# mario-linov/graphs4cfd

Measured on AMD Instinct MI355X. Metric: rollout timesteps/s (100k-node 2D mesh), higher is better.
Workload: dtype f32 (MLP products: two-way fp16 split of both operands, 22 significand bits each, 3 partial products on the f16 MFMA pipe, fp32 accumulate; error vs fp64 within that of an fp32 GEMM)

## Files before the change

### graphs4cfd_amd/_lib.py

```python
from __future__ import annotations

import ctypes as C
import os
from typing import Optional

import torch

_HERE = os.path.dirname(os.path.abspath(__file__))
LIB_PATH = os.environ.get("G4C_LIB_PATH") or os.path.join(_HERE, "lib", "libg4c.so")

OK, EINVAL, ELAUNCH, EUNSUPPORTED = 0, -1, -2, -3
ACT_NONE, ACT_SELU, ACT_TANH = 0, 1, 2
MAX_SRC, MAX_LAYERS = 4, 4
MAX_HEADS = 2
NARROW_MAX = 8
KERNEL_MLP_RS = 5
KERNEL_MLP_RS2 = 6
KERNEL_MLP_BX6, KERNEL_MLP_WS = 2, 4
KERNEL_MLP_BX6_CERT, KERNEL_MLP_WS_CERT = 7, 8
KERNEL_NAMES = {0: "none", 1: "mlp_split_kernel", 2: "mlp_bx6_kernel", 3: "mlp_bx6i_kernel", 4: "mlp_ws_kernel", 5: "mlp_rs1_kernel", 6: "mlp_rs2_kernel",
                7: "mlp_bx6_kernel", 8: "mlp_ws_kernel"}

TILE_SHAPE_GENERIC, TILE_SHAPE_NODE, TILE_SHAPE_UP, TILE_SHAPE_DOWN = 0, 1, 2, 3

_ACT_CODES = {None: ACT_NONE, "none": ACT_NONE, "selu": ACT_SELU, "tanh": ACT_TANH}


def act_code(activation) -> Optional[int]:
    if activation is None or isinstance(activation, str):
        return _ACT_CODES[activation]
    if activation is torch.tanh or activation is torch.nn.functional.tanh:
        return ACT_TANH
    if activation is torch.nn.functional.selu or activation is torch.selu:
        return ACT_SELU
    return None


class g4c_src_t(C.Structure):
    _fields_ = [("ptr", C.c_void_p), ("idx", C.c_void_p), ("width", C.c_int32), ("ld", C.c_int32),
                ("col0", C.c_int32), ("pre_act", C.c_int32), ("additive", C.c_int32), ("seg_mean", C.c_int32),
                ("w", C.c_void_p), ("seg_off", C.c_void_p), ("seg_perm", C.c_void_p), ("dtype", C.c_int32)]


class g4c_mlp_t(C.Structure):
    _fields_ = [("n_layers", C.c_int32), ("k_pad", C.c_int32 * MAX_LAYERS), ("n_pad", C.c_int32 * MAX_LAYERS),
                ("w", C.c_void_p * MAX_LAYERS), ("b", C.c_void_p * MAX_LAYERS),
                ("ln_gamma", C.c_void_p), ("ln_beta", C.c_void_p), ("ln_eps", C.c_float), ("n_out", C.c_int32), ("w_format", C.c_int32),
                ("range_slot", C.c_int32), ("range_certified", C.c_int32)]


WFMT_FP32, WFMT_F16X2, WFMT_BF16X3, WFMT_BF16_RS, WFMT_BF16_RS2, WFMT_BF16_RS2N, WFMT_BF16 = 0, 1, 2, 3, 4, 5, 6
DTYPE_F32, DTYPE_BF16 = 0, 1


class g4c_mlp_io_t(C.Structure):
    _fields_ = [("size", C.c_int32), ("act", C.c_int32), ("row_begin", C.c_int64), ("row_count", C.c_int64),
                ("out", C.c_void_p), ("out_ld", C.c_int32), ("out_dtype", C.c_int32), ("out_idx", C.c_void_p),
                ("resid", C.c_void_p), ("resid_ld", C.c_int32), ("resid_col0", C.c_int32),
                ("n_heads", C.c_int32), ("head_ld", C.c_int32), ("head_dtype", C.c_int32), ("head_out", C.c_void_p * MAX_HEADS),
                ("tile_rows", C.c_void_p), ("tile_seg", C.c_void_p), ("seg_off", C.c_void_p), ("n_tiles", C.c_int32),
                ("agg", C.c_void_p), ("agg_ld", C.c_int32), ("agg_mode", C.c_int32),
                ("n_save", C.c_int32), ("save", C.c_void_p * MAX_LAYERS), ("save_ld", C.c_int32),
                ("mul", C.c_void_p * MAX_LAYERS), ("mul_ld", C.c_int32),
                ("upd", C.POINTER(g4c_mlp_t)), ("v", C.c_void_p), ("v_ld", C.c_int32), ("v_act", C.c_int32),
                ("v_out", C.c_void_p), ("v_out_ld", C.c_int32), ("range_flag", C.c_void_p),
                ("save_dtype", C.c_int32), ("mul_dtype", C.c_int32)]

    def __init__(self, **kw):
        super().__init__(size=C.sizeof(g4c_mlp_io_t), **kw)


_SIGNATURES = {
    "g4c_version": (C.c_int, []),
    "g4c_device_info": (C.c_int, [C.c_void_p, C.POINTER(C.c_int32), C.POINTER(C.c_int32)]),
    "g4c_last_error": (C.c_char_p, []),
    "g4c_plan_csr": (C.c_int, [C.c_void_p, C.c_int64, C.c_int64, C.c_void_p, C.c_void_p]),
    "g4c_plan_pool_edge": (C.c_int64, [C.c_void_p, C.c_int64, C.c_void_p, C.c_int64, C.c_void_p, C.c_void_p,
                                       C.c_void_p, C.c_void_p]),
    "g4c_plan_pool_edge_ordered": (C.c_int64, [C.c_void_p, C.c_int64, C.c_void_p, C.c_int64, C.c_int32, C.c_void_p, C.c_void_p,
                                               C.c_void_p, C.c_void_p]),
    "g4c_segment_reduce": (C.c_int, [C.c_void_p, C.c_int32, C.c_void_p, C.c_void_p, C.c_int32, C.c_int32, C.c_int32,
                                     C.c_int32, C.c_int32, C.c_void_p, C.c_int32, C.c_void_p]),
    "g4c_weighted_segment_mean": (C.c_int, [C.c_void_p, C.c_int32, C.c_void_p, C.c_void_p, C.c_void_p, C.c_int32,
                                            C.c_int32, C.c_void_p, C.c_int32, C.c_void_p, C.c_void_p]),
    "g4c_mlp_pack_layer": (C.c_int, [C.c_void_p, C.c_int32, C.c_int32, C.c_void_p, C.c_void_p, C.c_int32, C.c_int32, C.c_void_p,
                                     C.c_int32, C.c_int32, C.c_void_p]),
    "g4c_mlp_run": (C.c_int, [C.POINTER(g4c_mlp_t), C.POINTER(g4c_src_t), C.c_int32, C.c_int64, C.POINTER(g4c_mlp_io_t), C.c_void_p]),
    "g4c_plan_tiles": (C.c_int64, [C.c_void_p, C.c_int32, C.c_int32, C.c_void_p, C.c_void_p, C.c_int64]),
    "g4c_mlp_bx6i_enable": (C.c_int, [C.c_int]),
    "g4c_mlp_ws_enable": (C.c_int, [C.c_int]),
    "g4c_mlp_small_launch_tiles": (C.c_int, [C.c_int]),
    "g4c_layer_norm": (C.c_int, [C.c_void_p, C.c_int32, C.c_int64, C.c_int32, C.c_void_p, C.c_void_p, C.c_float, C.c_int32, C.c_void_p, C.c_int32, C.c_void_p]),
    "g4c_debug_mean_div": (C.c_int, [C.c_void_p, C.c_void_p, C.c_void_p, C.c_int64, C.c_void_p]),
    "g4c_mlp_last_kernel": (C.c_int, []),
    "g4c_mlp_shapes_enable": (C.c_int, [C.c_int]),
    "g4c_mlp_last_shape": (C.c_int, []),
    "g4c_project_to_edges": (C.c_int, [C.c_void_p, C.c_int32, C.c_void_p, C.c_void_p, C.c_int64, C.c_int32,
                                       C.c_void_p, C.c_int32, C.c_void_p]),
    "g4c_edge_scalar_to_node_vector": (C.c_int, [C.c_void_p, C.c_int32, C.c_void_p, C.c_int32, C.c_int64, C.c_int32,
                                                 C.c_void_p, C.c_int32, C.c_void_p]),
    "g4c_knn_grid": (C.c_int, [C.c_void_p, C.c_void_p, C.c_void_p, C.c_void_p, C.c_int64, C.c_int32, C.c_void_p,
                               C.c_void_p, C.c_float, C.c_int32, C.c_void_p, C.c_void_p]),
    "g4c_knn_grid_query": (C.c_int, [C.c_void_p, C.c_void_p, C.c_void_p, C.c_int64, C.c_int32, C.c_void_p, C.c_void_p,
                                     C.c_float, C.c_void_p, C.c_void_p, C.c_int64, C.c_int32, C.c_void_p, C.c_void_p]),
    "g4c_rollout_advance": (C.c_int, [C.c_void_p, C.c_int32, C.c_void_p, C.c_int32, C.c_void_p, C.c_int32,
                                      C.c_void_p, C.c_int64, C.c_void_p]),
    "g4c_activation_inplace": (C.c_int, [C.c_void_p, C.c_int64, C.c_int32, C.c_void_p]),
    "g4c_add_cols": (C.c_int, [C.c_void_p, C.c_int32, C.c_int32, C.c_void_p, C.c_int32, C.c_void_p, C.c_int32,
                               C.c_int32, C.c_int64, C.c_void_p]),
    "g4c_copy_cols": (C.c_int, [C.c_void_p, C.c_int32, C.c_int32, C.c_void_p, C.c_void_p, C.c_int32, C.c_int32,
                                C.c_int32, C.c_int64, C.c_void_p]),
    "g4c_train_gather": (C.c_int, [C.c_void_p, C.c_int32, C.c_int32, C.c_void_p, C.c_int32, C.c_int32, C.c_void_p, C.c_int32,
                                   C.c_int32, C.c_int32, C.c_int64, C.c_int32, C.c_void_p]),
    "g4c_act_grad": (C.c_int, [C.c_void_p, C.c_int32, C.c_void_p, C.c_int32, C.c_int32, C.c_int32, C.c_void_p, C.c_int32,
                               C.c_int32, C.c_int64, C.c_void_p]),
    "g4c_act_grad_ref16": (C.c_int, [C.c_void_p, C.c_int32, C.c_void_p, C.c_int32, C.c_int32, C.c_int32, C.c_void_p, C.c_int32,
                                     C.c_int32, C.c_int64, C.c_void_p]),
    "g4c_layernorm_grad_partials": (C.c_int32, [C.c_int64]),
    "g4c_layernorm_grad": (C.c_int, [C.c_void_p, C.c_int32, C.c_void_p, C.c_void_p, C.c_int32, C.c_void_p, C.c_int32,
                                     C.c_void_p, C.c_int32, C.c_int64, C.c_float, C.c_void_p]),
    "g4c_layernorm_grad_z16": (C.c_int, [C.c_void_p, C.c_int32, C.c_void_p, C.c_void_p, C.c_int32, C.c_void_p, C.c_int32,
                                         C.c_void_p, C.c_int32, C.c_int64, C.c_float, C.c_void_p]),
    "g4c_colsum_partials": (C.c_int32, [C.c_int64]),
    "g4c_colsum": (C.c_int, [C.c_void_p, C.c_int32, C.c_int32, C.c_int64, C.c_void_p, C.c_void_p, C.c_void_p]),
    "g4c_weight_grad_partials": (C.c_int32, [C.c_int64]),
    "g4c_weight_grad_scratch_floats": (C.c_int64, [C.c_int64]),
    "g4c_weight_grad": (C.c_int, [C.c_void_p, C.c_int32, C.c_void_p, C.c_int32, C.c_int64, C.c_void_p, C.c_void_p, C.c_int32,
                                  C.c_void_p]),
    "g4c_weight_grad_bf16": (C.c_int, [C.c_void_p, C.c_int32, C.c_void_p, C.c_int32, C.c_int64, C.c_void_p, C.c_void_p, C.c_int32,
                                       C.c_void_p]),
    "g4c_weight_grad_bf16_a16": (C.c_int, [C.c_void_p, C.c_int32, C.c_void_p, C.c_int32, C.c_int64, C.c_void_p, C.c_void_p, C.c_int32,
                                           C.c_void_p]),
    "g4c_segment_broadcast": (C.c_int, [C.c_void_p, C.c_int32, C.c_void_p, C.c_void_p, C.c_int32, C.c_int32, C.c_int32,
                                        C.c_void_p, C.c_int32, C.c_void_p]),
}

EXPORTED_SYMBOLS = tuple(_SIGNATURES)

_lib = None


def load() -> C.CDLL:
    global _lib
    if _lib is None:
        if not os.path.exists(LIB_PATH):
            raise RuntimeError(
                f"graphs4cfd_amd: HIP library not found at {LIB_PATH}. Build it with "
                "`python -c 'import __graft_entry__ as g; g.build()'` (hipcc --offload-arch=gfx950). "
                "There is no CPU fallback.")
        lib = C.CDLL(LIB_PATH)
        for name, (res, args) in _SIGNATURES.items():
            fn = getattr(lib, name)
            fn.restype, fn.argtypes = res, args
        _lib = lib
    return _lib


def check(code: int) -> None:
    if code == OK:
        return
    msg = load().g4c_last_error().decode("utf-8", "replace")
    if code == EINVAL:
        raise ValueError(msg)
    if code == EUNSUPPORTED:
        raise NotImplementedError(msg)
    raise RuntimeError(msg)


def require_hip(*tensors: torch.Tensor) -> torch.device:
    dev = None
    for t in tensors:
        if t is None:
            continue
        if not t.is_cuda:
# ... 16 lines not shown
```

### graphs4cfd_amd/csrc/mlp_common.h

```cpp
#pragma once
#include "g4c_common.h"
#include <type_traits>

#ifndef G4C_ABLATE
#define G4C_ABLATE 0
#endif

namespace g4cm {

constexpr int KC = 32;
constexpr int XS = KC + 2;
constexpr int HS = 128 + 4;
constexpr int NP = 128;
constexpr int CHUNK_FLOATS = KC * NP;

typedef float f32x16 __attribute__((ext_vector_type(16)));
typedef float f32x8 __attribute__((ext_vector_type(8)));
typedef float f32x4 __attribute__((ext_vector_type(4)));
typedef float f32x2 __attribute__((ext_vector_type(2)));

struct Src {
    const float *ptr;
    const int *idx;
    int width, wpad, ld, col0, vec, pre_act;
// ... 101 lines not shown
    const u32x4 v = __builtin_amdgcn_raw_buffer_load_b128(rs, voff_bytes, soff_bytes, 0);
    return __builtin_bit_cast(bf16x8, v);
}

__device__ __forceinline__ f32x4 selu4(f32x4 x) {
    f32x4 y;
#pragma unroll
    for (int e = 0; e < 4; ++e) y[e] = g4c::selu_f(x[e]);
    return y;
}
__device__ __forceinline__ f32x2 selu2(f32x2 x) {
    f32x2 y;
    y[0] = g4c::selu_f(x[0]); y[1] = g4c::selu_f(x[1]);
    return y;
}

typedef __bf16 bf16x2 __attribute__((ext_vector_type(2)));
__device__ __forceinline__ unsigned pack_bf16(f32x2 x, f32x2 &back) {
    bf16x2 b;
    b[0] = (__bf16)x[0]; b[1] = (__bf16)x[1];
    const unsigned u = __builtin_bit_cast(unsigned, b);
    back[0] = __builtin_bit_cast(float, u << 16);
    back[1] = __builtin_bit_cast(float, u & 0xffff0000u);
    return u;
}
typedef _Float16 f16x8 __attribute__((ext_vector_type(8)));
typedef _Float16 f16x2 __attribute__((ext_vector_type(2)));
constexpr float F16_LO_SCALE = 2048.f, F16_LO_UNSCALE = 1.f / 2048.f;
__device__ __forceinline__ f32x16 mfma_f16(bf16x8 a, bf16x8 b, f32x16 c) {
    return __builtin_amdgcn_mfma_f32_32x32x16_f16(__builtin_bit_cast(f16x8, a), __builtin_bit_cast(f16x8, b), c, 0, 0, 0);
}
#ifndef G4C_F16_SATURATE
#define G4C_F16_SATURATE 1
#endif
__device__ __forceinline__ void f16_range_mode() { if (G4C_F16_SATURATE) __builtin_amdgcn_s_setreg(1 | (23 << 6) | (0 << 11), 1); }
__device__ __forceinline__ unsigned pack_f16(f32x2 x, f32x2 &back) {
    f16x2 b;
    b[0] = (_Float16)x[0]; b[1] = (_Float16)x[1];
    back[0] = (float)b[0]; back[1] = (float)b[1];
    return __builtin_bit_cast(unsigned, b);
}
#ifndef G4C_SPLIT_MIX
#define G4C_SPLIT_MIX 1
#endif
constexpr float F16_RANGE_END = 65504.f;
struct RangeV { float m = 0.f; };
struct RangeS { unsigned long long any = 0ull; };
struct RangeNone {};
__device__ __forceinline__ void range_track(RangeNone &, f32x2) {}
__device__ __forceinline__ void range_track(RangeNone &, f32x4) {}
__device__ __forceinline__ bool range_hit(const RangeNone &) { return false; }
__device__ __forceinline__ void range_track(RangeV &r, f32x2 y) { r.m = fmaxf(fmaxf(r.m, fabsf(y[0])), fabsf(y[1])); }
__device__ __forceinline__ void range_track(RangeS &r, f32x2 y) {
    r.any |= __builtin_amdgcn_ballot_w64(fmaxf(fabsf(y[0]), fabsf(y[1])) >= F16_RANGE_END);
}
__device__ __forceinline__ void range_track(RangeV &r, f32x4 y) {
    f32x2 a, b; a[0] = y[0]; a[1] = y[1]; b[0] = y[2]; b[1] = y[3];
    range_track(r, a); range_track(r, b);
}
__device__ __forceinline__ void range_track(RangeS &r, f32x4 y) {
    r.any |= __builtin_amdgcn_ballot_w64(fmaxf(fmaxf(fmaxf(fabsf(y[0]), fabsf(y[1])), fabsf(y[2])), fabsf(y[3])) >= F16_RANGE_END);
}
__device__ __forceinline__ bool range_hit(const RangeV &r) { return __builtin_amdgcn_ballot_w64(r.m >= F16_RANGE_END) != 0ull; }
__device__ __forceinline__ bool range_hit(const RangeS &r) { return r.any != 0ull; }
template <class R>
__device__ __forceinline__ void range_report(const Params &p, const R &r) {
    if (p.range_flag && range_hit(r)) {
        if ((threadIdx.x & 63) == 0) p.range_flag[p.range_slot] = 1;
    }
}
__device__ __forceinline__ void split_pair_f16(f32x2 y, unsigned &hu, unsigned &lu) {
    f16x2 b;
    b[0] = (_Float16)y[0]; b[1] = (_Float16)y[1];
    hu = __builtin_bit_cast(unsigned, b);
    if (G4C_SPLIT_MIX) {
        const f32x2 ys = y * F16_LO_SCALE;
        const float c = -F16_LO_SCALE;
        asm("v_fma_mixlo_f16 %0, %1, %2, %3 op_sel_hi:[1,0,0]" : "=v"(lu) : "v"(hu), "s"(c), "v"(ys[0]));
        asm("v_fma_mixhi_f16 %0, %1, %2, %3 op_sel:[1,0,0] op_sel_hi:[1,0,0]" : "+v"(lu) : "v"(hu), "s"(c), "v"(ys[1]));
    } else {
        f32x2 hf, lf;
        hf[0] = (float)b[0]; hf[1] = (float)b[1];
        lu = pack_f16((y - hf) * F16_LO_SCALE, lf);
    }
}
template <class R>
__device__ __forceinline__ void split_pair_f16(f32x2 y, unsigned &hu, unsigned &lu, R &rng) {
    range_track(rng, y);
    split_pair_f16(y, hu, lu);
}
template <class R>
__device__ __forceinline__ void split2x4(f32x4 x, bf16x4 &h, bf16x4 &l, R &rng) {
    range_track(rng, x);
    unsigned hu[2], lu[2];
#pragma unroll
    for (int j = 0; j < 2; ++j) {
        f32x2 v;
        v[0] = x[2 * j]; v[1] = x[2 * j + 1];
        split_pair_f16(v, hu[j], lu[j]);
    }
    typedef unsigned u32x2 __attribute__((ext_vector_type(2)));
    u32x2 hh, ll;
    hh[0] = hu[0]; hh[1] = hu[1]; ll[0] = lu[0]; ll[1] = lu[1];
    h = __builtin_bit_cast(bf16x4, hh); l = __builtin_bit_cast(bf16x4, ll);
}
__device__ __forceinline__ void split2(float x, __bf16 &h, __bf16 &l) {
    const _Float16 a = (_Float16)x;
    const _Float16 b = (_Float16)((x - (float)a) * F16_LO_SCALE);
    h = __builtin_bit_cast(__bf16, a); l = __builtin_bit_cast(__bf16, b);
}

template <int SP, class R> __device__ __forceinline__ void split3x4(f32x4 x, bf16x4 &h, bf16x4 &m, bf16x4 &l, R &rng);
template <int SP = 3>
__device__ __forceinline__ void split3x4(f32x4 x, bf16x4 &h, bf16x4 &m, bf16x4 &l) { RangeNone none; split3x4<SP>(x, h, m, l, none); }
template <int SP, class R>
__device__ __forceinline__ void split3x4(f32x4 x, bf16x4 &h, bf16x4 &m, bf16x4 &l, R &rng) {
    if (SP == 2) { split2x4(x, h, m, rng); l = m; return; }
    if (SP == 1 || (G4C_ABLATE & 512)) {
#pragma unroll
        for (int e = 0; e < 4; ++e) { h[e] = (__bf16)x[e]; m[e] = h[e]; l[e] = h[e]; }
        return;
    }
    unsigned hu[2], mu[2], lu[2];
#pragma unroll
    for (int j = 0; j < 2; ++j) {
        f32x2 v, hf, mf, lf;
        v[0] = x[2 * j]; v[1] = x[2 * j + 1];
        hu[j] = pack_bf16(v, hf);
        const f32x2 r1 = v - hf;
        mu[j] = pack_bf16(r1, mf);
        const f32x2 r2 = r1 - mf;
        lu[j] = pack_bf16(r2, lf);
    }
    typedef unsigned u32x2 __attribute__((ext_vector_type(2)));
    u32x2 hh, mm, ll;
    hh[0] = hu[0]; hh[1] = hu[1]; mm[0] = mu[0]; mm[1] = mu[1]; ll[0] = lu[0]; ll[1] = lu[1];
    h = __builtin_bit_cast(bf16x4, hh); m = __builtin_bit_cast(bf16x4, mm); l = __builtin_bit_cast(bf16x4, ll);
}

__device__ __forceinline__ void split3(float x, __bf16 &h, __bf16 &m, __bf16 &l) {
    h = (__bf16)x;
    const float r1 = x - (float)h;
    m = (__bf16)r1;
    l = (__bf16)(r1 - (float)m);
}

struct Launch {
    Params p;
    NodeParams node;
    bool has_node;
    int fmt;
    bool round1, f16x2, bx6, row_split;
    bool agg, save;
    bool all_vec;
    long long row_begin, row_count;
    int io_n_tiles;
    bool deep_ring, shapes;
};
struct Ran { int kernel = G4C_KERNEL_NONE, shape = G4C_TILE_SHAPE_GENERIC; };

inline bool message_form(const Launch &L) {
    const Params &p = L.p;
    const Src &s = p.src[0];
    if (L.save || p.n_src != 1 || p.n_nar != 0 || (p.n_add != 0 && p.n_add != 2) || p.n_heads || p.n_out != NP || p.resid) return false;
    if (p.out_idx && (L.agg || !p.out)) return false;
    if (s.width != NP || !s.vec || s.seg_off) return false;
    for (int a = 0; a < p.n_add; ++a)
        if (p.add[a].width != NP || (p.add[a].ld & 3) || ((uintptr_t)p.add[a].ptr & (p.add[a].bf16 ? 7 : 15))) return false;
    if (p.out && !p.out_bf16 && ((p.out_ld & 3) || ((uintptr_t)p.out & 15))) return false;
    if (p.gamma && (((uintptr_t)p.gamma & 15) || ((uintptr_t)p.beta & 15))) return false;
    return ((uintptr_t)p.b & 15) == 0 && p.M < (1LL << 31);
}

bool split_takes(const Launch &L);
int split_launch(const Launch &L, hipStream_t st, Ran &ran);
bool tile_takes(const Launch &L);
int tile_launch(const Launch &L, hipStream_t st, Ran &ran);
bool bx6i_takes(const Launch &L);
int bx6i_launch(const Launch &L, hipStream_t st, Ran &ran);
bool ws_takes(const Launch &L);
int ws_launch(const Launch &L, hipStream_t st, Ran &ran);
bool rs_takes(const Launch &L);
int rs_launch(const Launch &L, hipStream_t st, Ran &ran);
bool rs2_takes(const Launch &L);
int rs2_launch(const Launch &L, hipStream_t st, Ran &ran);

typedef unsigned u32x2 __attribute__((ext_vector_type(2)));
__device__ __forceinline__ f32x4 widen_bf16x4(u32x2 w) {
    f32x4 x;
    x[0] = __builtin_bit_cast(float, w[0] << 16); x[1] = __builtin_bit_cast(float, w[0] & 0xffff0000u);
    x[2] = __builtin_bit_cast(float, w[1] << 16); x[3] = __builtin_bit_cast(float, w[1] & 0xffff0000u);
    return x;
}


}
```

### graphs4cfd_amd/csrc/mlp_run.hip

```cpp
#include "mlp_common.h"
#include <atomic>
#include <climits>
using namespace g4cm;

namespace {

std::atomic<int> g_ws_mode{1};
std::atomic<int> g_bx6i_mode{1};
std::atomic<int> g_deep_tiles{512};
#ifndef G4C_TILE_SHAPES_DEFAULT
#define G4C_TILE_SHAPES_DEFAULT 1
#endif
std::atomic<int> g_shapes{G4C_TILE_SHAPES_DEFAULT};

constexpr long long WS_MIN_ROWS = 20000;
constexpr long long BX6I_MIN_ROWS = 400000;

int knob(std::atomic<int> &k, int value, int max_value) {
    const int prev = k.load(std::memory_order_relaxed);
    if (value >= 0) k.store(value > max_value ? max_value : value, std::memory_order_relaxed);
    return prev;
}

thread_local Ran g_last;

int stage_call(const g4c_mlp_t *mlp, const g4c_src_t *srcs, int32_t n_src, int64_t n_rows, const g4c_mlp_io_t *io, Launch &L) {
    G4C_REQUIRE(io && io->size == (int32_t)sizeof(g4c_mlp_io_t), G4C_EINVAL,
                "g4c_mlp_run: io->size %d, this library's g4c_mlp_io_t has %d bytes (a binding out of step with g4c.h)", io ? io->size : 0,
                (int)sizeof(g4c_mlp_io_t));
    G4C_REQUIRE(mlp && srcs, G4C_EINVAL, "g4c_mlp_run: null pointer");
    const int fmt = L.fmt = mlp->w_format;
    G4C_REQUIRE(fmt >= G4C_WFMT_FP32 && fmt <= G4C_WFMT_BF16, G4C_EINVAL, "g4c_mlp_run: unknown w_format %d", fmt);
    L.row_split = fmt == G4C_WFMT_BF16_RS || fmt == G4C_WFMT_BF16_RS2 || fmt == G4C_WFMT_BF16_RS2N;
    L.round1 = fmt == G4C_WFMT_BF16 || L.row_split;
    L.f16x2 = fmt == G4C_WFMT_F16X2;
    L.bx6 = fmt != G4C_WFMT_FP32;
    L.agg = io->agg != nullptr; L.save = io->n_save != 0; L.has_node = io->upd != nullptr;
    L.row_begin = io->row_begin; L.row_count = io->row_count; L.io_n_tiles = io->n_tiles;
    G4C_REQUIRE(L.row_begin >= 0 && L.row_count >= 0 && L.row_begin + L.row_count <= n_rows && L.row_begin % 32 == 0, G4C_EINVAL,
                "g4c_mlp_run: bad row range [%lld, +%lld) of %lld (row_begin must be a multiple of 32)", L.row_begin, L.row_count,
                (long long)n_rows);
    G4C_REQUIRE(n_src >= 1 && n_src <= G4C_MAX_SRC, G4C_EUNSUPPORTED, "g4c_mlp_run: %d sources (max %d)", n_src, G4C_MAX_SRC);
    G4C_REQUIRE(mlp->n_layers >= 1 && mlp->n_layers <= G4C_MAX_LAYERS, G4C_EUNSUPPORTED,
                "g4c_mlp_run: %d layers (supported 1..%d)", mlp->n_layers, G4C_MAX_LAYERS);
    G4C_REQUIRE(n_rows >= 0 && n_rows < (1LL << 31), G4C_EINVAL, "g4c_mlp_run: n_rows %lld out of range", (long long)n_rows);
    G4C_REQUIRE(io->act >= 0 && io->act <= 2, G4C_EINVAL, "g4c_mlp_run: bad activation %d", io->act);
    G4C_REQUIRE(io->n_heads >= 0 && io->n_heads <= G4C_MAX_HEADS, G4C_EINVAL, "g4c_mlp_run: bad heads (n=%d)", io->n_heads);
    G4C_REQUIRE((L.row_begin == 0 && L.row_count == n_rows) || (!L.agg && !L.save && !L.has_node && !io->n_heads && !io->out_dtype),
                G4C_EUNSUPPORTED, "g4c_mlp_run: a row sub-range needs a plain launch (no heads / aggregation / save / upd / out_dtype)");
    G4C_REQUIRE(!L.agg || (io->tile_rows && io->tile_seg && io->seg_off && io->n_tiles >= 0 && io->agg_ld >= NP), G4C_EINVAL,
                "g4c_mlp_run: bad aggregation plan");
    G4C_REQUIRE(io->out_dtype == G4C_DTYPE_F32 || io->out_dtype == G4C_DTYPE_BF16 || io->out_dtype == G4C_DTYPE_BF16_SELU, G4C_EINVAL,
                "g4c_mlp_run: unknown out_dtype %d", io->out_dtype);
    G4C_REQUIRE(io->out_dtype != G4C_DTYPE_BF16_SELU || (L.agg && io->act == G4C_ACT_NONE), G4C_EINVAL,
                "g4c_mlp_run: G4C_DTYPE_BF16_SELU needs the fused aggregation and no output activation");
    G4C_REQUIRE(io->head_dtype == G4C_DTYPE_F32 || io->head_dtype == G4C_DTYPE_BF16, G4C_EINVAL, "g4c_mlp_run: unknown head_dtype %d", io->head_dtype);
    G4C_REQUIRE(!io->range_flag || (mlp->range_slot >= 0 && (!L.has_node || io->upd->range_slot >= 0)), G4C_EINVAL,
                "g4c_mlp_run: negative range_slot (mlp %d, upd %d)", mlp->range_slot, L.has_node ? io->upd->range_slot : 0);
    return G4C_OK;
}

int stage_sources(const g4c_src_t *srcs, int32_t n_src, int32_t k_pad0, Launch &L) {
    Params &p = L.p;
    const bool bx6 = L.bx6, round1 = L.round1;
    int kp = 0, nk = 0;
    L.all_vec = true;
    for (int s = 0; s < n_src; ++s) {
        const g4c_src_t &g = srcs[s];
        G4C_REQUIRE(g.ptr && g.width > 0 && g.ld >= g.col0 + g.width && g.col0 >= 0, G4C_EINVAL,
                    "g4c_mlp_run: bad source %d (width=%d ld=%d col0=%d)", s, g.width, g.ld, g.col0);
        if (g.additive == 2) {
            G4C_REQUIRE(bx6, G4C_EUNSUPPORTED, "g4c_mlp_run: narrow sources (additive == 2) need a split-operand w_format");
            G4C_REQUIRE(g.width <= G4C_NARROW_MAX && !g.idx && g.pre_act == G4C_ACT_NONE && g.w && ((uintptr_t)g.w & 15) == 0, G4C_EINVAL,
                        "g4c_mlp_run: bad narrow source %d (width %d <= %d, no index, no pre_act, 16-byte aligned weights)", s,
                        g.width, G4C_NARROW_MAX);
            NarSrc &a = p.nar[p.n_nar++];
            a.ptr = g.ptr + g.col0; a.w = g.w; a.width = g.width; a.ld = g.ld;
            continue;
        }
        if (g.additive) {
            G4C_REQUIRE(g.pre_act == G4C_ACT_NONE && g.width <= NP && (g.dtype == G4C_DTYPE_F32 || g.dtype == G4C_DTYPE_BF16), G4C_EINVAL,
                        "g4c_mlp_run: bad additive source %d", s);
            AddSrc &a = p.add[p.n_add++];
            a.idx = g.idx; a.width = g.width; a.ld = g.ld; a.bf16 = g.dtype == G4C_DTYPE_BF16;
            if (a.bf16) {
                G4C_REQUIRE(round1 && g.width == NP && g.ld % 4 == 0 && g.col0 % 4 == 0 && (uintptr_t)g.ptr % 8 == 0, G4C_EUNSUPPORTED,
                            "g4c_mlp_run: bf16 additive rows need the rounded-bf16 mode (w_format G4C_WFMT_BF16*) and a 128-wide, 8-byte aligned block");
                a.ptr = reinterpret_cast<const float *>(reinterpret_cast<const __bf16 *>(g.ptr) + g.col0);
            } else {
                a.ptr = g.ptr + g.col0;
            }
            continue;
        }
        G4C_REQUIRE(g.pre_act == G4C_ACT_NONE || g.pre_act == G4C_ACT_SELU, G4C_EUNSUPPORTED,
                    "g4c_mlp_run: source %d pre_act %d (only NONE / SELU can be applied on load)", s, g.pre_act);
        Src &d = p.src[nk++];
        if (bx6) G4C_REQUIRE(g.width <= NP, G4C_EUNSUPPORTED, "g4c_mlp_run: input block %d is %d wide (max 128 in a split-operand w_format)", s, g.width);
        d.ptr = g.ptr; d.idx = g.idx; d.width = g.width; d.wpad = bx6 ? NP : (g.width + KC - 1) / KC * KC; d.ld = g.ld; d.col0 = g.col0;
        d.pre_act = g.pre_act;
        d.bf16 = g.dtype == G4C_DTYPE_BF16;
        if (d.bf16)
            G4C_REQUIRE(round1 && g.width == NP && !g.seg_off && g.ld % 4 == 0 && g.col0 % 4 == 0 && (uintptr_t)g.ptr % 8 == 0, G4C_EUNSUPPORTED,
                        "g4c_mlp_run: bf16 rows need the rounded-bf16 mode (w_format G4C_WFMT_BF16*) and a 128-wide, 8-byte aligned block");
        else
            G4C_REQUIRE(g.dtype == G4C_DTYPE_F32, G4C_EINVAL, "g4c_mlp_run: source %d has unknown dtype %d", s, g.dtype);
        d.seg_off = g.seg_off; d.seg_mean = g.seg_mean; d.seg_perm = g.seg_off ? g.seg_perm : nullptr;
        if (g.seg_off)
            G4C_REQUIRE(bx6 && !g.idx && g.width == NP && g.ld % 4 == 0 && g.col0 % 4 == 0 && (uintptr_t)g.ptr % 16 == 0, G4C_EUNSUPPORTED,
                        "g4c_mlp_run: aggregation on load needs a split-operand w_format and a 128-wide aligned block without gather index");
        d.vec = (g.width % 4 == 0) && (g.ld % 4 == 0) && (g.col0 % 4 == 0) && ((uintptr_t)g.ptr % (d.bf16 ? 8 : 16) == 0);
        L.all_vec = L.all_vec && d.vec;
        kp += d.wpad;
    }
    G4C_REQUIRE(nk >= 1 || p.n_nar >= 1, G4C_EINVAL, "g4c_mlp_run: no input block goes through the weights");
    p.n_src = nk;
    if (nk == 0) p.src[0] = Src{nullptr, nullptr, 0, 0, 0, 0, 1, 0, nullptr, 0, nullptr, 0};
    for (int s = (nk ? nk : 1); s < G4C_MAX_SRC; ++s) p.src[s] = p.src[0];
    G4C_REQUIRE(kp == k_pad0, G4C_EINVAL, "g4c_mlp_run: sources give %d padded columns, layer 1 packed for %d", kp, k_pad0);
    p.chunks0 = kp / KC;
    return G4C_OK;
}

int check_contiguous(const g4c_mlp_t *m, int wbytes, const char *w_text, const char *b_text) {
    for (int l = 1; l < m->n_layers; ++l) {
        G4C_REQUIRE((const char *)m->w[l] == (const char *)m->w[l - 1] + (size_t)m->k_pad[l - 1] * NP * wbytes, G4C_EINVAL, w_text, l);
        G4C_REQUIRE((const float *)m->b[l] == (const float *)m->b[l - 1] + NP, G4C_EINVAL, b_text, l);
    }
    return G4C_OK;
}

int stage_stream(const g4c_mlp_t *mlp, Launch &L) {
    Params &p = L.p;
    p.n_layers = mlp->n_layers;
    for (int l = 0; l < mlp->n_layers; ++l) {
        G4C_REQUIRE(mlp->n_pad[l] == NP, G4C_EINVAL, "g4c_mlp_run: layer %d n_pad %d (must be 128)", l, mlp->n_pad[l]);
        if (l > 0) G4C_REQUIRE(mlp->k_pad[l] == NP, G4C_EINVAL, "g4c_mlp_run: layer %d k_pad %d (must be 128)", l, mlp->k_pad[l]);
    }
    if (const int rc = check_contiguous(mlp, L.bx6 ? 6 : 4, "g4c_mlp_run: packed layers must be contiguous (layer %d)",
                                        "g4c_mlp_run: padded biases must be contiguous (layer %d)"))
        return rc;
    p.w = (const float *)mlp->w[0]; p.b = (const float *)mlp->b[0];
    G4C_REQUIRE(p.w && p.b, G4C_EINVAL, "g4c_mlp_run: null weights");
    p.gamma = mlp->ln_gamma; p.beta = mlp->ln_beta; p.eps = mlp->ln_eps;
    G4C_REQUIRE((p.gamma == nullptr) == (p.beta == nullptr), G4C_EINVAL, "g4c_mlp_run: LayerNorm needs both gamma and beta");
    p.n_out = mlp->n_out;
    return G4C_OK;
}

int stage_outputs(const g4c_mlp_io_t *io, Launch &L) {
    Params &p = L.p;
    p.out = (float *)io->out; p.out_ld = io->out_ld; p.out_idx = io->out_idx; p.act = io->act;
    G4C_REQUIRE(p.out || L.agg, G4C_EINVAL, "g4c_mlp_run: null output");
    G4C_REQUIRE(p.n_out > 0 && p.n_out <= NP && p.out_ld >= p.n_out, G4C_EINVAL, "g4c_mlp_run: n_out=%d out_ld=%d", p.n_out, p.out_ld);
    p.resid = io->resid; p.resid_ld = io->resid_ld; p.resid_col0 = io->resid_col0;
    p.row_base = L.row_begin;
    p.M = L.row_begin + L.row_count;
    if (L.agg) {
        G4C_REQUIRE(L.bx6 && p.n_out == NP && !p.out_idx && !p.resid, G4C_EUNSUPPORTED,
                    "g4c_mlp_run: the fused aggregation needs a split-operand w_format and a plain 128-wide output");
        const int32_t mode = io->agg_mode;
        p.tile_rows = io->tile_rows; p.tile_seg = io->tile_seg; p.seg_off = io->seg_off;
        p.agg = (float *)io->agg; p.agg_ld = io->agg_ld; p.agg_mean = mode & 1; p.agg_deg = (mode >> 8) & 0xff; p.agg_bf16 = (mode >> 16) & 1;
        const bool rs_fmt = L.fmt == G4C_WFMT_BF16_RS;
        G4C_REQUIRE((mode >> 17) == 0 && (!p.agg_bf16 || rs_fmt) && p.agg_deg <= 32 && (p.agg_deg == 0 || L.row_count % p.agg_deg == 0), G4C_EINVAL,
                    "fused aggregation: agg_mode = %d is not 0 / 1 [| G4C_AGG_UNIFORM(k), 1 <= k <= 32, k dividing the %lld rows]", mode,
                    L.row_count);
        G4C_REQUIRE(p.agg_deg == 0 || L.row_begin == 0, G4C_EINVAL,
                    "g4c_mlp_run: uniform segments (G4C_AGG_UNIFORM) need the whole row range, got rows [%lld, %lld)", L.row_begin, p.M);
    }
    if (io->out_dtype) {
        G4C_REQUIRE(L.round1 && !p.resid && !p.out_idx && p.n_out == NP && (!p.out || ((p.out_ld & 3) == 0 && ((uintptr_t)p.out & 7) == 0)), G4C_EUNSUPPORTED,
                    "g4c_mlp_run: bf16 output rows need the rounded-bf16 mode, a plain 128-wide output, out_ld a multiple of 4 and an 8-byte aligned out");
        p.out_bf16 = io->out_dtype;
    }
    return G4C_OK;
}

int stage_save(const g4c_mlp_io_t *io, Launch &L) {
    Params &p = L.p;
    const int n_layers = p.n_layers;
    if (!L.save) return G4C_OK;
    G4C_REQUIRE(L.bx6 && (!L.round1 || L.fmt == G4C_WFMT_BF16) && !io->out_dtype && !L.agg && !io->n_heads && !p.out_idx && io->save_ld >= NP &&
                    (io->save_ld & 3) == 0,
                G4C_EUNSUPPORTED,
                "g4c_mlp_run: save needs w_format BF16X3 / F16X2 / BF16 without heads / aggregation / output index / bf16 rows, save_ld >= 128 "
                "and a multiple of 4");
    G4C_REQUIRE(io->n_save == n_layers, G4C_EINVAL, "g4c_mlp_run: n_save %d for %d layers", io->n_save, n_layers);
    G4C_REQUIRE((io->save_dtype == G4C_DTYPE_F32 || io->save_dtype == G4C_DTYPE_BF16) &&
                    (io->mul_dtype == G4C_DTYPE_F32 || io->mul_dtype == G4C_DTYPE_BF16),
                G4C_EINVAL, "g4c_mlp_run: save_dtype %d / mul_dtype %d (G4C_DTYPE_F32 or G4C_DTYPE_BF16)", io->save_dtype, io->mul_dtype);
    G4C_REQUIRE((!io->save_dtype && !io->mul_dtype) || L.fmt == G4C_WFMT_BF16, G4C_EINVAL,
                "g4c_mlp_run: bf16 save / mul rows need w_format G4C_WFMT_BF16 (the plain rounded-bf16 stream); w_format %d keeps fp32 rows",
                L.fmt);
    bool mul = false;
    for (int l = 0; l < n_layers; ++l) {
        G4C_REQUIRE(((uintptr_t)io->save[l] & 15) == 0, G4C_EINVAL, "g4c_mlp_run: save[%d] is not 16-byte aligned", l);
        p.save[l] = static_cast<float *>(io->save[l]);
        if (l + 1 == n_layers) break;
        G4C_REQUIRE(((uintptr_t)io->mul[l] & 15) == 0, G4C_EINVAL, "g4c_mlp_run: mul[%d] is not 16-byte aligned", l);
        p.mul[l] = static_cast<const float *>(io->mul[l]);
        mul = mul || io->mul[l];
    }
    p.save_bf16 = io->save_dtype == G4C_DTYPE_BF16;
    p.mul_bf16 = io->mul_dtype == G4C_DTYPE_BF16;
    p.save_ld = io->save_ld;
    G4C_REQUIRE(!mul || (io->mul_ld >= NP && (io->mul_ld & 3) == 0), G4C_EINVAL, "g4c_mlp_run: mul_ld=%d", io->mul_ld);
    p.mul_ld = io->mul_ld;
    return G4C_OK;
}

void stage_range(const g4c_mlp_t *mlp, const g4c_mlp_io_t *io, Launch &L) {
    L.p.range_certified = (L.f16x2 && mlp->range_certified && !L.save && (!L.has_node || io->upd->range_certified)) ? 1 : 0;
    L.p.range_flag = (L.f16x2 && !L.p.range_certified) ? io->range_flag : nullptr;
    L.p.range_slot = mlp->range_slot;
}

int stage_heads(const g4c_mlp_io_t *io, Launch &L) {
    Params &p = L.p;
    const int n_heads = io->n_heads;
    for (int hd = 0; hd < n_heads; ++hd) G4C_REQUIRE(io->head_out[hd], G4C_EINVAL, "g4c_mlp_run: null head output %d", hd);
    if (L.has_node || !n_heads) return G4C_OK;
    p.n_heads = n_heads; p.head_ld = io->head_ld;
    for (int hd = 0; hd < n_heads; ++hd) p.head_out[hd] = (float *)io->head_out[hd];
    if (io->head_dtype) {
        G4C_REQUIRE(L.round1 && (p.head_ld & 1) == 0, G4C_EUNSUPPORTED, "g4c_mlp_run: bf16 head rows need the rounded-bf16 mode and an even head_ld");
        for (int hd = 0; hd < n_heads; ++hd)
            G4C_REQUIRE(((uintptr_t)io->head_out[hd] & 3) == 0, G4C_EINVAL, "g4c_mlp_run: head output %d is not 4-byte aligned", hd);
        p.head_bf16 = 1;
    }
    G4C_REQUIRE(!L.agg, G4C_EUNSUPPORTED, "g4c_mlp_run: heads with the fused aggregation");
    G4C_REQUIRE((p.head_ld & 3) == 0 || !L.bx6, G4C_EINVAL, "g4c_mlp_run: head outputs need a leading dimension that is a multiple of 4");
    G4C_REQUIRE(p.n_out == NP && !p.resid && !p.out_idx && p.head_ld >= NP, G4C_EINVAL,
                "g4c_mlp_run: heads need a 128-wide output without residual / output index (n_out=%d)", p.n_out);
    return G4C_OK;
}

int stage_node(const g4c_mlp_io_t *io, Launch &L) {
    if (!L.has_node) return G4C_OK;
    const g4c_mlp_t *u = io->upd;
    const int n_heads = io->n_heads;
    G4C_REQUIRE(L.f16x2 && L.agg && u->w_format == G4C_WFMT_F16X2 && io->act == G4C_ACT_NONE, G4C_EUNSUPPORTED,
                "g4c_mlp_run: the fused node update needs the f16x3 format (G4C_WFMT_F16X2) for both MLPs, the aggregation plan and act NONE");
    G4C_REQUIRE(u->n_layers == L.p.n_layers && u->k_pad[0] == 2 * NP && u->n_out == NP && u->w[0] && u->b[0], G4C_EUNSUPPORTED,
                "g4c_mlp_run: upd must have the message MLP's depth (%d), two 128-wide input blocks and a 128-wide output", L.p.n_layers);
    for (int l = 0; l < u->n_layers; ++l)
        G4C_REQUIRE(u->n_pad[l] == NP && (l == 0 || u->k_pad[l] == NP), G4C_EUNSUPPORTED, "g4c_mlp_run: upd layer %d is not 128 wide", l);
    const char *const text = "g4c_mlp_run: upd's packed layers / biases must be contiguous (layer %d)";
    if (const int rc = check_contiguous(u, 6, text, text)) return rc;
    G4C_REQUIRE((u->ln_gamma == nullptr) == (u->ln_beta == nullptr), G4C_EINVAL, "g4c_mlp_run: upd's LayerNorm needs both gamma and beta");
    G4C_REQUIRE(!u->ln_gamma || (((uintptr_t)u->ln_gamma & 15) == 0 && ((uintptr_t)u->ln_beta & 15) == 0), G4C_EINVAL,
                "g4c_mlp_run: upd's LayerNorm parameters must be 16-byte aligned");
    G4C_REQUIRE(io->v && io->v_out && (io->v_ld & 3) == 0 && io->v_ld >= NP && (io->v_out_ld & 3) == 0 && io->v_out_ld >= NP &&
                ((uintptr_t)io->v & 15) == 0 && ((uintptr_t)io->v_out & 15) == 0 && (io->agg_ld & 3) == 0 && ((uintptr_t)io->agg & 15) == 0,
                G4C_EINVAL, "g4c_mlp_run: v / v_out / agg need 16-byte aligned rows of at least 128 columns");
    G4C_REQUIRE(io->v_act >= 0 && io->v_act <= 2, G4C_EINVAL, "g4c_mlp_run: bad v_act %d", io->v_act);
    NodeParams &q = L.node;
    q.v = io->v; q.v_ld = io->v_ld; q.w = (const float *)u->w[0]; q.b = (const float *)u->b[0];
    q.gamma = u->ln_gamma; q.beta = u->ln_beta; q.eps = u->ln_eps; q.act = io->v_act;
    q.out = io->v_out; q.out_ld = io->v_out_ld; q.n_heads = n_heads; q.head_ld = io->head_ld;
    q.range_flag = L.p.range_certified ? nullptr : io->range_flag; q.range_slot = u->range_slot;
    if (n_heads) {
        G4C_REQUIRE(io->head_dtype == G4C_DTYPE_F32 && (io->head_ld & 3) == 0 && io->head_ld >= NP, G4C_EINVAL,
                    "g4c_mlp_run: upd's heads need fp32 rows, head_ld a multiple of 4 and >= 128");
        for (int hd = 0; hd < n_heads; ++hd) {
            G4C_REQUIRE(((uintptr_t)io->head_out[hd] & 15) == 0, G4C_EINVAL, "g4c_mlp_run: bad head output %d", hd);
            q.head_out[hd] = (float *)io->head_out[hd];
        }
    }
    return G4C_OK;
}

typedef int (*LaunchFn)(const Launch &, hipStream_t, Ran &);

bool at_size(const std::atomic<int> &mode_knob, long long min_rows, const Launch &L) {
    const int mode = mode_knob.load(std::memory_order_relaxed);
    return mode == 2 || (mode == 1 && L.row_count >= min_rows);
}

LaunchFn choose(Launch &L) {
    L.deep_ring = L.p.n_tiles <= g_deep_tiles.load(std::memory_order_relaxed);
    L.shapes = g_shapes.load(std::memory_order_relaxed) != 0;
    if (L.has_node) {
        G4C_REQUIRE(ws_takes(L), nullptr,
                    "g4c_mlp_run: the message launch of the fused MP layer is outside the weight-stationary kernel's envelope (one 128-wide "
                    "weighted block, two 128-wide additive blocks, two or three 128-wide layers, aligned rows)");
        return ws_launch;
    }
    if (L.fmt == G4C_WFMT_BF16_RS) {
        G4C_REQUIRE(!L.save && rs_takes(L), nullptr,
                    "g4c_mlp_run: weights packed for the row-split kernel (G4C_WFMT_BF16_RS), launch outside its envelope");
        return rs_launch;
    }
    if (L.row_split) {
        G4C_REQUIRE(!L.save && !L.agg && rs2_takes(L), nullptr,
                    "g4c_mlp_run: weights packed for the row-split update kernel (G4C_WFMT_BF16_RS2), launch outside its envelope");
        return rs2_launch;
    }
    if (at_size(g_ws_mode, WS_MIN_ROWS, L) && ws_takes(L)) return ws_launch;
    if (at_size(g_bx6i_mode, BX6I_MIN_ROWS, L) && bx6i_takes(L)) return bx6i_launch;
    return tile_takes(L) ? tile_launch : split_launch;
}

}

extern "C" int g4c_mlp_run(const g4c_mlp_t *mlp, const g4c_src_t *srcs, int32_t n_src, int64_t n_rows, const g4c_mlp_io_t *io,
                           void *stream) {
    g_last = Ran{};
    Launch L{};
    int rc;
    if ((rc = stage_call(mlp, srcs, n_src, n_rows, io, L))) return rc;
    if (n_rows == 0) return G4C_OK;
    g4c::DeviceGuard on_device(mlp->w[0]);
    if ((rc = stage_sources(srcs, n_src, mlp->k_pad[0], L))) return rc;
    if ((rc = stage_stream(mlp, L))) return rc;
    if ((rc = stage_outputs(io, L))) return rc;
    if ((rc = stage_save(io, L))) return rc;
    stage_range(mlp, io, L);
    if ((rc = stage_heads(io, L))) return rc;
    if (L.row_count == 0) return G4C_OK;
    if ((rc = stage_node(io, L))) return rc;
    L.p.n_tiles = (L.agg && !L.row_split) ? L.io_n_tiles : (int)((L.row_count + 31) / 32);
    const LaunchFn launch = choose(L);
    if (!launch) return G4C_EUNSUPPORTED;
    if (L.p.n_tiles == 0) return G4C_OK;
    return launch(L, (hipStream_t)stream, g_last);
}

extern "C" int g4c_mlp_ws_enable(int on) { return knob(g_ws_mode, on, 2); }
extern "C" int g4c_mlp_bx6i_enable(int on) { return knob(g_bx6i_mode, on, 2); }
extern "C" int g4c_mlp_small_launch_tiles(int n_tiles) { return knob(g_deep_tiles, n_tiles, INT_MAX); }
extern "C" int g4c_mlp_shapes_enable(int on) { return knob(g_shapes, on, 1); }
extern "C" int g4c_mlp_last_kernel(void) { return g_last.kernel; }
extern "C" int g4c_mlp_last_shape(void) { return g_last.shape; }
```

### graphs4cfd_amd/csrc/mlp_ws.hip

```cpp
#include "mlp_common.h"
#include <cstdlib>
using namespace g4cm;

#ifdef G4C_WS_TIMING
__device__ unsigned long long g4c_ws_stamps[256 * 32];
extern "C" int g4c_ws_read_stamps(unsigned long long *host, int n) {
    return (int)hipMemcpyFromSymbol(host, HIP_SYMBOL(g4c_ws_stamps), sizeof(unsigned long long) * n);
}
#define WS_STAMP(k) do { if (it == 1 && tid == 0 && blockIdx.x < 256) g4c_ws_stamps[blockIdx.x * 32 + (k)] = __builtin_readcyclecounter(); } while (0)
#define WS_STAMP_T(k) do { if (its == 1 && tid == 0 && blockIdx.x < 256) { asm volatile("s_waitcnt lgkmcnt(0)" ::: "memory"); g4c_ws_stamps[blockIdx.x * 32 + (k)] = __builtin_readcyclecounter(); } } while (0)
#define WS_STAMP_ONCE(k, v) do { if (tid == 0 && blockIdx.x < 256) g4c_ws_stamps[blockIdx.x * 32 + (k)] = (v); } while (0)
#else
#define WS_STAMP(k) do {} while (0)
#define WS_STAMP_T(k) do {} while (0)
#define WS_STAMP_ONCE(k, v) do {} while (0)
#endif

#ifndef G4C_WS_ABLATE
#define G4C_WS_ABLATE 0
#endif

namespace {

constexpr int PS = 128;
constexpr int PLN = 32 * PS;
constexpr int TILE_BF16 = 2 * PLN;
constexpr int FIN = 32 * HS;
constexpr int SEGCAP = 64;

template <int SP>
__device__ __forceinline__ f32x4 mfma16(bf16x8 a, bf16x8 b, f32x4 c) {
    if constexpr (SP == 1) return __builtin_amdgcn_mfma_f32_16x16x32_bf16(a, b, c, 0, 0, 0);
    else return __builtin_amdgcn_mfma_f32_16x16x32_f16(__builtin_bit_cast(f16x8, a), __builtin_bit_cast(f16x8, b), c, 0, 0, 0);
}

struct Meta { int r0[2], n[2], s0[2], s1[2]; };

struct Other {
    __bf16 *plane_acc;
    __bf16 *plane_park;
    float *fin;
};

template <bool LOADED = false>
__device__ __forceinline__ f32x2 selu2w(f32x2 x) {
    if (G4C_WS_ABLATE & 16) return x;
    if constexpr (!LOADED) return selu2(x);
    const float sa = 1.6732632423543772848170429916717f * 1.0507009873554804934193349852946f;
    const float scale = 1.0507009873554804934193349852946f;
    f32x2 r;
#pragma unroll
    for (int e = 0; e < 2; ++e) {
        const float ex = __builtin_amdgcn_fmed3f(__builtin_amdgcn_exp2f(x[e] * 1.4426950408889634f), 0.f, 1.f);
        float m;
        asm("v_max_f32 %0, 0, %1" : "=v"(m) : "v"(x[e]));
        r[e] = fmaf(m, scale, fmaf(sa, ex, -sa));
    }
    return r;
}

#ifndef G4C_WS_SCALED
#define G4C_WS_SCALED 1
#endif
#ifndef G4C_WS_MEAN_DIV
#define G4C_WS_MEAN_DIV 1
#endif


template <bool LOADED = false>
__device__ __forceinline__ f32x2 selu2w_scaled(f32x2 x) {
    const float sa = 1.6732632423543772848170429916717f * 1.0507009873554804934193349852946f * F16_LO_SCALE;
    const float scale = 1.0507009873554804934193349852946f * F16_LO_SCALE;
    f32x2 r;
#pragma unroll
    for (int e = 0; e < 2; ++e) {
        const float ex = __builtin_amdgcn_fmed3f(__builtin_amdgcn_exp2f(x[e] * 1.4426950408889634f), 0.f, 1.f);
        float m;
        if constexpr (LOADED) asm("v_max_f32 %0, 0, %1" : "=v"(m) : "v"(x[e]));
        else m = fmaxf(x[e], 0.f);
        r[e] = fmaf(m, scale, fmaf(sa, ex, -sa));
    }
    return r;
}
__device__ __forceinline__ void range_track_scaled(RangeV &rng, f32x2 S) { rng.m = fmaxf(fmaxf(rng.m, fabsf(S[0])), fabsf(S[1])); }
__device__ __forceinline__ void range_track_scaled(RangeNone &, f32x2) {}
template <class R>
__device__ __forceinline__ void put_pair_scaled(__bf16 *d, f32x2 S, R &rng) {
    range_track_scaled(rng, S);
    unsigned hu, lu;
    const float up = F16_LO_UNSCALE, dn = -F16_LO_SCALE;
    asm("v_fma_mixlo_f16 %0, %2, %4, 0\n\t"
        "v_fma_mixhi_f16 %0, %3, %4, 0\n\t"
        "v_fma_mixlo_f16 %1, %0, %5, %2 op_sel_hi:[1,0,0]\n\t"
        "v_fma_mixhi_f16 %1, %0, %5, %3 op_sel:[1,0,0] op_sel_hi:[1,0,0]"
        : "=&v"(hu), "=&v"(lu) : "v"(S[0]), "v"(S[1]), "s"(up), "s"(dn));
    *reinterpret_cast<unsigned *>(d) = hu;
    *reinterpret_cast<unsigned *>(d + PLN) = lu;
}

template <int SP, class R>
__device__ __forceinline__ void put_pair(__bf16 *d, f32x2 y, R &rng) {
    if constexpr (SP == 1) {
        typedef __bf16 bf16x2 __attribute__((ext_vector_type(2)));
        bf16x2 b;
        b[0] = (__bf16)y[0]; b[1] = (__bf16)y[1];
        *reinterpret_cast<bf16x2 *>(d) = b;
    } else {
        unsigned hu, lu;
        split_pair_f16(y, hu, lu, rng);
        if (G4C_WS_ABLATE & 32) lu = hu;
        *reinterpret_cast<unsigned *>(d) = hu;
        *reinterpret_cast<unsigned *>(d + PLN) = lu;
    }
}

__device__ __forceinline__ float row16_sum(float v) {
    v += __builtin_bit_cast(float, __builtin_amdgcn_update_dpp(0, __builtin_bit_cast(int, v), 0xB1, 0xF, 0xF, false));
    v += __builtin_bit_cast(float, __builtin_amdgcn_update_dpp(0, __builtin_bit_cast(int, v), 0x4E, 0xF, 0xF, false));
    v += __builtin_bit_cast(float, __builtin_amdgcn_update_dpp(0, __builtin_bit_cast(int, v), 0x141, 0xF, 0xF, false));
    v += __builtin_bit_cast(float, __builtin_amdgcn_update_dpp(0, __builtin_bit_cast(int, v), 0x140, 0xF, 0xF, false));
    return v;
}

__device__ __forceinline__ void row16_sum2(float &a, float &b) {
#define G4C_DPP_ADD(v, ctrl) v += __builtin_bit_cast(float, __builtin_amdgcn_update_dpp(0, __builtin_bit_cast(int, v), ctrl, 0xF, 0xF, false))
    G4C_DPP_ADD(a, 0xB1); G4C_DPP_ADD(b, 0xB1);
    G4C_DPP_ADD(a, 0x4E); G4C_DPP_ADD(b, 0x4E);
    G4C_DPP_ADD(a, 0x141); G4C_DPP_ADD(b, 0x141);
    G4C_DPP_ADD(a, 0x140); G4C_DPP_ADD(b, 0x140);
#undef G4C_DPP_ADD
}

template <int SP, int EK, bool PACT, class R>
__device__ __forceinline__ void other_piece(int s, const f32x4 (&accE)[2], const f32x4 (&accE1)[2], const f32x4 (&xe)[2], const Other &o, f32x2 &hold, R &rng) {
    const int u = s >> 2, pc4 = s & 3, pr = pc4 >> 1;
    if (EK == 1) {
        if ((pc4 & 1) == 0) {
            f32x2 x, x1;
            x[0] = accE[u][2 * pr]; x[1] = accE[u][2 * pr + 1];
            x1[0] = accE1[u][2 * pr]; x1[1] = accE1[u][2 * pr + 1];
            if (SP == 2 && G4C_WS_SCALED && !(G4C_WS_ABLATE & 48)) hold = selu2w_scaled(x1 * F16_LO_UNSCALE + x);
            else hold = SP == 1 ? selu2w(x) : selu2w(x1 * F16_LO_UNSCALE + x);
        } else {
            if (SP == 2 && G4C_WS_SCALED && !(G4C_WS_ABLATE & 48)) put_pair_scaled(o.plane_acc + u * 16 * PS + 2 * pr, hold, rng);
            else put_pair<SP>(o.plane_acc + u * 16 * PS + 2 * pr, hold, rng);
        }
    } else if (EK == 2) {
        if ((pc4 & 1) == 0) {
            f32x2 x;
            x[0] = xe[u][2 * pr]; x[1] = xe[u][2 * pr + 1];
            if (SP == 2 && G4C_WS_SCALED && !(G4C_WS_ABLATE & 48)) hold = PACT ? selu2w_scaled<true>(x) : x * F16_LO_SCALE;
            else hold = PACT ? selu2w<true>(x) : x;
        } else {
            if (SP == 2 && G4C_WS_SCALED && !(G4C_WS_ABLATE & 48)) put_pair_scaled(o.plane_park + u * 16 * PS + 2 * pr, hold, rng);
            else put_pair<SP>(o.plane_park + u * 16 * PS + 2 * pr, hold, rng);
        }
    } else if (EK == 3) {
        if (pc4 == 0) {
            f32x4 x;
#pragma unroll
            for (int e = 0; e < 4; ++e) x[e] = SP == 1 ? accE[u][e] : fmaf(accE1[u][e], F16_LO_UNSCALE, accE[u][e]);
            *reinterpret_cast<f32x4 *>(o.fin + u * 16 * HS) = x;
        }
    }
}

constexpr int WS_VALU_PER_MFMA = 4;
constexpr int WS_FRAG_AHEAD = 2;
template <int SP, int EK, bool PACT = false, class R>
__device__ __forceinline__ void m_block(const __bf16 *const (&pa)[4], const bf16x8 (&W)[4][SP], f32x4 (&acc)[2], f32x4 (&acc1)[2],
                                        const f32x4 (&accE)[2], const f32x4 (&accE1)[2], const f32x4 (&xe)[2], const Other &o, R &rng) {
    constexpr int AH = WS_FRAG_AHEAD, RING = AH + 1;
    bf16x8 fh[RING], fl[RING];
#pragma unroll
    for (int s = 0; s < AH; ++s) {
        const __bf16 *pn = pa[s >> 1] + (s & 1) * 16 * PS;
        fh[s] = *reinterpret_cast<const bf16x8 *>(pn);
        if (SP == 2) fl[s] = *reinterpret_cast<const bf16x8 *>(pn + PLN);
    }
    f32x2 hold = {0.f, 0.f};
#pragma unroll
    for (int s = 0; s < 8; ++s) {
        const int ks = s >> 1, rb = s & 1;
        if (s + AH < 8 && !(G4C_WS_ABLATE & 4)) {
            const __bf16 *pn = pa[(s + AH) >> 1] + ((s + AH) & 1) * 16 * PS;
            fh[(s + AH) % RING] = *reinterpret_cast<const bf16x8 *>(pn);
            if (SP == 2) fl[(s + AH) % RING] = *reinterpret_cast<const bf16x8 *>(pn + PLN);
        }
        if (!EK) __builtin_amdgcn_sched_barrier(0);
        if constexpr (EK == 4) {
            other_piece<SP, 3, false>(s, accE, accE1, xe, o, hold, rng);
            other_piece<SP, 2, PACT>(s, accE, accE1, xe, o, hold, rng);
        } else {
            other_piece<SP, EK, PACT>(s, accE, accE1, xe, o, hold, rng);
        }
        const bf16x8 ch = fh[s % RING];
        if constexpr (SP == 1) {
            acc[rb] = mfma16<1>(W[ks][0], ch, acc[rb]);
        } else {
            const bf16x8 cl = fl[s % RING];
            if (G4C_WS_ABLATE & 2) {
                asm volatile("" :: "v"(ch), "v"(cl));
            } else {
                acc1[rb] = mfma16<2>(W[ks][0], cl, acc1[rb]);
                acc[rb] = mfma16<2>(W[ks][0], ch, acc[rb]);
                acc1[rb] = mfma16<2>(W[ks][1], ch, acc1[rb]);
            }
        }
        if (EK) {
            __builtin_amdgcn_sched_group_barrier(0x100, SP, 0);
#pragma unroll
            for (int m = 0; m < (SP == 2 ? 3 : 1); ++m) {
                __builtin_amdgcn_sched_group_barrier(0x008, 1, 0);
                __builtin_amdgcn_sched_group_barrier(0x002, SP == 2 ? WS_VALU_PER_MFMA : 3 * WS_VALU_PER_MFMA, 0);
            }
            __builtin_amdgcn_sched_group_barrier(0x200, SP, 0);
        }
        __builtin_amdgcn_sched_barrier(0);
    }
}

template <int SP, int EK, bool PACT, class R>
__device__ __forceinline__ void other_all(const f32x4 (&accE)[2], const f32x4 (&accE1)[2], const f32x4 (&xe)[2], const Other &o, R &rng) {
    f32x2 hold = {0.f, 0.f};
#pragma unroll
    for (int s = 0; s < 8; ++s) other_piece<SP, EK, PACT>(s, accE, accE1, xe, o, hold, rng);
}

struct NodeCtx {
    int tid, wave, n, g, fcol, prow, pc;
    unsigned lo_b;
    const float *sBiasN, *sGBN;
    float *fA, *fB;
    Other oA, oB;
    const __bf16 *paA[4], *paB[4];
};

template <int SP, int NL, bool TRACK>
__device__ __forceinline__ void node_phase(const NodeCtx &c, const float *x0, const int x0_ld, const NodeParams &q, const int S0, const int S1) {
    const int wave = c.wave, n = c.n, g = c.g, fcol = c.fcol, prow = c.prow, pc = c.pc;
    const unsigned lo_b = c.lo_b;
    const float *const sBiasN = c.sBiasN, *const sGBN = c.sGBN;
    float *const fA = c.fA, *const fB = c.fB;
    const Other &oA = c.oA, &oB = c.oB;
    const __bf16 *const (&paA)[4] = c.paA;
    const __bf16 *const (&paB)[4] = c.paB;
    f32x4 accA[2], accB[2], accA1[2], accB1[2];
    const __amdgpu_buffer_rsrc_t rq = __builtin_amdgcn_make_buffer_rsrc(const_cast<float *>(q.w), 0, 0x7fffffff, 0x00020000);
    typename std::conditional<TRACK, RangeV, RangeNone>::type rngN;
    const int n_blk = NL + 1 + q.n_heads;
    auto ld_block = [&](bf16x8 (&Wb)[4][SP], int blk) __attribute__((always_inline)) {
        if (blk >= n_blk) return;
#pragma unroll
        for (int ks = 0; ks < 4; ++ks)
#pragma unroll
            for (int pl = 0; pl < SP; ++pl) Wb[ks][pl] = ldw(rq, lo_b + 1024u * pl, (unsigned)blk * 2u * BLOCK6 + (unsigned)ks * 4u * STEP6);
    };
    auto bias_n = [&](f32x4 (&acc)[2], f32x4 (&acc1)[2], int l) __attribute__((always_inline)) {
        f32x4 b4 = {0.f, 0.f, 0.f, 0.f};
        if (l >= 0) b4 = *reinterpret_cast<const f32x4 *>(sBiasN + l * NP + fcol);
        acc[0] = b4; acc[1] = b4;
        acc1[0] = f32x4{0.f, 0.f, 0.f, 0.f}; acc1[1] = f32x4{0.f, 0.f, 0.f, 0.f};
    };
    const int rowL = wave * 4 + g;
    const int cqn[2] = {n * 4, 64 + n * 4};
    auto finish_rows = [&](float *frows, int rb, int nrows) __attribute__((always_inline)) {
        float x[8];
        float *const rowp = frows + rowL * HS;
#pragma unroll
        for (int c = 0; c < 8; c += 4) {
            const f32x4 v4 = *reinterpret_cast<const f32x4 *>(rowp + cqn[c >> 2]);
            x[c] = v4[0]; x[c + 1] = v4[1]; x[c + 2] = v4[2]; x[c + 3] = v4[3];
        }
        if (q.gamma) {
            float sum = 0.f;
#pragma unroll
            for (int c = 0; c < 8; ++c) sum += x[c];
            sum = row16_sum(sum);
            const float mean = sum * (1.0f / NP);
            float var = 0.f;
#pragma unroll
            for (int c = 0; c < 8; ++c) { const float dl = x[c] - mean; var += dl * dl; }
            var = row16_sum(var);
            const float rstd = rsqrtf(var * (1.0f / NP) + q.eps);
#pragma unroll
            for (int c = 0; c < 8; c += 4) {
                const f32x4 g4 = *reinterpret_cast<const f32x4 *>(sGBN + cqn[c >> 2]), b4 = *reinterpret_cast<const f32x4 *>(sGBN + NP + cqn[c >> 2]);
#pragma unroll
                for (int u = 0; u < 4; ++u) x[c + u] = fmaf((x[c + u] - mean) * rstd, g4[u], b4[u]);
            }
        }
        if (q.act == G4C_ACT_SELU) {
#pragma unroll
            for (int c = 0; c < 8; ++c) x[c] = g4c::selu_f(x[c]);
        } else if (q.act == G4C_ACT_TANH) {
#pragma unroll
            for (int c = 0; c < 8; ++c) x[c] = g4c::tanh_f(x[c]);
        }
        f32x4 v0, v1;
        v0[0] = x[0]; v0[1] = x[1]; v0[2] = x[2]; v0[3] = x[3]; v1[0] = x[4]; v1[1] = x[5]; v1[2] = x[6]; v1[3] = x[7];
        if (q.n_heads) { *reinterpret_cast<f32x4 *>(rowp + cqn[0]) = v0; *reinterpret_cast<f32x4 *>(rowp + cqn[1]) = v1; }
        if (rowL < nrows) {
            float *op = q.out + (long long)(rb + rowL) * q.out_ld;
            *reinterpret_cast<f32x4 *>(op + cqn[0]) = v0; *reinterpret_cast<f32x4 *>(op + cqn[1]) = v1;
        }
    };
    auto store_head = [&](int hd, const float *frows, int rb, int nrows) __attribute__((always_inline)) {
        if (rowL < nrows) {
            const float *rowp = frows + rowL * HS;
            float *op = q.head_out[hd] + (long long)(rb + rowL) * q.head_ld;
            *reinterpret_cast<f32x4 *>(op + cqn[0]) = *reinterpret_cast<const f32x4 *>(rowp + cqn[0]);
            *reinterpret_cast<f32x4 *>(op + cqn[1]) = *reinterpret_cast<const f32x4 *>(rowp + cqn[1]);
        }
    };
    auto load_rows = [&](const float *base, int ld, int rb, int nrows, f32x4 (&x)[2]) __attribute__((always_inline)) {
#pragma unroll
        for (int hh = 0; hh < 2; ++hh) {
            const int r = prow + 16 * hh;
            x[hh] = *reinterpret_cast<const f32x4 *>(base + (long long)(rb + (r < nrows ? r : nrows - 1)) * ld + pc);
        }
    };
    for (int r0 = S0; r0 < S1; r0 += 64) {
        const int nr = (S1 - r0) < 64 ? (S1 - r0) : 64;
        bf16x8 Wa[4][SP], Wb[4][SP];
        ld_block(Wa, 0); ld_block(Wb, 1);
        auto &H0 = (NL == 3) ? Wa : Wb;
        auto &H1 = (NL == 3) ? Wb : Wa;
        f32x4 ga[2], va[2], gb[2], vb[2];
        {
            const int nA = nr < 32 ? nr : 32;
            load_rows(x0, x0_ld, r0, nA, ga); load_rows(q.v, q.v_ld, r0, nA, va);
            if (nr > 32) { load_rows(x0, x0_ld, r0 + 32, nr - 32, gb); load_rows(q.v, q.v_ld, r0 + 32, nr - 32, vb); }
        }
        if (nr > 32) {
            const int nB = nr - 32;
            other_all<SP, 2, false>(accA, accA1, ga, oA, rngN);
            other_all<SP, 2, false>(accA, accA1, gb, oB, rngN);
            bias_n(accA, accA1, 0); bias_n(accB, accB1, 0);
            __syncthreads();
            m_block<SP, 0>(paA, Wa, accA, accA1, accA, accA1, ga, oA, rngN);
            __syncthreads();
            m_block<SP, 2, false>(paB, Wa, accB, accB1, accB, accB1, va, oA, rngN);
            ld_block(Wa, 2);
            __syncthreads();
            m_block<SP, 2, false>(paA, Wb, accA, accA1, accA, accA1, vb, oB, rngN);
// ... 9 lines not shown
                m_block<SP, 1>(paB, Wa, accB, accB1, accA, accA1, va, oA, rngN);
                ld_block(Wa, 4);
                bias_n(accA, accA1, 2);
                __syncthreads();
                m_block<SP, 1>(paA, Wb, accA, accA1, accB, accB1, va, oB, rngN);
                bias_n(accB, accB1, 2);
                __syncthreads();
                m_block<SP, 3>(paB, Wb, accB, accB1, accA, accA1, va, oA, rngN);
                ld_block(Wb, 5);
            } else {
                m_block<SP, 3>(paB, Wa, accB, accB1, accA, accA1, va, oA, rngN);
                ld_block(Wa, 4);
            }
            other_all<SP, 3, false>(accB, accB1, va, oB, rngN);
            __syncthreads();
            finish_rows(fA, r0, 32);
            finish_rows(fB, r0 + 32, nB);
            if (q.n_heads) {
                __syncthreads();
                f32x4 ha[2], hb[2];
#pragma unroll
                for (int hh = 0; hh < 2; ++hh) {
                    ha[hh] = *reinterpret_cast<const f32x4 *>(fA + (prow + 16 * hh) * HS + pc);
                    hb[hh] = *reinterpret_cast<const f32x4 *>(fB + (prow + 16 * hh) * HS + pc);
                }
                other_all<SP, 2, false>(accA, accA1, ha, oA, rngN);
                other_all<SP, 2, false>(accA, accA1, hb, oB, rngN);
                bias_n(accA, accA1, -1); bias_n(accB, accB1, -1);
                __syncthreads();
                m_block<SP, 0>(paA, H0, accA, accA1, accA, accA1, va, oA, rngN);
                m_block<SP, 3>(paB, H0, accB, accB1, accA, accA1, va, oA, rngN);
                bias_n(accA, accA1, -1);
                __syncthreads();
                store_head(0, fA, r0, 32);
                if (q.n_heads > 1) {
                    m_block<SP, 3>(paA, H1, accA, accA1, accB, accB1, va, oB, rngN);
                    bias_n(accB, accB1, -1);
                    __syncthreads();
                    store_head(0, fB, r0 + 32, nB);
                    m_block<SP, 3>(paB, H1, accB, accB1, accA, accA1, va, oA, rngN);
                    __syncthreads();
                    store_head(1, fA, r0, 32);
                    other_all<SP, 3, false>(accB, accB1, va, oB, rngN);
                    __syncthreads();
                    store_head(1, fB, r0 + 32, nB);
                } else {
                    other_all<SP, 3, false>(accB, accB1, va, oB, rngN);
                    __syncthreads();
                    store_head(0, fB, r0 + 32, nB);
                }
            }
            __syncthreads();
            continue;
        }
        other_all<SP, 2, false>(accA, accA1, ga, oA, rngN);
        other_all<SP, 2, false>(accA, accA1, va, oB, rngN);
        bias_n(accA, accA1, 0);
        __syncthreads();
        m_block<SP, 0>(paA, Wa, accA, accA1, accA, accA1, ga, oA, rngN);
        ld_block(Wa, 2);
        m_block<SP, 0>(paB, Wb, accA, accA1, accA, accA1, ga, oA, rngN);
        ld_block(Wb, 3);
        __syncthreads();
        other_all<SP, 1, false>(accA, accA1, ga, oA, rngN);
        bias_n(accA, accA1, 1);
        __syncthreads();
        m_block<SP, 0>(paA, Wa, accA, accA1, accA, accA1, ga, oA, rngN);
        if constexpr (NL == 3) {
            ld_block(Wa, 4);
            other_all<SP, 1, false>(accA, accA1, ga, oB, rngN);
            bias_n(accA, accA1, 2);
            __syncthreads();
            m_block<SP, 0>(paB, Wb, accA, accA1, accA, accA1, ga, oA, rngN);
            ld_block(Wb, 5);
        } else {
            ld_block(Wa, 4);
        }
        other_all<SP, 3, false>(accA, accA1, ga, oA, rngN);
        __syncthreads();
        finish_rows(fA, r0, nr);
        if (q.n_heads) {
            __syncthreads();
            f32x4 xh[2];
#pragma unroll
            for (int hh = 0; hh < 2; ++hh) xh[hh] = *reinterpret_cast<const f32x4 *>(fA + (prow + 16 * hh) * HS + pc);
            other_all<SP, 2, false>(accA, accA1, xh, oA, rngN);
            bias_n(accA, accA1, -1);
            bias_n(accB, accB1, -1);
            __syncthreads();
            m_block<SP, 0>(paA, H0, accA, accA1, accA, accA1, ga, oA, rngN);
            if (q.n_heads > 1) m_block<SP, 0>(paA, H1, accB, accB1, accA, accA1, ga, oA, rngN);
            other_all<SP, 3, false>(accA, accA1, ga, oB, rngN);
            other_all<SP, 3, false>(accB, accB1, ga, oA, rngN);
            __syncthreads();
            store_head(0, fB, r0, nr);
            if (q.n_heads > 1) store_head(1, fA, r0, nr);
        }
        __syncthreads();
    }
    if constexpr (TRACK) {
        if (G4C_WS_SCALED && !(G4C_WS_ABLATE & 48)) rngN.m *= F16_LO_UNSCALE;
        if (q.range_flag && range_hit(rngN)) {
            if ((threadIdx.x & 63) == 0) q.range_flag[q.range_slot] = 1;
        }
    }
}

struct WsArgs {
    const float *x;
    const int *x_idx;
    int x_ld, x_pact;
    const float *add_ptr[2];
    const int *add_idx[2];
    int add_ld[2];
    const float *w, *b, *gamma, *beta;
    float eps;
    int act;
    float *out;
    const int *out_idx;
    int out_ld, out_bf16;
    const int *tile_rows, *tile_seg, *seg_off;
    float *agg;
    int agg_ld, agg_mean, agg_deg;
    int M, row_base, n_tiles;
    int *range_flag;
    int range_slot;
};
struct WsKernArgs {
    WsArgs a;
    int n_pairs;
    NodeParams q;
};
__device__ __forceinline__ NodeParams node_params_now() {
    typedef const WsKernArgs __attribute__((address_space(4))) *KernArgPtr;
    KernArgPtr k = (KernArgPtr)__builtin_amdgcn_kernarg_segment_ptr();
    asm volatile("" : "+s"(k));
    NodeParams q;
    q.v = k->q.v; q.v_ld = k->q.v_ld; q.w = k->q.w; q.b = k->q.b; q.gamma = k->q.gamma; q.beta = k->q.beta; q.eps = k->q.eps; q.act = k->q.act;
    q.out = k->q.out; q.out_ld = k->q.out_ld; q.n_heads = k->q.n_heads; q.head_ld = k->q.head_ld;
#pragma unroll
    for (int hd = 0; hd < G4C_MAX_HEADS; ++hd) q.head_out[hd] = k->q.head_out[hd];
    q.range_flag = k->q.range_flag; q.range_slot = k->q.range_slot;
    return q;
}
__device__ __forceinline__ int *range_word_now() {
    typedef const WsKernArgs __attribute__((address_space(4))) *KernArgPtr;
    KernArgPtr k = (KernArgPtr)__builtin_amdgcn_kernarg_segment_ptr();
    asm volatile("" : "+s"(k));
    int *const flag = k->a.range_flag;
    return flag ? flag + k->a.range_slot : nullptr;
}

constexpr int G4C_WS_SP1_MINW = 2;
template <bool AGG, bool DIRECT, bool ADDS, int SP, int NL, bool XB16, bool AB16 = false, bool NODE = false, bool DENSE = false, bool TRACK = true>
__global__ __launch_bounds__(512, SP == 1 ? G4C_WS_SP1_MINW : 2) void mlp_ws_kernel(const WsKernArgs ka) {
    const WsArgs &p = ka.a;
    const int n_pairs = ka.n_pairs;
    static_assert((SP == 1 || SP == 2) && (NL == 2 || NL == 3) && (SP == 1 || !XB16) && (SP == 1 || !AB16) && (ADDS || !AB16) &&
                  (!NODE || (AGG && SP == 2)) && (TRACK || SP == 2), "mlp_ws_kernel: unsupported instantiation");
    typedef typename std::conditional<AB16, u32x2, f32x4>::type AddV;
    __shared__ __attribute__((aligned(16))) __bf16 sP[2 * TILE_BF16];
    __shared__ __attribute__((aligned(16))) float sF[2 * FIN];
    __shared__ int sIdx[2][2 * 3 * 32];
    __shared__ int sSeg[4][2 * (SEGCAP + 1)];
    __shared__ __attribute__((aligned(16))) float sBias[3 * NP];
    __shared__ __attribute__((aligned(16))) float sGB[2 * NP];
    __shared__ __attribute__((aligned(16))) float sZero[NP];
    __shared__ __attribute__((aligned(16))) float sCarry[NP];
    __shared__ __attribute__((aligned(16))) float sBiasN[NODE ? 3 * NP : 4];
    __shared__ __attribute__((aligned(16))) float sGBN[NODE ? 2 * NP : 4];

    const int tid = threadIdx.x, lane = tid & 63;
    const int wave = __builtin_amdgcn_readfirstlane(tid >> 6);
    const int n = lane & 15, g = lane >> 4;
    const int fcol = 16 * wave + 4 * g;
    const int prow = tid >> 5, pc = (tid & 31) * 4;

    static_assert((AGG || !DENSE) && !(NODE && DENSE), "dense pairs belong to the fused aggregation of a plain message launch");
    const int KU = DENSE ? p.agg_deg : 0;
    int p_begin, p_end, R0 = 0, R1 = 0;
    {
        const int G = gridDim.x, b = blockIdx.x;
        const int slot = (G & 7) ? b : (b & 7) * (G >> 3) + (b >> 3);
        if constexpr (DENSE) {
            const int n_seg = p.M / KU;
            R0 = __builtin_amdgcn_readfirstlane((int)(((long long)slot * n_seg) / G) * KU);
            R1 = __builtin_amdgcn_readfirstlane((int)(((long long)(slot + 1) * n_seg) / G) * KU);
            p_begin = 0; p_end = (R1 - R0 + 63) >> 6;
        } else {
            p_begin = __builtin_amdgcn_readfirstlane((int)(((long long)slot * n_pairs) / G));
            p_end = __builtin_amdgcn_readfirstlane((int)(((long long)(slot + 1) * n_pairs) / G));
        }
    }
    if (p_begin >= p_end) return;
    WS_STAMP_ONCE(12, __builtin_readcyclecounter());
    WS_STAMP_ONCE(14, (unsigned long long)(p_end - p_begin));

    auto load_meta = [&](int pair) __attribute__((always_inline)) {
        Meta m;
        if constexpr (DENSE) {
            if (pair > p_end - 1) pair = p_end - 1;
            const int r0 = R0 + 64 * pair, nr = (R1 - r0) < 64 ? (R1 - r0) : 64;
            m.r0[0] = r0; m.n[0] = nr < 32 ? nr : 32; m.r0[1] = r0 + 32; m.n[1] = nr - m.n[0];
            m.s0[0] = m.s1[0] = m.s0[1] = m.s1[1] = 0;
            if (m.n[1] == 0) m.r0[1] = m.r0[0];
            return m;
        }
        if (pair > n_pairs - 1) pair = n_pairs - 1;
        const int t0 = 2 * pair;
        if (AGG) {
            const int t1 = t0 + 1 < p.n_tiles ? t0 + 1 : p.n_tiles, t2 = t0 + 2 < p.n_tiles ? t0 + 2 : p.n_tiles;
            const int r0 = p.tile_rows[t0], r1 = p.tile_rows[t1], r2 = p.tile_rows[t2];
            const int q0 = p.tile_seg[t0], q1 = p.tile_seg[t1], q2 = p.tile_seg[t2];
            m.r0[0] = r0; m.n[0] = r1 - r0; m.r0[1] = r1; m.n[1] = r2 - r1;
            m.s0[0] = q0; m.s1[0] = q1; m.s0[1] = q1; m.s1[1] = q2;
        } else {
#pragma unroll
            for (int t = 0; t < 2; ++t) {
                const int tile = t0 + t;
                m.s0[t] = 0; m.s1[t] = 0;
                if (tile >= p.n_tiles) { m.r0[t] = 0; m.n[t] = 0; }
                else { m.r0[t] = p.row_base + tile * 32; const int lim = p.M - m.r0[t]; m.n[t] = lim < 32 ? lim : 32; }
            }
        }
        if (m.n[1] == 0) m.r0[1] = m.r0[0];
        return m;
    };
    auto fix_meta = [&](const Meta &r) __attribute__((always_inline)) {
        Meta m;
#pragma unroll
        for (int t = 0; t < 2; ++t) {
            m.r0[t] = __builtin_amdgcn_readfirstlane(r.r0[t]); m.n[t] = __builtin_amdgcn_readfirstlane(r.n[t]);
            m.s0[t] = __builtin_amdgcn_readfirstlane(r.s0[t]); m.s1[t] = __builtin_amdgcn_readfirstlane(r.s1[t]);
        }
        return m;
    };
    const int *const dummy = reinterpret_cast<const int *>(p.x);
    auto load_tables = [&](const Meta &m) __attribute__((always_inline)) {
        const int *ix0 = DIRECT ? nullptr : p.x_idx, *ix1 = ADDS ? p.add_idx[0] : nullptr, *ix2 = ADDS ? p.add_idx[1] : nullptr;
        const int tt = tid < 192 ? tid : 0;
        const int t = tt / 96, k = (tt % 96) >> 5, r = tt & 31;
        const int nn = m.n[t] > 0 ? m.n[t] : m.n[0];
        const int gr = m.r0[t] + (r < nn ? r : nn - 1);
        const int *ix = (k == 0) ? ix0 : (k == 1 ? ix1 : ix2);
        const int *addr = ix ? ix + gr : dummy;
        int j = 0, ts = 0;
        if (AGG && !DENSE) {
            const int q = tid - 256;
            const bool is_seg = q >= 0 && q < 2 * (SEGCAP + 1);
            ts = is_seg && q >= SEGCAP + 1 ? 1 : 0;
            j = is_seg ? q - ts * (SEGCAP + 1) : 0;
            int sg = m.s0[ts] + j;
            if (sg > m.s1[ts]) sg = m.s1[ts];
            if (is_seg) addr = p.seg_off + sg;
        }
        const int v = *addr;
        return (tid < 192 && !ix) ? gr : v;
    };
    auto store_tables = [&](int v, int it) __attribute__((always_inline)) {
        if (tid < 192) sIdx[it & 1][tid] = v;
        if (AGG && !DENSE && tid >= 256 && tid < 256 + 2 * (SEGCAP + 1)) sSeg[it & 3][tid - 256] = v;
    };
    auto gather_x = [&](const Meta &m, int ring, int t, f32x4 (&xt)[2], unsigned (&raw)[2][2]) __attribute__((always_inline)) {
        {
            const int nn = m.n[t] > 0 ? m.n[t] : m.n[0];
#pragma unroll
            for (int hh = 0; hh < 2; ++hh) {
                const int r = prow + 16 * hh;
                const int gr = DIRECT ? m.r0[t] + (r < nn ? r : nn - 1) : sIdx[ring][t * 96 + r];
                if constexpr (XB16) {
                    typedef unsigned u32x2 __attribute__((ext_vector_type(2)));
                    const u32x2 w = *reinterpret_cast<const u32x2 *>(reinterpret_cast<const __bf16 *>(p.x) + (long long)gr * p.x_ld + pc);
                    raw[hh][0] = w[0]; raw[hh][1] = w[1];
                } else
                xt[hh] = *reinterpret_cast<const f32x4 *>(p.x + (long long)gr * p.x_ld + pc);
            }
        }
    };
    auto widen_x = [&](f32x4 (&xt)[2], const unsigned (&raw)[2][2]) __attribute__((always_inline)) {
        if constexpr (XB16) {
#pragma unroll
            for (int hh = 0; hh < 2; ++hh) {
                xt[hh][0] = __builtin_bit_cast(float, raw[hh][0] << 16); xt[hh][1] = __builtin_bit_cast(float, raw[hh][0] & 0xffff0000u);
                xt[hh][2] = __builtin_bit_cast(float, raw[hh][1] << 16); xt[hh][3] = __builtin_bit_cast(float, raw[hh][1] & 0xffff0000u);
            }
        }
    };
    auto gather_adds = [&](int t, int ring, AddV (&ad)[2][2]) __attribute__((always_inline)) {
        if (ADDS) {
#pragma unroll
            for (int rb = 0; rb < 2; ++rb) {
                const int r = n + 16 * rb;
                if constexpr (AB16) {
                    ad[rb][0] = *reinterpret_cast<const u32x2 *>(reinterpret_cast<const __bf16 *>(p.add_ptr[0]) + (long long)sIdx[ring][t * 96 + 32 + r] * p.add_ld[0] + fcol);
                    ad[rb][1] = *reinterpret_cast<const u32x2 *>(reinterpret_cast<const __bf16 *>(p.add_ptr[1]) + (long long)sIdx[ring][t * 96 + 64 + r] * p.add_ld[1] + fcol);
                } else {
                    ad[rb][0] = *reinterpret_cast<const f32x4 *>(p.add_ptr[0] + (long long)sIdx[ring][t * 96 + 32 + r] * p.add_ld[0] + fcol);
                    ad[rb][1] = *reinterpret_cast<const f32x4 *>(p.add_ptr[1] + (long long)sIdx[ring][t * 96 + 64 + r] * p.add_ld[1] + fcol);
                }
            }
        }
    };

    const __amdgpu_buffer_rsrc_t rs = __builtin_amdgcn_make_buffer_rsrc(const_cast<float *>(p.w), 0, 0x7fffffff, 0x00020000);
    const unsigned lo_b = 2u * (unsigned)((wave >> 1) * 8 * STEP6 + (g >> 1) * STEP6 + ((g & 1) * 32 + 16 * (wave & 1) + n) * 8);
    bf16x8 W[NL][4][SP];
    if (SP == 2) f16_range_mode();
    typename std::conditional<TRACK, RangeV, RangeNone>::type rng;

    Meta m0 = fix_meta(load_meta(p_begin)), m1 = fix_meta(load_meta(p_begin + 1)), m2 = fix_meta(load_meta(p_begin + 2));
    auto meta_at = [&](int pair_, const Meta &carried) __attribute__((always_inline)) {
        if constexpr (DENSE) { asm volatile("" : "+s"(pair_)); return load_meta(pair_); }
        else return carried;
    };
    {
        const int v0 = load_tables(m0), v1 = load_tables(m1);
        store_tables(v0, 0);
        store_tables(v1, 1);
    }
#pragma unroll
    for (int l = 0; l < NL; ++l)
#pragma unroll
        for (int ks = 0; ks < 4; ++ks)
#pragma unroll
            for (int pl = 0; pl < SP; ++pl) W[l][ks][pl] = ldw(rs, lo_b + 1024u * pl, (unsigned)l * 2u * BLOCK6 + (unsigned)ks * 4u * STEP6);
    if (tid < NL * NP) sBias[tid] = p.b[tid];
    if (tid < NP) sZero[tid] = 0.f;
    if (tid < 2 * NP) sGB[tid] = p.gamma ? (tid < NP ? p.gamma[tid] : p.beta[tid - NP]) : 0.f;
    if constexpr (NODE) {
        const NodeParams &q = ka.q;
        if (tid < NL * NP) sBiasN[tid] = q.b[tid];
        if (tid < 2 * NP) sGBN[tid] = q.gamma ? (tid < NP ? q.gamma[tid] : q.beta[tid - NP]) : 0.f;
    }
    __syncthreads();

    const bool pact = p.x_pact != 0;
    __bf16 *const sA = sP, *const sB = sP + TILE_BF16;
    float *const fA = sF, *const fB = sF + FIN;
    Other oA, oB;
    {
        const int l32 = tid & 31;
        const int acc_off = n * PS + 8 * ((2 * wave + (g >> 1)) ^ n) + 4 * (g & 1);
        const int park_off = prow * PS + 8 * ((l32 >> 1) ^ prow) + 4 * (l32 & 1);
        oA.plane_acc = sA + acc_off; oA.plane_park = sA + park_off; oA.fin = fA + n * HS + fcol;
        oB.plane_acc = sB + acc_off; oB.plane_park = sB + park_off; oB.fin = fB + n * HS + fcol;
    }
    const __bf16 *paA[4], *paB[4];
#pragma unroll
    for (int ks = 0; ks < 4; ++ks) { paA[ks] = sA + n * PS + 8 * ((4 * ks + g) ^ n); paB[ks] = paA[ks] + TILE_BF16; }

    f32x4 accA[2], accB[2], accA1[2], accB1[2];
    f32x4 xr[2][2];
    auto bias_init = [&](f32x4 (&acc)[2], f32x4 (&acc1)[2], int l) __attribute__((always_inline)) {
        const f32x4 b4 = *reinterpret_cast<const f32x4 *>(sBias + l * NP + fcol);
        acc[0] = b4; acc[1] = b4;
        acc1[0] = f32x4{0.f, 0.f, 0.f, 0.f}; acc1[1] = f32x4{0.f, 0.f, 0.f, 0.f};
    };
    auto start_values = [&](f32x4 (&acc)[2], f32x4 (&acc1)[2], const AddV (&a)[2][2]) __attribute__((always_inline)) {
        bias_init(acc, acc1, 0);
        if (ADDS) {
#pragma unroll
            for (int rb = 0; rb < 2; ++rb) {
                f32x4 a0, a1;
                if constexpr (AB16) { a0 = widen_bf16x4(a[rb][0]); a1 = widen_bf16x4(a[rb][1]); }
                else { a0 = a[rb][0]; a1 = a[rb][1]; }
#pragma unroll
                for (int e = 0; e < 4; ++e) acc[rb][e] = (acc[rb][e] + a0[e]) + a1[e];
            }
        }
    };
    auto ln_tail = [&](const Meta &mm, const int its) __attribute__((always_inline)) {
        {
            const int row = wave * 4 + g;
            constexpr bool rows16 = SP == 1;
            const int cq[2] = {rows16 ? n * 8 : n * 4, rows16 ? n * 8 + 4 : 64 + n * 4};
            float *const rowp[2] = {fA + row * HS, fB + row * HS};
            float x[2][8];
#pragma unroll
            for (int t = 0; t < 2; ++t)
#pragma unroll
                for (int c = 0; c < 8; c += 4) {
                    const f32x4 v = *reinterpret_cast<const f32x4 *>(rowp[t] + cq[c >> 2]);
                    x[t][c] = v[0]; x[t][c + 1] = v[1]; x[t][c + 2] = v[2]; x[t][c + 3] = v[3];
                }
            WS_STAMP_T(17);
            if (p.gamma) {
                float sum[2], mean[2], var[2], rstd[2];
#pragma unroll
                for (int t = 0; t < 2; ++t) {
                    sum[t] = 0.f;
#pragma unroll
                    for (int c = 0; c < 8; ++c) sum[t] += x[t][c];
                }
                row16_sum2(sum[0], sum[1]);
#pragma unroll
                for (int t = 0; t < 2; ++t) {
                    mean[t] = sum[t] * (1.0f / NP);
                    var[t] = 0.f;
#pragma unroll
                    for (int c = 0; c < 8; ++c) { const float dl = x[t][c] - mean[t]; var[t] += dl * dl; }
                }
                row16_sum2(var[0], var[1]);
#pragma unroll
                for (int t = 0; t < 2; ++t) rstd[t] = rsqrtf(var[t] * (1.0f / NP) + p.eps);
#pragma unroll
                for (int c = 0; c < 8; c += 4) {
                    const f32x4 g4 = *reinterpret_cast<const f32x4 *>(sGB + cq[c >> 2]), b4 = *reinterpret_cast<const f32x4 *>(sGB + NP + cq[c >> 2]);
#pragma unroll
                    for (int t = 0; t < 2; ++t)
#pragma unroll
                        for (int u = 0; u < 4; ++u) x[t][c + u] = fmaf((x[t][c + u] - mean[t]) * rstd[t], g4[u], b4[u]);
                }
            }
            if (p.act == G4C_ACT_SELU) {
#pragma unroll
                for (int t = 0; t < 2; ++t)
#pragma unroll
                    for (int c = 0; c < 8; ++c) x[t][c] = g4c::selu_f(x[t][c]);
            } else if (p.act == G4C_ACT_TANH) {
#pragma unroll
                for (int t = 0; t < 2; ++t)
#pragma unroll
                    for (int c = 0; c < 8; ++c) x[t][c] = g4c::tanh_f(x[t][c]);
            }
            WS_STAMP_T(18);
#pragma unroll
            for (int t = 0; t < 2; ++t) {
                f32x4 v0, v1;
                v0[0] = x[t][0]; v0[1] = x[t][1]; v0[2] = x[t][2]; v0[3] = x[t][3]; v1[0] = x[t][4]; v1[1] = x[t][5]; v1[2] = x[t][6]; v1[3] = x[t][7];
                if (AGG) { *reinterpret_cast<f32x4 *>(rowp[t] + cq[0]) = v0; *reinterpret_cast<f32x4 *>(rowp[t] + cq[1]) = v1; }
                if (G4C_WS_ABLATE & 64) { asm volatile("" :: "v"(v0), "v"(v1)); continue; }
                if (p.out && row < mm.n[t]) {
                    const long long orow = (!AGG && p.out_idx) ? p.out_idx[mm.r0[t] + row] : mm.r0[t] + row;
                    if (SP == 1 && p.out_bf16) {
                        f32x4 w0 = v0, w1 = v1;
                        if (p.out_bf16 == 2) { w0 = selu4(v0); w1 = selu4(v1); }
                        bf16x8 b;
#pragma unroll
                        for (int c = 0; c < 4; ++c) { b[c] = (__bf16)w0[c]; b[4 + c] = (__bf16)w1[c]; }
                        *reinterpret_cast<bf16x8 *>(reinterpret_cast<__bf16 *>(p.out) + orow * p.out_ld + n * 8) = b;
                    } else {
                        float *op = p.out + orow * p.out_ld;
                        *reinterpret_cast<f32x4 *>(op + cq[0]) = v0; *reinterpret_cast<f32x4 *>(op + cq[1]) = v1;
                    }
                }
            }
        }
    };
    auto agg_tail = [&](const Meta &mm, const int itp) __attribute__((always_inline)) {
            const int its = itp; (void)its;
            const int c4 = (tid & 31) * 4;
            const int *sg_tab = sSeg[itp & 3];
            const int nsA = mm.s1[0] - mm.s0[0], nsB = mm.s1[1] - mm.s0[1];
            auto reduce_rows = [&](const float *sH, int b, int e, int sg) __attribute__((always_inline)) {
                f32x4 a = {0.f, 0.f, 0.f, 0.f};
                WS_STAMP_T(20);
                for (int r0 = b; r0 < e; r0 += 8) {
                    f32x4 v[8];
                    if constexpr (SP == 1) {
#pragma unroll
                        for (int u = 0; u < 8; ++u) v[u] = *reinterpret_cast<const f32x4 *>((r0 + u < e ? sH + __umul24((unsigned)(r0 + u), (unsigned)HS) : sZero) + c4);
#pragma unroll
                        for (int u = 0; u < 8; ++u)
#pragma unroll
                            for (int el = 0; el < 4; ++el) a[el] += v[u][el];
                    } else {
#pragma unroll
                        for (int u = 0; u < 8; ++u) v[u] = *reinterpret_cast<const f32x4 *>(sH + (r0 + u < e ? r0 + u : e - 1) * HS + c4);
#pragma unroll
                        for (int u = 0; u < 8; ++u) {
                            const bool on = r0 + u < e;
#pragma unroll
                            for (int el = 0; el < 4; ++el) a[el] += on ? v[u][el] : 0.f;
                        }
                    }
                }
                WS_STAMP_T(21);
                if (p.agg_mean) {
                    if (G4C_WS_MEAN_DIV) {
                        a = g4c::mean_div4(a, (e - b) > 1 ? (e - b) : 1);
                    } else {
                        const float cnt = (float)((e - b) > 1 ? (e - b) : 1);
#pragma unroll
                        for (int el = 0; el < 4; ++el) a[el] /= cnt;
                    }
                }
                WS_STAMP_T(22);
                *reinterpret_cast<f32x4 *>(p.agg + (long long)sg * p.agg_ld + c4) = a;
            };
            auto reduce_uniform = [&](auto KC) __attribute__((always_inline)) {
                constexpr int K = decltype(KC)::value;
                constexpr float cK = (float)K, yK = 1.0f / (float)K;
                const int r0 = mm.r0[0], nr = mm.n[0] + mm.n[1], j0 = (int)((unsigned)r0 / (unsigned)K);
                const int lead = (j0 * K < r0) ? (j0 * K + K - r0) : 0;
                const int nfull = (nr - lead) / K, rest = nr - lead - nfull * K;
                const int jf = j0 + (lead ? 1 : 0);
                auto mean4 = [&](f32x4 a) __attribute__((always_inline)) {
                    if (p.agg_mean) {
#pragma unroll
                        for (int el = 0; el < 4; ++el) {
                            const float q0 = a[el] * yK;
                            a[el] = fmaf(fmaf(-cK, q0, a[el]), yK, q0);
                        }
                    }
                    return a;
                };
                for (int q = tid >> 5; q < nfull; q += 16) {
                    const float *base = fA + __umul24((unsigned)(lead + q * K), (unsigned)HS) + c4;
                    f32x4 v[K];
                    WS_STAMP_T(20);
#pragma unroll
                    for (int u = 0; u < K; ++u) v[u] = *reinterpret_cast<const f32x4 *>(base + u * HS);
                    f32x4 a = {0.f, 0.f, 0.f, 0.f};
#pragma unroll
                    for (int u = 0; u < K; ++u) a += v[u];
                    WS_STAMP_T(21);
                    a = mean4(a);
                    WS_STAMP_T(22);
                    *reinterpret_cast<f32x4 *>(p.agg + (long long)(jf + q) * p.agg_ld + c4) = a;
                }
                if (wave == 7 && (lead | rest)) {
                    const bool hi = lane >= 32;
                    const int b = hi ? nr - rest : 0, cnt = hi ? rest : lead;
                    f32x4 v[K - 1];
#pragma unroll
                    for (int u = 0; u < K - 1; ++u) v[u] = *reinterpret_cast<const f32x4 *>((u < cnt ? fA + __umul24((unsigned)(b + u), (unsigned)HS) : sZero) + c4);
                    f32x4 a = *reinterpret_cast<const f32x4 *>((hi || !lead ? sZero : sCarry) + c4);
#pragma unroll
                    for (int u = 0; u < K - 1; ++u) a += v[u];
                    if (!hi && lead) *reinterpret_cast<f32x4 *>(p.agg + (long long)j0 * p.agg_ld + c4) = mean4(a);
                    if (hi && rest) *reinterpret_cast<f32x4 *>(sCarry + c4) = a;
                }
            };
            if constexpr (DENSE) {
                typedef std::integral_constant<int, 4> K4; typedef std::integral_constant<int, 5> K5; typedef std::integral_constant<int, 6> K6;
                typedef std::integral_constant<int, 7> K7; typedef std::integral_constant<int, 8> K8;
                if (KU == 6) reduce_uniform(K6{});
                else if (KU == 5) reduce_uniform(K5{});
                else if (KU == 4) reduce_uniform(K4{});
                else if (KU == 7) reduce_uniform(K7{});
                else reduce_uniform(K8{});
                return;
            }
            for (int q = tid >> 5; q < nsA + nsB; q += 16) {
                const int t = q >= nsA ? 1 : 0, j = q - (t ? nsA : 0);
                if (j < SEGCAP) {
                    const int b = sg_tab[t * (SEGCAP + 1) + j] - mm.r0[t], e = sg_tab[t * (SEGCAP + 1) + j + 1] - mm.r0[t];
                    reduce_rows(t ? fB : fA, b, e, mm.s0[t] + j);
                }
            }
            if (nsA > SEGCAP || nsB > SEGCAP) {
                for (int q = tid >> 5; q < nsA + nsB; q += 16) {
                    const int t = q >= nsA ? 1 : 0, j = q - (t ? nsA : 0);
                    if (j >= SEGCAP) {
                        const int sg = mm.s0[t] + j;
                        reduce_rows(t ? fB : fA, p.seg_off[sg] - mm.r0[t], p.seg_off[sg + 1] - mm.r0[t], sg);
                    }
                }
            }
    };
    AddV adB[2][2];
    unsigned rawB[2][2] = {{0u, 0u}, {0u, 0u}};
    {
        AddV adA[2][2];
        unsigned rawA[2][2] = {{0u, 0u}, {0u, 0u}};
        gather_x(m0, 0, 0, xr[0], rawA);
        gather_x(m0, 0, 1, xr[1], rawB);
        gather_adds(0, 0, adA);
        gather_adds(1, 0, adB);
        widen_x(xr[0], rawA);
        if (pact) other_all<SP, 2, true>(accA, accA1, xr[0], oA, rng);
        else other_all<SP, 2, false>(accA, accA1, xr[0], oA, rng);
        start_values(accA, accA1, adA);
    }
    __syncthreads();

    for (int it = 0, pair = p_begin; pair < p_end; ++pair, ++it) {
        WS_STAMP(0);
        Meta m3raw;
        if constexpr (!DENSE) m3raw = load_meta(pair + 3);
        const int tv = load_tables(meta_at(pair + 2, m2));
        WS_STAMP(1);
        widen_x(xr[1], rawB);
        if (pact) m_block<SP, 2, true>(paA, W[0], accA, accA1, accA, accA1, xr[1], oB, rng);
        else m_block<SP, 2, false>(paA, W[0], accA, accA1, accA, accA1, xr[1], oB, rng);
        start_values(accB, accB1, adB);
        __syncthreads();
        WS_STAMP(2);
        f32x4 nxa[2];
        AddV nadA[2][2];
        unsigned nraw[2][2] = {{0u, 0u}, {0u, 0u}};
        gather_x(meta_at(pair + 1, m1), (it + 1) & 1, 0, nxa, nraw);
        m_block<SP, 1>(paB, W[0], accB, accB1, accA, accA1, xr[1], oA, rng);
        bias_init(accA, accA1, 1);
        __syncthreads();
        WS_STAMP(3);
        gather_adds(0, (it + 1) & 1, nadA);
        m_block<SP, 1>(paA, W[1], accA, accA1, accB, accB1, xr[1], oB, rng);
        bias_init(accB, accB1, 1);
        __syncthreads();
        WS_STAMP(4);
        if constexpr (NL == 3) {
            m_block<SP, 1>(paB, W[1], accB, accB1, accA, accA1, xr[1], oA, rng);
            bias_init(accA, accA1, 2);
            __syncthreads();
            WS_STAMP(5);
            m_block<SP, 1>(paA, W[2], accA, accA1, accB, accB1, xr[1], oB, rng);
            bias_init(accB, accB1, 2);
            __syncthreads();
            WS_STAMP(6);
        }
        widen_x(nxa, nraw);
        if (pact) m_block<SP, 4, true>(paB, W[NL - 1], accB, accB1, accA, accA1, nxa, oA, rng);
        else m_block<SP, 4, false>(paB, W[NL - 1], accB, accB1, accA, accA1, nxa, oA, rng);
        other_all<SP, 3, false>(accB, accB1, xr[1], oB, rng);
        __syncthreads();
        WS_STAMP(7);
        start_values(accA, accA1, nadA);
        asm volatile("" : "+v"(accA[0]), "+v"(accA[1]) :: "memory");
        Meta m3;
        if constexpr (!DENSE) m3 = fix_meta(m3raw);
        gather_x(meta_at(pair + 1, m1), (it + 1) & 1, 1, xr[1], rawB);
        store_tables(tv, it + 2);
        WS_STAMP(8);

        if (!(G4C_WS_ABLATE & 256)) ln_tail(meta_at(pair, m0), it);
        if constexpr (SP == 1) gather_adds(1, (it + 1) & 1, adB);
        WS_STAMP(9);
        if (AGG) {
            __syncthreads();
            WS_STAMP(15);
            if (!(G4C_WS_ABLATE & 128)) agg_tail(meta_at(pair, m0), it);
        }
        WS_STAMP(16);
        if constexpr (SP != 1) gather_adds(1, (it + 1) & 1, adB);
        WS_STAMP(10);
        if constexpr (!DENSE) { m0 = m1; m1 = m2; m2 = m3; }
    }

    if constexpr (NODE) {
        __builtin_amdgcn_fence(__ATOMIC_RELEASE, "workgroup");
        __syncthreads();
        __builtin_amdgcn_fence(__ATOMIC_ACQUIRE, "workgroup");
        NodeCtx nc;
        nc.tid = tid; nc.wave = wave; nc.n = n; nc.g = g; nc.fcol = fcol; nc.prow = prow; nc.pc = pc; nc.lo_b = lo_b;
        nc.sBiasN = sBiasN; nc.sGBN = sGBN; nc.fA = fA; nc.fB = fB; nc.oA = oA; nc.oB = oB;
#pragma unroll
        for (int ks = 0; ks < 4; ++ks) { nc.paA[ks] = paA[ks]; nc.paB[ks] = paB[ks]; }
        const int t1 = 2 * p_end < p.n_tiles ? 2 * p_end : p.n_tiles;
        const int S0 = __builtin_amdgcn_readfirstlane(p.tile_seg[2 * p_begin]), S1 = __builtin_amdgcn_readfirstlane(p.tile_seg[t1]);
        const NodeParams q = node_params_now();
        node_phase<SP, NL, TRACK>(nc, p.agg, p.agg_ld, q, S0, S1);
    }
    WS_STAMP_ONCE(13, __builtin_readcyclecounter());
    if constexpr (SP == 2 && TRACK) {
        if (G4C_WS_SCALED && !(G4C_WS_ABLATE & 48)) rng.m *= F16_LO_UNSCALE;
        if (range_hit(rng)) {
            int *const word = range_word_now();
            if (word && (threadIdx.x & 63) == 0) *word = 1;
        }
    }
}


#ifdef G4C_WS_ISA_ONLY
template __global__ void mlp_ws_kernel<true, true, true, 2, 3, false, false, false, true, true>(const WsKernArgs);
template __global__ void mlp_ws_kernel<true, true, true, 2, 3, false, false, false, true, false>(const WsKernArgs);
template __global__ void mlp_ws_kernel<true, true, true, 2, 3, false, false, true, false, true>(const WsKernArgs);
template __global__ void mlp_ws_kernel<true, true, true, 2, 3, false, false, true, false, false>(const WsKernArgs);
#endif

}

#ifndef G4C_WS_ISA_ONLY
namespace g4cm {

bool ws_takes(const Launch &L) {
    const Params &p = L.p;
    const bool round1 = L.round1;
    if (!(L.f16x2 || round1) || !message_form(L)) return false;
    if ((round1 && p.n_add != 2) || (p.n_layers != 3 && p.n_layers != 2)) return false;
    if (p.out_bf16 && (!round1 || (p.out_ld & 7) || ((uintptr_t)p.out & 15))) return false;
    if (p.src[0].bf16 && !round1) return false;
    for (int a = 0; a < p.n_add; ++a)
        if (p.add[a].bf16 != p.add[0].bf16 || (p.add[a].bf16 && !round1)) return false;
    return true;
}

int ws_launch(const Launch &L, hipStream_t st, Ran &ran) {
    const Params &p = L.p;
    const bool agg = L.agg, round1 = L.round1, node = L.has_node;
    const bool dense = agg && !node && p.agg_deg >= 4 && p.agg_deg <= 8;
    const int n_pairs = dense ? (int)((p.M + 63) / 64) : (p.n_tiles + 1) / 2;
    ran.kernel = G4C_KERNEL_MLP_WS;
    const int n_wg = g4c::cu_count() * (round1 ? G4C_WS_SP1_MINW / 2 : 1);
    const dim3 grid(n_pairs < n_wg ? n_pairs : n_wg), blk(512);
    const bool direct = p.src[0].idx == nullptr, adds = p.n_add == 2, two = p.n_layers == 2, xb16 = p.src[0].bf16 != 0;
    const bool ab16 = adds && p.add[0].bf16 != 0;
    const bool cert = p.range_certified && !round1 && adds;
    if (cert) ran.kernel = G4C_KERNEL_MLP_WS_CERT;
    WsArgs a{};
    const Src &s = p.src[0];
    a.x = s.bf16 ? reinterpret_cast<const float *>(reinterpret_cast<const __bf16 *>(s.ptr) + s.col0) : s.ptr + s.col0;
    a.x_idx = s.idx; a.x_ld = s.ld; a.x_pact = s.pre_act;
    for (int j = 0; j < 2; ++j) { a.add_ptr[j] = adds ? p.add[j].ptr : nullptr; a.add_idx[j] = adds ? p.add[j].idx : nullptr; a.add_ld[j] = adds ? p.add[j].ld : 0; }
    a.w = p.w; a.b = p.b; a.gamma = p.gamma; a.beta = p.beta; a.eps = p.eps; a.act = p.act;
    a.out = p.out; a.out_idx = p.out_idx; a.out_ld = p.out_ld; a.out_bf16 = p.out_bf16;
    a.tile_rows = p.tile_rows; a.tile_seg = p.tile_seg; a.seg_off = p.seg_off;
    a.agg = p.agg; a.agg_ld = p.agg_ld; a.agg_mean = p.agg_mean; a.agg_deg = p.agg_deg;
    a.M = (int)p.M; a.row_base = (int)p.row_base; a.n_tiles = p.n_tiles;
    a.range_flag = p.range_certified ? nullptr : p.range_flag; a.range_slot = p.range_slot;
    const WsKernArgs ka{a, n_pairs, L.node};
    if (node) {
        G4C_REQUIRE(agg && !round1 && adds, G4C_EUNSUPPORTED, "g4c_mlp_run (upd): needs the hoisted f16x3 message launch with the fused aggregation");
#define G4C_WS_NODE(DIRECT, NL)                                                                                                        \
    do { if (cert) mlp_ws_kernel<true, DIRECT, true, 2, NL, false, false, true, false, false><<<grid, blk, 0, st>>>(ka);    \
         else mlp_ws_kernel<true, DIRECT, true, 2, NL, false, false, true><<<grid, blk, 0, st>>>(ka); } while (0)
        if (direct) { if (two) G4C_WS_NODE(true, 2); else G4C_WS_NODE(true, 3); }
        else { if (two) G4C_WS_NODE(false, 2); else G4C_WS_NODE(false, 3); }
#undef G4C_WS_NODE
        return g4c::check_launch("g4c_mlp_run (ws, upd)");
    }
#define G4C_WS_GO(AGG, DIRECT, ADDS, SP, NL, XB16)                                                                                      \
    do { if (AGG && dense) mlp_ws_kernel<AGG, DIRECT, ADDS, SP, NL, XB16, false, false, AGG><<<grid, blk, 0, st>>>(ka);       \
         else mlp_ws_kernel<AGG, DIRECT, ADDS, SP, NL, XB16><<<grid, blk, 0, st>>>(ka); } while (0)
#define G4C_WS_GOC(AGG, DIRECT, NL)                                           \
    do { if (AGG && dense) mlp_ws_kernel<AGG, DIRECT, true, 2, NL, false, false, false, AGG, false><<<grid, blk, 0, st>>>(ka);       \
         else mlp_ws_kernel<AGG, DIRECT, true, 2, NL, false, false, false, false, false><<<grid, blk, 0, st>>>(ka); } while (0)
#define G4C_WS_GO1(AGG, DIRECT, NL, XB16)                                                                                               \
    do { if (AGG && dense) { if (ab16) mlp_ws_kernel<AGG, DIRECT, true, 1, NL, XB16, true, false, AGG><<<grid, blk, 0, st>>>(ka);       \
                             else mlp_ws_kernel<AGG, DIRECT, true, 1, NL, XB16, false, false, AGG><<<grid, blk, 0, st>>>(ka); }        \
         else if (ab16) mlp_ws_kernel<AGG, DIRECT, true, 1, NL, XB16, true><<<grid, blk, 0, st>>>(ka);                        \
         else mlp_ws_kernel<AGG, DIRECT, true, 1, NL, XB16, false><<<grid, blk, 0, st>>>(ka); } while (0)
#define G4C_WS_SHAPE(AGG, DIRECT)                                                                    \
    do {                                                                                             \
        if (round1) {                                                                                \
            if (two) { if (xb16) G4C_WS_GO1(AGG, DIRECT, 2, true); else G4C_WS_GO1(AGG, DIRECT, 2, false); }      \
            else { if (xb16) G4C_WS_GO1(AGG, DIRECT, 3, true); else G4C_WS_GO1(AGG, DIRECT, 3, false); }          \
        } else if (cert) {                                                                           \
            if (two) G4C_WS_GOC(AGG, DIRECT, 2); else G4C_WS_GOC(AGG, DIRECT, 3);                    \
        } else if (two) {                                                                            \
            if (adds) G4C_WS_GO(AGG, DIRECT, true, 2, 2, false); else G4C_WS_GO(AGG, DIRECT, false, 2, 2, false);                 \
        } else {                                                                                     \
            if (adds) G4C_WS_GO(AGG, DIRECT, true, 2, 3, false); else G4C_WS_GO(AGG, DIRECT, false, 2, 3, false);                 \
        }                                                                                            \
    } while (0)
    if (agg) { if (direct) G4C_WS_SHAPE(true, true); else G4C_WS_SHAPE(true, false); }
    else { if (direct) G4C_WS_SHAPE(false, true); else G4C_WS_SHAPE(false, false); }
#undef G4C_WS_SHAPE
#undef G4C_WS_GO1
#undef G4C_WS_GOC
#undef G4C_WS_GO
    return g4c::check_launch("g4c_mlp_run (ws)");
}

}
#endif
```

### graphs4cfd_amd/nn/blocks.py

```python
from __future__ import annotations

from collections import OrderedDict
from dataclasses import dataclass
from typing import Callable, List, Optional, Sequence, Tuple

import torch
from torch import nn

from .. import _lib, ops, plan
from ..graph import Graph
from ..ops import Source

import os
HOIST_MIN_ROWS = 24576

Tensor = torch.Tensor


def _narrow_flags(sources: Sequence[Source]) -> List[bool]:
    return [s.width <= _lib.NARROW_MAX and s.index is None and s.pre_act == _lib.ACT_NONE and not s.additive for s in sources]


def _split_wide(sources: Sequence[Source]) -> List[Source]:
    if ops.grad_mode() or not any(s.width > 128 and not s.additive and s.segments is None for s in sources):
# ... 347 lines not shown
        if (len(lin) not in (2, 3) or tuple(lin[0].weight.shape) != (128, 384) or any(tuple(l.weight.shape) != (128, 128) for l in lin[1:])
                or getattr(self.MLP, "layer_norm", None) is None or not self.fits_one_launch()):
            return False
        return n_rows >= RS1_MIN_ROWS and n_rows == csr.n and 4 <= csr.uniform_deg <= 8 and csr.tiles() is not None

    def _rs1_takes(self, k_sources, gathered, n_rows, act_code, products, kw) -> bool:
        agg = kw.get("agg")
        if agg is None or act_code != _lib.ACT_NONE or not set(kw) <= {"agg", "store_rows", "rows_dtype", "rows_act"}:
            return False
        if not self.rs1_ready(n_rows, agg[0]) or len(k_sources) != 1 or len(gathered) != 2:
            return False
        x = k_sources[0]
        if (x.width != 128 or x.col0 != 0 or x.negate or x.index is not None or x.segments is not None or x.additive
                or x.pre_act not in (_lib.ACT_NONE, _lib.ACT_SELU)):
            return False
        if x.tensor.dtype == torch.bfloat16 and not (isinstance(x.tensor, ops.RsOrderedRows) and x.pre_act == _lib.ACT_NONE):
            return False
        if any(int(t.size(1)) != 128 for t, _ in gathered):
            return False
        if products is None and any(t.dtype not in (torch.float32, torch.bfloat16) for t, _ in gathered):
            return False
        if products is not None and not (len(products) == 2 and all(isinstance(t, ops.RsOrderedRows) for t in products)):
            return False
        if kw.get("rows_dtype") == torch.bfloat16 and kw.get("store_rows", True) and kw.get("rows_act", _lib.ACT_NONE) != _lib.ACT_SELU:
            return False
        return (agg[1].dtype in (torch.float32, torch.bfloat16) and agg[1].stride(1) == 1 and agg[1].data_ptr() % 16 == 0
                and agg[1].stride(0) % (8 if agg[1].dtype == torch.bfloat16 else 4) == 0)

    def _run_rs1(self, x: Source, gathered, n_rows: int, products, kw) -> Optional[Tensor]:
        adds = []
        for j, (t, idx) in enumerate(gathered):
            if products is not None:
                part = products[j]
            else:
                tagged = isinstance(t, ops.RsOrderedRows)
                pk1 = self._packed_cols(128 * (j + 1), 128 * (j + 2), [128], [False], True, rs_rows=True, rs_in=tagged)
                part = torch.empty((int(t.size(0)), 128), dtype=torch.bfloat16, device=t.device)
                ops.mlp_forward(pk1, [Source(t)], int(t.size(0)), out=part)
                part = ops.RsOrderedRows.tag(part)
            adds.append(Source(part, index=idx, additive=True))
        pk = self._packed_cols(0, 128, [128], [False], False, rs_order=True)
        y = ops.mlp_forward(pk, [x] + adds, n_rows, _lib.ACT_NONE, **kw)
        return ops.RsOrderedRows.tag(y) if (y is not None and y.dtype == torch.bfloat16) else y

    def forward(self, x: Tensor) -> Tensor:
        lead = x.shape[:-1]
        x2 = x.reshape(-1, x.size(-1))
        y = self.run([Source(x2)], int(x2.size(0)))
        return y.reshape(*lead, y.size(-1))


def _blocks(sources: Sequence[Source]):
    return [s.width for s in sources], [s.negate for s in sources], _narrow_flags(sources), _rs_blocks(sources)


def _rs_blocks(sources: Sequence[Source]) -> Tuple[bool, ...]:
    return tuple(isinstance(s.tensor, ops.RsOrderedRows) and s.width == 128 and s.col0 == 0 and s.segments is None
                 for s in sources if not s.additive)


def scatter(src: Tensor, index: Tensor, dim: int = 0, dim_size: Optional[int] = None, reduce: str = "sum") -> Tensor:
    if dim != 0:
        raise NotImplementedError("scatter along dim != 0")
    if reduce not in ("sum", "add", "mean"):
        raise ValueError(f"unsupported reduce {reduce!r}")
    csr = plan.segments_of_sorted(index, dim_size)
    squeeze = src.dim() == 1
    out = ops.segment_reduce(src.reshape(src.size(0), -1), csr, reduce == "mean")
    return out.reshape(-1) if squeeze else out.reshape((csr.n_seg,) + tuple(src.shape[1:]))


def restriction(graph: Graph, coarse_mask: Tensor, edge_attr: Tensor, edge_index: Tensor, num_nodes: int,
                device: torch.device) -> None:
    lut = torch.full((num_nodes,), -1, dtype=torch.long, device=device)
    lut[coarse_mask] = torch.arange(graph.field.size(0), dtype=torch.long, device=device)
    graph.edge_index = lut[edge_index]
    graph.edge_attr = edge_attr


def knn_interpolate(x: Tensor, y_idx: Tensor, x_idx: Tensor, weights: Tensor,
                    *, out: Optional[Tensor] = None, out_idx32: Optional[Tensor] = None) -> Tensor:
    csr = plan.segments_of_sorted(y_idx)
    return ops.weighted_segment_mean(x, plan.index32(x_idx), weights, csr, out, out_idx32)


def pool_edge(idxHR_to_idxLR: Tensor, edge_index: Tensor, edge_attr: Tensor, aggr: str = "mean") -> Tuple[Tensor, Tensor]:
    if aggr not in ("mean", "sum", "add"):
        raise ValueError(f"unsupported aggr {aggr!r}")
    pp = plan.pool_edge_plan(idxHR_to_idxLR, edge_index)
    return pp.edge_index, ops.segment_reduce(edge_attr, pp.csr, aggr == "mean")


def lstsq(A: Tensor, B: Tensor) -> Tensor:
    return torch.linalg.pinv(A) @ B


def _num_nodes_of(edge_index: Tensor) -> int:
    return plan.segments_of_sorted(edge_index[1]).n_seg


def edgeScalarToNodeVector(edge_attr: Tensor, edge_index: Tensor, edgeUnitVector: Optional[Tensor] = None,
                           edgeUnitVectorInverse: Optional[Tensor] = None, coarse_mask: Optional[Tensor] = None) -> Tensor:
    assert (edgeUnitVector is None) != (edgeUnitVectorInverse is None), \
        "Either edgeUnitVector or edgeUnitVectorInverse must be provided."
    if edgeUnitVectorInverse is None:
        n = int(coarse_mask.sum()) if coarse_mask is not None else _num_nodes_of(edge_index)
        edgeUnitVectorInverse = torch.linalg.pinv(edgeUnitVector.reshape(n, -1, 2))
    n, k = int(edgeUnitVectorInverse.size(0)), int(edgeUnitVectorInverse.size(2))
    if edge_attr.size(0) != n * k:
        raise ValueError(f"{edge_attr.size(0)} edges cannot be viewed as {n} nodes x {k} incoming edges")
    return ops.edge_scalar_to_node_vector(edge_attr, edgeUnitVectorInverse, n, k)


COMPACT_MESSAGES = True
HOIST_BF16 = True
PRODUCTS_BF16 = True
ROW_SPLIT_BF16 = __import__('os').environ.get('G4C_ROW_SPLIT_BF16', '1') != '0'
AGGREGATE_BF16 = __import__('os').environ.get('G4C_AGGREGATE_BF16', '1') != '0'
COMPACT_LATENTS = __import__('os').environ.get('G4C_COMPACT_LATENTS', '1') != '0'
UPDATE_ROW_SPLIT = __import__('os').environ.get('G4C_UPDATE_ROW_SPLIT', '1') != '0'
RS1_MIN_ROWS = 20000


FUSE_LAYER = os.environ.get("G4C_FUSE_LAYER", "1") != "0"
FUSE_LAYER_MIN_ROWS = 2048
FUSE_LAYER_MAX_ROWS = 120_000


def will_fuse_layer(msg_mlp: MLP, upd_mlp: MLP, edge_index: Tensor, n_nodes: int) -> bool:
    if not FUSE_LAYER or ops.grad_mode() or ops.mlp_precision() != "f16x3":
        return False
    if not (FUSE_LAYER_MIN_ROWS <= int(edge_index.size(1)) < FUSE_LAYER_MAX_ROWS):
        return False
    lm, lu = msg_mlp._linears(), upd_mlp._linears()
    if len(lm) != len(lu) or len(lm) not in (2, 3) or any(l.out_features != 128 for l in lm + lu):
        return False
    if msg_mlp.input_size != 384 or upd_mlp.input_size != 256:
        return False
    _, csr = plan.edge_csr(edge_index, n_nodes)
    return csr.perm is None and csr.tiles() is not None


def _can_fuse_layer(msg_mlp: MLP, upd_mlp: MLP, v: Tensor, e, edge_index: Tensor, csr, v_src, n_targets, v_out, compact_messages: bool) -> bool:
    if v_src is not None or n_targets is not None or v_out is not None or compact_messages:
        return False
    if not will_fuse_layer(msg_mlp, upd_mlp, edge_index, int(v.size(0))):
        return False
    e_t = e.tensor if isinstance(e, Source) else e
    if isinstance(e, Source) and (e.index is not None or e.col0 != 0 or e.negate or e.segments is not None or e.additive):
        return False
    return int(v.size(1)) == 128 and int(e_t.size(1)) == 128 and e_t.dtype == torch.float32


def _fused_layer(msg_mlp: MLP, upd_mlp: MLP, v: Tensor, e_src: Source, ep, csr, mean: bool, act_code: int, products,
                 next_msg: Optional[MLP], keep_e: bool, rb: ops.RangeBounds):
    H = 128
    dev = v.device
    n_t = int(v.size(0))
    pb = [rb.product(0), rb.product(1)]
    if products is None:
        products = []
        for j in range(2):
            products.append(ops.mlp_forward(msg_mlp._packed_cols(H * (1 + j), H * (2 + j), [H], [False], True), [Source(v, bound=rb.v)], n_t))
            pb[j] = ops.take_bounds().out
    pk_msg = msg_mlp._packed_cols(0, H, [H], [e_src.negate], False)
    srcs = [e_src, Source(products[0], index=ep.row, additive=True, bound=pb[0]), Source(products[1], index=ep.col, additive=True, bound=pb[1])]
    heads = None
    if next_msg is not None and next_msg.input_size == 3 * H and next_msg._linears()[0].out_features == H:
        spec = upd_mlp._heads_spec(([H, H], [False, False]), next_msg, next_msg.input_size - 2 * H, [H, H])
        if spec is not None:
            pk_upd = upd_mlp._image(spec)
            heads = [torch.empty((n_t, H), dtype=torch.float32, device=dev) for _ in range(2)]
    if heads is None:
        pk_upd = upd_mlp.packed([H, H], [False, False])
    e_new, v_new, _ = ops.mp_layer_forward(pk_msg, srcs, ep.n_edges, csr, mean, pk_upd, v, act_code, store_rows=keep_e, head_outs=heads,
                                           v_bound=rb.v)
    lb = ops.take_bounds()
    rb.v, rb.e, rb.products = lb.out, lb.e, (lb.heads if heads is not None else None)
    return v_new, e_new, heads


def _mp_step(msg_mlp: MLP, upd_mlp: MLP, v: Tensor, e: Tensor, index: Tensor, aggr: str, act_code: int,
             e_pre_act: int = _lib.ACT_NONE, v_src: Optional[Tensor] = None,
             products: Optional[Sequence[Tensor]] = None, next_msg: Optional[MLP] = None, keep_e: bool = True,
             n_targets: Optional[int] = None, v_out: Optional[Tensor] = None, compact_messages: bool = False,
             next_graph: Optional[Tuple[int, "plan.CsrPlan"]] = None, compact_v: bool = False,
             bounds: Optional[ops.RangeBounds] = None):
    if aggr not in ("mean", "sum", "add"):
        raise ValueError(f"unsupported aggr {aggr!r}")
    n_t = int(v.size(0)) if n_targets is None else int(n_targets)
    if n_targets is not None and next_msg is not None:
        raise NotImplementedError("next_msg with n_targets")
    ep, csr = plan.edge_csr(index, n_t)
    senders = v if v_src is None else v_src
    mean = aggr == "mean"
    rb = bounds if bounds is not None else ops.RangeBounds()
    e_src = e if isinstance(e, Source) else Source(e, pre_act=e_pre_act, bound=rb.e)
    if next_graph is None and _can_fuse_layer(msg_mlp, upd_mlp, v, e, index, csr, v_src, n_targets, v_out, compact_messages):
        v_new, e_new, nxt = _fused_layer(msg_mlp, upd_mlp, v, e_src, ep, csr, mean, act_code, products, next_msg, keep_e, rb)
        return (v_new, e_new, nxt) if next_msg is not None else (v_new, e_new)
    hoist_kw = dict(gathered_bounds=[rb.v if v_src is None else None, rb.v], product_bounds=rb.products)
    v_in = Source(v, bound=rb.v)
    if ops.can_fuse_aggregation(csr, msg_mlp.output_size):
        kw = dict(store_rows=keep_e, rows_dtype=torch.bfloat16 if compact_messages and COMPACT_MESSAGES else None,
                  rows_act=_lib.ACT_SELU if compact_messages and COMPACT_MESSAGES else _lib.ACT_NONE)
        gathered = [(senders, ep.row), (v, ep.col)]
        agg = None
        if (AGGREGATE_BF16 and ops.mlp_precision() == "bf16" and msg_mlp.output_size == 128 and int(v.size(1)) == 128
                and upd_mlp.fits_one_launch() and ops.effective_precision([128, 128]) == "bf16"):
            agg16 = torch.empty((csr.n_seg, 128), dtype=torch.bfloat16, device=v.device)
            if msg_mlp._rs1_takes([e_src], gathered, ep.n_edges, _lib.ACT_NONE, products, dict(kw, agg=(csr, agg16, mean))):
                agg = agg16
        if agg is None:
            agg = torch.empty((csr.n_seg, msg_mlp.output_size), dtype=torch.float32, device=v.device)
        e_new = msg_mlp.run_hoisted([e_src], gathered, ep.n_edges, products=products, agg=(csr, agg, mean), **hoist_kw, **kw)
        rb.e = ops.take_bounds().out
        agg_src = Source(ops.RsOrderedRows.tag(agg) if agg.dtype == torch.bfloat16 else agg, bound=ops.agg_bound(rb.e, csr, mean))
    elif ops.can_aggregate_on_load(csr, msg_mlp.output_size, [msg_mlp.output_size, int(v.size(1))]):
        e_new = msg_mlp.run_hoisted([e_src], [(senders, ep.row), (v, ep.col)], ep.n_edges, products=products, **hoist_kw)
        rb.e = ops.take_bounds().out
        agg_src = Source(e_new, segments=csr, seg_mean=mean, bound=rb.e)
    elif ops.grad_mode():
        e_new = msg_mlp.run_hoisted([e_src], [(senders, ep.row), (v, ep.col)], ep.n_edges)
        rb.e = None
        agg_src = Source(ops.segment_reduce(e_new, csr, mean))
    else:
        agg = torch.empty((csr.n_seg, msg_mlp.output_size), dtype=torch.float32, device=v.device)
        e_new = msg_mlp.run_hoisted([e_src], [(senders, ep.row), (v, ep.col)], ep.n_edges,
                                    products=products, agg=(csr, agg, mean), **hoist_kw)
        rb.e = ops.take_bounds().out
        agg_src = Source(agg, bound=ops.agg_bound(rb.e, csr, mean))
    v16 = (compact_v and compact_latents_now(upd_mlp.output_size) and upd_mlp.fits_one_launch() and n_targets is None and v_out is None
           and ops.effective_precision([128, int(v.size(1))]) == "bf16")
    if next_msg is not None:
        nxt = None
        nx_rows, nx_csr = (ep.n_edges, csr) if next_graph is None else next_graph
        if nx_rows >= HOIST_MIN_ROWS:
            w = upd_mlp.output_size
            nxt = upd_mlp.run_with_heads([agg_src, v_in], int(v.size(0)), act_code, next_msg,
                                         next_msg.input_size - 2 * w, [w, w], rs_rows=next_msg.rs1_ready(nx_rows, nx_csr),
                                         out=torch.empty((int(v.size(0)), 128), dtype=torch.bfloat16, device=v.device) if v16 else None)
        if nxt is None:
            out16 = torch.empty((int(v.size(0)), 128), dtype=torch.bfloat16, device=v.device) if v16 else None
            v_new = upd_mlp.run_coded([agg_src, v_in], int(v.size(0)), act_code, out=out16)
            rb.v, rb.products = ops.take_bounds().out, None
            return v_new, e_new, None
        lb = ops.take_bounds()
        rb.v, rb.products = lb.out, lb.heads
        return nxt[0], e_new, nxt[1]
    v_new = upd_mlp.run_coded([agg_src, v_in], n_t, act_code,
                              out=torch.empty((n_t, 128), dtype=torch.bfloat16, device=v.device) if v16 else v_out)
    rb.v, rb.products = ops.take_bounds().out, None
    return v_new, e_new


def compact_latents_now(width: int = 128) -> bool:
    return bool(COMPACT_LATENTS and PRODUCTS_BF16 and HOIST_BF16 and ops.mlp_precision() == "bf16" and width == 128 and not ops.grad_mode()
                and ops.effective_precision([128, 128]) == "bf16")


def pending_act(e: Optional[Tensor]) -> int:
    return _lib.ACT_NONE if (e is not None and torch.is_tensor(e) and e.dtype == torch.bfloat16) else _lib.ACT_SELU


def _public_mp(msg_mlp: MLP, upd_mlp: MLP, v, e, index, aggr, activation, v_src=None):
    code = _lib.act_code(activation)
    v_new, e_new = _mp_step(msg_mlp, upd_mlp, v, e, index, aggr, _lib.ACT_NONE if code is None else code, v_src=v_src)
    if activation is not None:
        if code is None:
            v_new, e_new = activation(v_new), activation(e_new)
        elif ops.grad_mode():
            e_new = torch.nn.functional.selu(e_new) if code == _lib.ACT_SELU else (torch.tanh(e_new) if code == _lib.ACT_TANH else e_new)
        else:
            ops.activation_(e_new, code)
    return v_new, e_new


class GNBlock(nn.Module):

    def __init__(self, edge_mlp_args: Tuple, node_mlp_args: Tuple, aggr: str = 'mean'):
        super().__init__()
        self.edge_mlp = MLP(*edge_mlp_args)
        self.node_mlp = MLP(*node_mlp_args)
        self.aggr = aggr

    def reset_parameters(self):
        for m in (self.node_mlp, self.edge_mlp):
            if m is not None and hasattr(m, 'reset_parameters'):
                m.reset_parameters()

    def step(self, v: Tensor, e: Tensor, edge_index: Tensor, act_code: int, e_pre_act: int = _lib.ACT_NONE,
             products: Optional[Sequence[Tensor]] = None, next_msg: Optional[MLP] = None, keep_e: bool = True,
             bounds: Optional[ops.RangeBounds] = None):
        return _mp_step(self.edge_mlp, self.node_mlp, v, e, edge_index, self.aggr, act_code, e_pre_act,
                        products=products, next_msg=next_msg, keep_e=keep_e, bounds=bounds)

    def forward(self, v: Tensor, e: Tensor, edge_index: Tensor, *, activation=None) -> Tuple[Tensor, Tensor]:
        return _public_mp(self.edge_mlp, self.node_mlp, v, e, edge_index, self.aggr, activation)


MP = GNBlock


class DownMP(nn.Module):

    def __init__(self, down_mlp_args: Tuple, hr_graph_idx: int):
        super().__init__()
        self.down_mlp = MLP(*down_mlp_args)
        self.hr_graph_idx = hr_graph_idx
        self.lr_graph_idx = hr_graph_idx + 1
        self.reset_parameters()

    def reset_parameters(self):
        for item in [self.down_mlp]:
            if hasattr(item, 'reset_parameters'):
                item.reset_parameters()

    def pool(self, graph: Graph, field: Tensor, edge_index: Tensor, edge_attr: Tensor, activation=None,
             e_pre_act: int = _lib.ACT_NONE, target_major: bool = False, bounds: Optional[ops.RangeBounds] = None):
        rb = bounds if bounds is not None else ops.RangeBounds()
        h, l = self.hr_graph_idx, self.lr_graph_idx
        rel = getattr(graph, f'e_{h}{l}')
        csr = plan.cluster_plan(getattr(graph, f'cluster_{l}'), getattr(graph, f'mask_{l}'))
        m = self.down_mlp.run([Source(rel), Source(field, bound=rb.v)], int(field.size(0)))
        m_bound = ops.take_bounds().out
        code = _lib.act_code(activation)
        pooled = ops.segment_reduce(m, csr, True, _lib.ACT_NONE if code is None else code)
        pooled = _finish(pooled, activation, code)
        pp = plan.pool_edge_plan(getattr(graph, f'idx{h}_to_idx{l}'), edge_index, target_major)
        ea_l = ops.segment_reduce(edge_attr, pp.csr, True, src_act=e_pre_act)
        rb.v = ops.act_bound(m_bound, code) if (activation is None or code is not None) else None
        rb.e, rb.products = ops.act_bound(rb.e, e_pre_act), None
        return pooled, pp.edge_index, ea_l

    def forward(self, graph: Graph, activation: Optional[Callable] = None) -> Graph:
        field, ei, ea = self.pool(graph, graph.field, graph.edge_index, graph.edge_attr, activation)
        graph.pos = getattr(graph, f'pos_{self.lr_graph_idx}')
        graph.field, graph.edge_index, graph.edge_attr = field, ei, ea
        return graph


class UpMP(nn.Module):

    def __init__(self, up_mlp_args: Tuple, lr_graph_idx: int):
        super().__init__()
        self.up_mlp = MLP(*up_mlp_args)
        self.lr_graph_idx = lr_graph_idx
        self.hr_graph_idx = lr_graph_idx - 1
        self.reset_parameters()

    def reset_parameters(self):
        for item in [self.up_mlp]:
            if hasattr(item, 'reset_parameters'):
                item.reset_parameters()

    def sources(self, graph: Graph, field_lr: Tensor, field_hr_old: Tensor,
                bounds: Tuple[Optional[float], Optional[float]] = (None, None)) -> List[Source]:
        h, l = self.hr_graph_idx, self.lr_graph_idx
        parent = plan.index32(getattr(graph, f'idx{h}_to_idx{l}'))
        return [Source(getattr(graph, f'e_{h}{l}'), negate=True), Source(field_lr, parent, bound=bounds[0]),
                Source(field_hr_old, bound=bounds[1])]

    def unpool(self, graph: Graph, field_lr: Tensor, field_hr_old: Tensor, activation=None) -> Tensor:
        return self.up_mlp.run(self.sources(graph, field_lr, field_hr_old), int(field_hr_old.size(0)), activation=activation)

    def forward(self, graph: Graph, field_hr_old: Tensor, pos_hr: Tensor, activation: Optional[Callable] = None) -> Graph:
        graph.field = self.unpool(graph, graph.field, field_hr_old, activation)
        graph.pos = pos_hr
        return graph


class EdgeMP(nn.Module):

    def __init__(self, angle_mlp_args: Tuple, edge_mlp_args: Tuple, aggr: str = "mean"):
        super().__init__()
        self.angle_mlp = MLP(*angle_mlp_args)
        self.edge_mlp = MLP(*edge_mlp_args)
        self.aggr = aggr
        self.reset_parameters()

    def reset_parameters(self):
        for item in [self.edge_mlp, self.angle_mlp]:
            if hasattr(item, 'reset_parameters'):
                item.reset_parameters()

    def step(self, e: Tensor, a: Tensor, angle_index: Tensor, act_code: int, a_pre_act: int = _lib.ACT_NONE,
             products: Optional[Sequence[Tensor]] = None, next_msg: Optional[MLP] = None, keep_e: bool = True, compact_e: bool = False):
        return _mp_step(self.angle_mlp, self.edge_mlp, e, a, angle_index, self.aggr, act_code, a_pre_act,
                        products=products, next_msg=next_msg, keep_e=keep_e, compact_messages=True, compact_v=compact_e)

    def forward(self, e: Tensor, a: Tensor, angle_index: Tensor, *, activation=None) -> Tuple[Tensor, Tensor]:
        return _public_mp(self.angle_mlp, self.edge_mlp, e, a, angle_index, self.aggr, activation)


class DownEdgeMP(nn.Module):

    def __init__(self, angle_mlp_args: Tuple, edge_mlp_args: Tuple):
        super().__init__()
        self.angle_mlp = MLP(*angle_mlp_args)
        self.edge_mlp = MLP(*edge_mlp_args)
        self.reset_parameters()

    def reset_parameters(self):
        for item in [self.edge_mlp, self.angle_mlp]:
            if hasattr(item, 'reset_parameters'):
                item.reset_parameters()

    def forward(self, e1: Tensor, e2: Tensor, a12: Tensor, angle_index12: Tensor, *, activation=None) -> Tensor:
        return self.step(e1, e2, a12, angle_index12, activation)[0]

    def step(self, e1: Tensor, e2: Tensor, a12: Tensor, angle_index12: Tensor, activation=None, next_msg: Optional[MLP] = None,
             next_graph=None) -> Tuple[Tensor, Optional[Sequence[Tensor]]]:
        code = _lib.act_code(activation)
        if next_msg is None or code is None:
            e2_new, _ = _mp_step(self.angle_mlp, self.edge_mlp, e2, a12, angle_index12, "mean",
                                 _lib.ACT_NONE if code is None else code, v_src=e1, keep_e=False)
            return _finish(e2_new, activation, code), None
        e2_new, _, prods = _mp_step(self.angle_mlp, self.edge_mlp, e2, a12, angle_index12, "mean", code, v_src=e1, keep_e=False,
                                    next_msg=next_msg, next_graph=next_graph, compact_v=True)
        return e2_new, prods


class UpEdgeMP(nn.Module):

    def __init__(self, up_mlp_args: Tuple):
        super().__init__()
        self.up_mlp = MLP(*up_mlp_args)
        self.reset_parameters()

    def reset_parameters(self):
        for item in [self.up_mlp]:
            if hasattr(item, 'reset_parameters'):
                item.reset_parameters()

    def forward(self, pos: Tensor, y_idx_21: Tensor, x_idx_21: Tensor, weights_21: Tensor, edge_attr2: Tensor,
                edge_index2: Tensor, edgeUnitVectorInverse2: Tensor, coarse_mask2: Tensor, edge_attr1: Tensor,
                edge_index1: Tensor, edgeUnitVector1: Tensor, coarse_mask1=None, *, activation=None) -> Tensor:
        return self.step(pos, y_idx_21, x_idx_21, weights_21, edge_attr2, edge_index2, edgeUnitVectorInverse2, coarse_mask2, edge_attr1,
                         edge_index1, edgeUnitVector1, coarse_mask1, activation=activation)[0]

    def step(self, pos: Tensor, y_idx_21: Tensor, x_idx_21: Tensor, weights_21: Tensor, edge_attr2: Tensor,
             edge_index2: Tensor, edgeUnitVectorInverse2: Tensor, coarse_mask2: Tensor, edge_attr1: Tensor,
             edge_index1: Tensor, edgeUnitVector1: Tensor, coarse_mask1=None, *, activation=None, next_msg: Optional[MLP] = None,
             next_graph=None) -> Tuple[Tensor, Optional[Sequence[Tensor]]]:
        n_total, nfeat = int(pos.size(0)), int(edge_attr2.size(1))
        v2 = edgeScalarToNodeVector(edge_attr2, edge_index2, edgeUnitVectorInverse=edgeUnitVectorInverse2,
                                    coarse_mask=coarse_mask2)
        if ops.grad_mode() and v2.requires_grad:
# ... 21 lines not shown
```

### graphs4cfd_amd/nn/mus_gnn.py

```python
from __future__ import annotations

from typing import Optional

import torch

from .. import _lib, ops
from ..graph import Graph
from ..ops import Source
from . import blocks as _blocks
from .blocks import MLP, MP, DownMP, UpMP
from .model import GNN

SELU, TANH, NONE = _lib.ACT_SELU, _lib.ACT_TANH, _lib.ACT_NONE


class _MuSGNN(GNN):
    _PROGRAM: tuple = ()
    _PRETRAINED: dict = {}

    def __init__(self, model: str = None, *args, **kwargs) -> None:
        if model is not None:
            super().__init__(arch=None, weights=None, checkpoint=self._pretrained(self._PRETRAINED, model), *args, **kwargs)
        else:
            super().__init__(*args, **kwargs)

    def load_arch(self, arch: dict):
        self.arch = arch
        self.edge_encoder = MLP(*arch["edge_encoder"])
        self.node_encoder = MLP(*arch["node_encoder"])
        for name in self._PROGRAM:
            if name.startswith("down_mp"):
                setattr(self, name, DownMP(arch[name], int(name[-2])))
            elif name.startswith("up_mp"):
                setattr(self, name, UpMP(arch[name], int(name[-2])))
            else:
                setattr(self, name, MP(*arch[name]))
        self.node_decoder = MLP(*arch["decoder"])
        self.to(self.device)

    def _launch_for(self, mlp: MLP, sources, n_rows: int, act_code: int, k: int, edge_index: torch.Tensor):
        nxt = self._PROGRAM[k] if k < len(self._PROGRAM) else ""
        n_edges = int(edge_index.size(1))
        if nxt.startswith("mp") and (n_edges >= _blocks.HOIST_MIN_ROWS
                                     or _blocks.will_fuse_layer(getattr(self, nxt).edge_mlp, getattr(self, nxt).node_mlp, edge_index, n_rows)):
            cons = getattr(self, nxt).edge_mlp
            w = mlp.output_size
            res = mlp.run_with_heads(sources, n_rows, act_code, cons, cons.input_size - 2 * w, [w, w])
            if res is not None:
                return res
        return mlp.run_coded(sources, n_rows, act_code), None

    def forward(self, graph: Graph, t: Optional[int] = None) -> torch.Tensor:
        field0 = graph.field
        n = int(field0.size(0))
        inputs = [Source(getattr(graph, k)) for k in ('field', 'loc', 'glob', 'omega') if hasattr(graph, k)]
        edge_index = graph.edge_index
        e = ops.static_launch("edge_encoder", [graph.edge_attr],
                              lambda: self.edge_encoder.run_coded([Source(graph.edge_attr)], int(graph.edge_attr.size(0)), SELU))
        rb = ops.RangeBounds(e=ops.take_bounds().out)
        v, products = self._launch_for(self.node_encoder, inputs, n, SELU, 0, edge_index)
        lb = ops.take_bounds()
        rb.v, rb.products = lb.out, (lb.heads if products is not None else None)
        e_pending = NONE
        stash = []
        prog = self._PROGRAM
        for k, name in enumerate(prog):
            block = getattr(self, name)
            if name.startswith("down_mp"):
                stash.append((v, edge_index, e, e_pending, rb.v, rb.e))
                v, edge_index, e = block.pool(graph, v, edge_index, e, torch.tanh, e_pre_act=e_pending, target_major=True, bounds=rb)
                e_pending, products = NONE, None
            elif name.startswith("up_mp"):
                v_old, edge_index, e, e_pending, v_old_bound, rb.e = stash.pop()
                v, products = self._launch_for(block.up_mlp, block.sources(graph, v, v_old, (rb.v, v_old_bound)), int(v_old.size(0)), TANH,
                                               k + 1, edge_index)
                lb = ops.take_bounds()
                rb.v, rb.products = lb.out, (lb.heads if products is not None else None)
            else:
                nxt = prog[k + 1] if k + 1 < len(prog) else ""
                if nxt.startswith("mp"):
                    v, e, products = block.step(v, e, edge_index, SELU, e_pre_act=e_pending, products=products,
                                                next_msg=getattr(self, nxt).edge_mlp, bounds=rb)
                else:
                    drop_e = nxt.startswith("up_mp") or nxt == ""
                    v, e = block.step(v, e, edge_index, SELU, e_pre_act=e_pending, products=products, keep_e=not drop_e, bounds=rb)
                    products = None
                e_pending = SELU
        nf = self.num_fields
        return self.node_decoder.run_coded([Source(v)], n, NONE, resid=field0, resid_col0=int(field0.size(1)) - nf)


def _model(name: str, program: str, pretrained: dict, doc: str):
    cls = type(name, (_MuSGNN,), {"_PROGRAM": tuple(program.split()), "_PRETRAINED": pretrained, "__doc__": doc})
    cls.__module__ = __name__
    return cls


_DOC = """The {n}-GNN for {what} inference from Lino et al. (2022) (https://doi.org/10.1063/5.0097679)
(reference: nn/mus_gnn.py:{lines}).  `arch` keys: edge_encoder, node_encoder, {keys}, decoder — each MP entry
`((in, widths, layer_norm), (in, widths, layer_norm))`, each down/up entry `(in, widths, layer_norm)`."""

NsOneScaleGNN = _model(
    "NsOneScaleGNN", "mp11 mp12 mp13 mp14 mp15 mp16 mp17 mp18",
    {"1S-GNN-NsCircle-v1": "weights/NsMuSGNN/NsOneScaleGNN.chk"},
    _DOC.format(n="1S", what="incompressible flow", lines="11-97", keys="mp11..mp18"))

NsTwoScaleGNN = _model(
    "NsTwoScaleGNN", "mp111 mp112 mp113 mp114 down_mp12 mp21 mp22 mp23 mp24 up_mp21 mp121 mp122 mp123 mp124",
    {"2S-GNN-NsCircle-v1": "weights/NsMuSGNN/NsTwoScaleGNN.chk"},
    _DOC.format(n="2S", what="incompressible flow", lines="100-218", keys="mp111..mp114, down_mp12, mp21..mp24, up_mp21, mp121..mp124"))

NsThreeScaleGNN = _model(
    "NsThreeScaleGNN",
    "mp111 mp112 mp113 mp114 down_mp12 mp211 mp212 down_mp23 mp31 mp32 mp33 mp34 up_mp32 mp221 mp222 up_mp21 "
    "mp121 mp122 mp123 mp124",
    {"3S-GNN-NsCircle-v1": "weights/NsMuSGNN/NsThreeScaleGNN.chk"},
    _DOC.format(n="3S", what="incompressible flow", lines="221-373", keys="mp111.., down_mp12, mp211, mp212, down_mp23, mp31..mp34, up_mp32, mp221, mp222, up_mp21, mp121..mp124"))

NsFourScaleGNN = _model(
    "NsFourScaleGNN",
    "mp111 mp112 mp113 mp114 down_mp12 mp211 mp212 down_mp23 mp311 mp312 down_mp34 mp41 mp42 mp43 mp44 up_mp43 "
    "mp321 mp322 up_mp32 mp221 mp222 up_mp21 mp121 mp122 mp123 mp124",
    {"4S-GNN-NsCircle-v1": "weights/NsMuSGNN/NsFourScaleGNN.chk"},
    _DOC.format(n="4S", what="incompressible flow", lines="376-562", keys="mp111.., down_mp12, mp211.., down_mp23, mp311.., down_mp34, mp41..mp44, up_mp43, mp321.., up_mp32, mp221.., up_mp21, mp121.."))

AdvOneScaleGNN = _model(
    "AdvOneScaleGNN", "mp111 mp112 mp121 mp122",
    {"1S-GNN-UniformAdv-v1": "weights/AdvMuSGNN/AdvOneScaleGNN.chk"},
    _DOC.format(n="1S", what="advection", lines="566-636", keys="mp111, mp112, mp121, mp122"))

AdvTwoScaleGNN = _model(
    "AdvTwoScaleGNN", "mp111 mp112 down_mp12 mp21 mp22 mp23 mp24 up_mp21 mp121 mp122",
    {"2S-GNN-UniformAdv-v1": "weights/AdvMuSGNN/AdvTwoScaleGNN.chk"},
    _DOC.format(n="2S", what="advection", lines="639-741", keys="mp111, mp112, down_mp12, mp21..mp24, up_mp21, mp121, mp122"))

AdvThreeScaleGNN = _model(
    "AdvThreeScaleGNN",
    "mp111 mp112 down_mp12 mp211 mp212 down_mp23 mp31 mp32 mp33 mp34 up_mp32 mp221 mp222 up_mp21 mp121 mp122",
    {"3S-GNN-UniformAdv-v1": "weights/AdvMuSGNN/AdvThreeScaleGNN.chk"},
    _DOC.format(n="3S", what="advection", lines="744-880", keys="mp111, mp112, down_mp12, mp211, mp212, down_mp23, mp31..mp34, up_mp32, mp221, mp222, up_mp21, mp121, mp122"))

AdvFourScaleGNN = _model(
    "AdvFourScaleGNN",
    "mp111 mp112 down_mp12 mp211 mp212 down_mp23 mp311 mp312 down_mp34 mp41 mp42 mp43 mp44 up_mp43 mp321 mp322 "
    "up_mp32 mp221 mp222 up_mp21 mp121 mp122",
    {"4S-GNN-UniformAdv-v1": "weights/AdvMuSGNN/AdvFourScaleGNN.chk"},
    _DOC.format(n="4S", what="advection", lines="883-1053", keys="mp111, mp112, down_mp12, ..., up_mp21, mp121, mp122"))

__all__ = ["NsOneScaleGNN", "NsTwoScaleGNN", "NsThreeScaleGNN", "NsFourScaleGNN",
           "AdvOneScaleGNN", "AdvTwoScaleGNN", "AdvThreeScaleGNN", "AdvFourScaleGNN"]
```

### graphs4cfd_amd/ops.py

```python
from __future__ import annotations

import ctypes as C
import os
from typing import List, Optional, Sequence, Tuple

import torch

from . import _lib
from .plan import CsrPlan

Tensor = torch.Tensor


class KernelTimer:
    active = None

    def __init__(self):
        self.records = []

    def __enter__(self):
        KernelTimer.active = self
        return self

    def __exit__(self, *exc):
        KernelTimer.active = None
        return False

    def launch(self, kind: str, flops: float, nbytes: float, fn):
        a, b = torch.cuda.Event(enable_timing=True), torch.cuda.Event(enable_timing=True)
        a.record()
        out = fn()
        b.record()
        if kind.startswith("mlp_"):
            kind = _lib.KERNEL_NAMES.get(int(_lib.load().g4c_mlp_last_kernel()), kind)
        self.records.append((kind, flops, nbytes, a, b))
        return out

    def summary(self):
        out = {}
        for kind, flops, nbytes, a, b in self.records:
            d = out.setdefault(kind, {"launches": 0, "seconds": 0.0, "flops": 0.0, "bytes": 0.0})
            d["launches"] += 1
            d["seconds"] += a.elapsed_time(b) * 1e-3
            d["flops"] += flops
            d["bytes"] += nbytes
        return out


def _timed(kind: str, flops: float, nbytes: float, fn):
    kt = KernelTimer.active
    return fn() if kt is None else kt.launch(kind, flops, nbytes, fn)


class StaticCache:
    active: Optional["StaticCache"] = None

    def __init__(self):
        self.store = {}
        self.hits = self.misses = 0
        self._prev = None

    def __enter__(self):
        self._prev, StaticCache.active = StaticCache.active, self
        return self

    def __exit__(self, *exc):
        StaticCache.active = self._prev
        return False

    def get(self, name: str, inputs: Sequence[Tensor], fn):
        key = (weights_epoch(), mlp_precision()) + tuple((t.data_ptr(), t._version, tuple(t.shape), t.dtype) for t in inputs)
        hit = self.store.get(name)
        global _last_bounds
        if hit is not None and hit[0] == key:
            self.hits += 1
            _last_bounds = hit[3]
            return hit[1]
        self.misses += 1
        val = fn()
        self.store[name] = (key, val, tuple(inputs), _last_bounds)
        return val

    def stale(self) -> bool:
        head = (weights_epoch(), mlp_precision())
        for key, _, inputs, _ in self.store.values():
            if key != head + tuple((t.data_ptr(), t._version, tuple(t.shape), t.dtype) for t in inputs):
                return True
        return False


def static_launch(name: str, inputs: Sequence[Tensor], fn):
    c = StaticCache.active
    return fn() if (c is None or torch.is_grad_enabled()) else c.get(name, inputs, fn)


def _f32_2d(t: Tensor, name: str) -> Tensor:
    if t.dtype != torch.float32:
        raise TypeError(f"{name}: expected float32, got {t.dtype}")
    if t.dim() != 2:
        raise ValueError(f"{name}: expected a 2-D tensor, got shape {tuple(t.shape)}")
    if t.stride(1) != 1 and t.size(1) > 1:
        t = t.contiguous()
    if t.size(0) > 1 and t.stride(0) < t.size(1):
        t = t.contiguous()
    return t


def _bf16_2d(t: Tensor) -> Tensor:
    if t.dim() != 2 or t.stride(1) != 1:
        raise ValueError(f"bf16 source: expected a 2-D tensor with unit column stride, got shape {tuple(t.shape)}")
    return t


def _ld(t: Tensor) -> int:
    return int(t.stride(0)) if t.size(0) > 1 else int(max(t.size(1), t.stride(0)))


class Source:

    __slots__ = ("tensor", "index", "col0", "width", "negate", "pre_act", "additive", "segments", "seg_mean", "bound")

    def __init__(self, tensor: Tensor, index: Optional[Tensor] = None, col0: int = 0, width: Optional[int] = None,
                 negate: bool = False, pre_act: int = _lib.ACT_NONE, additive: bool = False,
                 segments: Optional[CsrPlan] = None, seg_mean: bool = True, bound: Optional[float] = None):
        self.tensor = _bf16_2d(tensor) if tensor.dtype == torch.bfloat16 else _f32_2d(tensor, "source")
        self.index = index
        self.col0 = col0
        self.width = int(self.tensor.size(1) - col0 if width is None else width)
        self.negate = negate
        self.pre_act = pre_act
        self.additive = additive
        self.segments = segments
        self.seg_mean = seg_mean
        self.bound = bound
        if segments is not None and (index is not None or additive or self.width != 128):
            raise ValueError("aggregation on load needs a 128-wide block without gather index")


def _rows_f32(t: Tensor, name: str, cols: Optional[int] = None, min_rows: int = 0, min_cols: int = 0) -> Tensor:
    if not torch.is_tensor(t):
        raise TypeError(f"{name}: expected a tensor, got {type(t).__name__}")
    if t.dtype != torch.float32:
        raise TypeError(f"{name}: expected float32, got {t.dtype}")
    if t.dim() != 2:
        raise ValueError(f"{name}: expected a 2-D tensor, got shape {tuple(t.shape)}")
    if t.size(1) > 1 and t.stride(1) != 1:
        raise ValueError(f"{name}: expected unit column stride, got strides {tuple(t.stride())}")
    if t.size(0) > 1 and t.stride(0) < t.size(1):
        raise ValueError(f"{name}: rows overlap (row stride {t.stride(0)} < {t.size(1)} columns)")
    if cols is not None and int(t.size(1)) != cols:
        raise ValueError(f"{name}: expected {cols} columns, got shape {tuple(t.shape)}")
    if int(t.size(1)) < min_cols:
        raise ValueError(f"{name}: expected at least {min_cols} columns, got shape {tuple(t.shape)}")
    if int(t.size(0)) < min_rows:
        raise ValueError(f"{name}: expected at least {min_rows} rows, got shape {tuple(t.shape)}")
    return t


def _index_i32(t: Optional[Tensor], name: str, n: Optional[int] = None, at_least: Optional[int] = None) -> Optional[Tensor]:
    if t is None:
        return None
    if not torch.is_tensor(t):
        raise TypeError(f"{name}: expected a tensor, got {type(t).__name__}")
    if t.dtype != torch.int32:
        raise TypeError(f"{name}: expected int32, got {t.dtype}")
    if t.dim() != 1 or (t.numel() > 1 and t.stride(0) != 1):
        raise ValueError(f"{name}: expected a contiguous 1-D tensor, got shape {tuple(t.shape)} strides {tuple(t.stride())}")
    if n is not None and t.numel() != n:
        raise ValueError(f"{name}: expected {n} entries, got {t.numel()}")
    if at_least is not None and t.numel() < at_least:
        raise ValueError(f"{name}: expected at least {at_least} entries, got {t.numel()}")
    return t


def _vector_f32(t: Optional[Tensor], name: str, n: int) -> Optional[Tensor]:
    if t is None:
        return None
    if not torch.is_tensor(t):
        raise TypeError(f"{name}: expected a tensor, got {type(t).__name__}")
    if t.dtype != torch.float32:
        raise TypeError(f"{name}: expected float32, got {t.dtype}")
    if t.dim() != 1 or t.numel() != n or (n > 1 and t.stride(0) != 1):
        raise ValueError(f"{name}: expected a contiguous vector of {n} entries, got shape {tuple(t.shape)} strides {tuple(t.stride())}")
    return t


def _act_arg(act, name: str) -> int:
    if act not in (_lib.ACT_NONE, _lib.ACT_SELU, _lib.ACT_TANH):
        raise ValueError(f"{name}: unknown activation code {act!r}")
    return int(act)


def _csr_arg(csr: CsrPlan, name: str) -> None:
    if csr.n < 0 or csr.n_seg < 0:
        raise ValueError(f"{name}: negative sizes n={csr.n} n_seg={csr.n_seg}")
    _index_i32(csr.off, f"{name}.off", n=csr.n_seg + 1)
    _index_i32(csr.perm, f"{name}.perm", at_least=csr.n)


def segment_reduce(src: Tensor, csr: CsrPlan, mean: bool, act: int = _lib.ACT_NONE, out: Optional[Tensor] = None,
                   src_act: int = _lib.ACT_NONE) -> Tensor:
    if torch.is_grad_enabled() and src.requires_grad:
        if out is not None:
            raise NotImplementedError("segment_reduce(out=...) is not differentiable")
        from . import autograd as _ag
        return _ag.segment_reduce(src, csr, mean, act, src_act)
    src = _f32_2d(src, "src")
    width = int(src.size(1))
    _csr_arg(csr, "csr")
    act, src_act = _act_arg(act, "act"), _act_arg(src_act, "src_act")
    if csr.perm is None and int(src.size(0)) < csr.n:
        raise ValueError(f"src: the plan reads rows 0 .. {csr.n - 1}, got shape {tuple(src.shape)}")
    if csr.perm is not None and csr.n > 0 and int(src.size(0)) == 0:
        raise ValueError(f"src: the plan reads {csr.n} rows through its permutation, got shape {tuple(src.shape)}")
    if out is not None:
        _rows_f32(out, "out", cols=width, min_rows=csr.n_seg)
# ... 647 lines not shown
            _lib.check(lib.g4c_mlp_pack_layer(_lib.ptr(Wc), n_out, k_in, seg_arr, neg_arr, len(segs), self.desc.w_format, wptr, k_pad, NP, stream))
        if bf16 and any(s > NP for s in seg_widths):
            raise NotImplementedError("bf16 MLP with an input block wider than 128")
        wide = [j for j in range(len(seg_widths)) if not narrow[j]]
        k_pad0 = NP * len(wide) if bf16 else sum((s + KC - 1) // KC * KC for s in seg_widths)
        k_pads = [k_pad0] + [NP] * (n_layers - 1)
        if len(heads) > _lib.MAX_HEADS or any(tuple(h.shape) != (NP, NP) for h in heads):
            raise NotImplementedError(f"heads must be at most {_lib.MAX_HEADS} weights of shape [128, 128]")
        if heads and int(weights[-1].size(0)) != NP:
            raise NotImplementedError("heads need a 128-wide MLP output")
        stream_buf = torch.zeros((sum(k_pads) + NP * len(heads) + (NP if bf16 else KC)) * NP * planes,
                                 dtype=torch.bfloat16 if bf16 else torch.float32, device=dev)
        esz = 2 * planes if bf16 else 4
        bias_buf = torch.zeros(n_layers * NP, dtype=torch.float32, device=dev)
        self._keep += [stream_buf, bias_buf]
        off = 0
        for l, (W, b) in enumerate(zip(weights, biases)):
            n_out, k_in = int(W.size(0)), int(W.size(1))
            if n_out > NP:
                raise NotImplementedError(f"layer width {n_out} > 128 is outside the fused-MLP kernel envelope")
            if l == 0:
                segs, negs = list(seg_widths), [1 if x else 0 for x in seg_negate]
                self.narrow_w = {}
                if any(narrow):
                    col0s = [sum(seg_widths[:j]) for j in range(len(seg_widths))]
                    W32 = W.detach().to(torch.float32)
                    for j in range(len(seg_widths)):
                        if narrow[j]:
                            rows = torch.zeros((seg_widths[j], NP), dtype=torch.float32, device=dev)
                            rows[:, :n_out] = W32[:, col0s[j]:col0s[j] + seg_widths[j]].T * (-1.0 if seg_negate[j] else 1.0)
                            self.narrow_w[j] = rows.contiguous()
                            self._keep.append(self.narrow_w[j])
                    if wide:
                        W = torch.cat([W32[:, col0s[j]:col0s[j] + seg_widths[j]] for j in wide], dim=1)
                        segs, negs = [seg_widths[j] for j in wide], [1 if seg_negate[j] else 0 for j in wide]
                        k_in = int(W.size(1))
                    else:
                        W = None
            else:
                prev = int(weights[l - 1].size(0))
                if k_in != prev:
                    raise ValueError(f"layer {l + 1} expects {k_in} inputs, previous layer gives {prev}")
                segs, negs = [k_in], [0]
            wptr = stream_buf.data_ptr() + esz * off
            if W is not None:
                pack(W, l, n_out, k_in, segs, negs, wptr, k_pads[l])
            if b is not None:
                bias_buf[l * NP: l * NP + n_out].copy_(b.detach())
            self.desc.k_pad[l], self.desc.n_pad[l] = k_pads[l], NP
            self.desc.w[l], self.desc.b[l] = wptr, bias_buf.data_ptr() + 4 * l * NP
            off += k_pads[l] * NP
        self.n_heads = len(heads)
        for W in heads:
            pack(W, None, NP, NP, [NP], [0], stream_buf.data_ptr() + esz * off, NP)
            off += NP * NP
        self.n_out = int(weights[-1].size(0))
        self.desc.n_out = self.n_out
        self.flops_per_row = float(sum(2 * int(W.size(0)) * int(W.size(1)) for W in list(weights) + list(heads)))
        if ln is not None:
            g, be, eps = ln
            g, be = g.detach().to(torch.float32).contiguous(), be.detach().to(torch.float32).contiguous()
            self.desc.ln_gamma, self.desc.ln_beta, self.desc.ln_eps = g.data_ptr(), be.data_ptr(), float(eps)
            self._keep += [g, be]
        else:
            self.desc.ln_gamma, self.desc.ln_beta, self.desc.ln_eps = None, None, 0.0
        self.seg_widths = tuple(seg_widths)
        self.device = dev
        self.norms = weight_norms(weights, biases, ln, heads, seg_widths, narrow) if self.split == "f16x2" else None
        self.params = (list(weights), list(biases), ln)
        self.heads_params = bool(heads)


def _src_array(sources: Sequence[Source]):
    arr = (_lib.g4c_src_t * len(sources))()
    for a, s in zip(arr, sources):
        a.ptr, a.idx, a.width, a.ld, a.col0, a.pre_act = (s.tensor.data_ptr(), _lib.ptr(s.index), s.width, _ld(s.tensor),
                                                          s.col0, s.pre_act)
        a.additive = 1 if s.additive else 0
        a.dtype = 1 if s.tensor.dtype == torch.bfloat16 else 0
        if s.segments is not None:
            a.seg_off, a.seg_mean, a.seg_perm = _lib.ptr(s.segments.off), 1 if s.seg_mean else 0, _lib.ptr(s.segments.perm)
    return arr


def agg_bound(bound: Optional[float], csr: CsrPlan, mean: bool) -> Optional[float]:
    return bound if (bound is None or mean) else bound * max(csr.max_deg, 1)


def _certify(packed: "PackedMLP", sources: Sequence[Source], act: int, residual: bool, tracked: bool) -> LaunchBounds:
    seg_len = max((s_.segments.max_deg for s_ in sources if s_.segments is not None), default=None)
    lb = range_bounds(packed.norms, sources, act, residual, seg_len)
    packed.desc.range_certified = 1 if (RANGE_PROOFS and not tracked and certifies(lb.converted)) else 0
    return lb


def _agg_mode(agg_mean: bool, csr: CsrPlan) -> int:
    return (1 if agg_mean else 0) | (csr.uniform_deg << 8)


def _set_agg(io, csr: CsrPlan, agg_out: Tensor, agg_mean: bool) -> None:
    t_rows, t_seg, nt = csr.tiles()
    io.tile_rows, io.tile_seg, io.seg_off, io.n_tiles = _lib.ptr(t_rows), _lib.ptr(t_seg), _lib.ptr(csr.off), nt
    io.agg, io.agg_ld, io.agg_mode = _lib.ptr(agg_out), _ld(agg_out), _agg_mode(agg_mean, csr)


def _set_heads(io, head_outs: Sequence[Tensor]) -> None:
    io.n_heads, io.head_ld = len(head_outs), _ld(head_outs[0])
    io.head_dtype = 1 if head_outs[0].dtype == torch.bfloat16 else 0
    for j, h in enumerate(head_outs):
        io.head_out[j] = h.data_ptr()


def _run(packed: PackedMLP, arr, n_src: int, n_rows: int, io, dev, flops: float, nbytes: float) -> None:
    if packed.split == "f16x2":
        io.range_flag = _launch_flags(dev).data_ptr()
    kind = "mlp_split_kernel<4>" if packed.precision == "fp32" else "mlp_bx6_kernel"
    _timed(kind, flops, nbytes, lambda: _lib.check(_lib.load().g4c_mlp_run(C.byref(packed.desc), arr, n_src, n_rows, C.byref(io),
                                                                           _lib.stream_handle(dev))))


def mp_layer_forward(msg: PackedMLP, sources: Sequence[Source], n_rows: int, csr: CsrPlan, agg_mean: bool, upd: PackedMLP,
                     v: Tensor, act: int, store_rows: bool = True, head_outs: Optional[Sequence[Tensor]] = None,
                     v_out: Optional[Tensor] = None, v_bound: Optional[float] = None) -> Tuple[Optional[Tensor], Tensor, Optional[Sequence[Tensor]]]:
    global _last_bounds
    _last_bounds = None
    dev = _lib.require_hip(*[s.tensor for s in sources], *[s.index for s in sources], v, v_out)
    if msg.split != "f16x2" or upd.split != "f16x2":
        raise NotImplementedError("mp_layer_forward needs both MLPs packed for the f16x3 arithmetic")
    if csr.tiles() is None or n_rows != csr.n:
        raise ValueError("mp_layer_forward: the rows must be in segment order with segments of at most 32 rows")
    v = _f32_2d(v, "v")
    n_t = csr.n_seg
    e_out = torch.empty((n_rows, 128), dtype=torch.float32, device=dev) if store_rows else None
    agg = torch.empty((n_t, 128), dtype=torch.float32, device=dev)
    if v_out is None:
        v_out = torch.empty((n_t, 128), dtype=torch.float32, device=dev)
    n_heads = 0 if head_outs is None else len(head_outs)
    if n_heads and (n_heads != upd.n_heads):
        raise ValueError(f"{n_heads} head outputs for a packing with {upd.n_heads} heads")
    io = _lib.g4c_mlp_io_t(row_count=n_rows, out=_lib.ptr(e_out), out_ld=128 if e_out is None else _ld(e_out), upd=C.pointer(upd.desc),
                           v=_lib.ptr(v), v_ld=_ld(v), v_act=act, v_out=_lib.ptr(v_out), v_out_ld=_ld(v_out))
    _set_agg(io, csr, agg, agg_mean)
    if n_heads:
        _set_heads(io, head_outs)
    in_b = 4.0 * 128 * (n_rows * (2 if store_rows else 1) + n_t * (2 + n_heads))
    lb_msg = _certify(msg, sources, _lib.ACT_NONE, False, False)
    lb_upd = _certify(upd, [Source(agg, bound=agg_bound(lb_msg.out, csr, agg_mean)), Source(v, bound=v_bound)], act, False, False)
    try:
        _run(msg, _src_array(sources), len(sources), n_rows, io, dev, msg.flops_per_row * n_rows + upd.flops_per_row * n_t, in_b)
    finally:
        msg.desc.range_certified = upd.desc.range_certified = 0
    _last_bounds = LaunchBounds(None, lb_upd.out, lb_upd.heads, e=lb_msg.out)
    return e_out, v_out, head_outs


def _rows_dtype(what: str, tensors: Sequence[Tensor]) -> int:
    kinds = {t.dtype for t in tensors}
    if not kinds <= {torch.float32, torch.bfloat16} or len(kinds) > 1:
        raise TypeError(f"{what} tensors must share one dtype, float32 or bfloat16 (got {sorted(str(k) for k in kinds)})")
    return _lib.DTYPE_BF16 if kinds == {torch.bfloat16} else _lib.DTYPE_F32


def mlp_forward(packed: PackedMLP, sources: Sequence[Source], n_rows: int, act: int = _lib.ACT_NONE,
                out: Optional[Tensor] = None, out_idx32: Optional[Tensor] = None,
                resid: Optional[Tensor] = None, resid_col0: int = 0, rows: Optional[Tuple[int, int]] = None,
                head_outs: Optional[Sequence[Tensor]] = None, agg: Optional[Tuple[CsrPlan, Tensor, bool]] = None,
                save: Optional[Sequence[Optional[Tensor]]] = None, mul: Optional[Sequence[Optional[Tensor]]] = None,
                store_rows: bool = True, rows_dtype: Optional[torch.dtype] = None, rows_act: int = _lib.ACT_NONE) -> Optional[Tensor]:
    global _last_bounds
    _last_bounds = None
    if torch.is_grad_enabled():
        from . import autograd as _ag
        if _ag.wants_grad(packed, sources, resid):
            if out is not None or out_idx32 is not None or head_outs is not None or agg is not None or rows is not None or save is not None:
                raise NotImplementedError("out= / heads / fused aggregation are inference-only forms of mlp_forward; "
                                          "call under torch.no_grad() or use the plain form")
            return _ag.mlp(packed, sources, n_rows, act, resid, resid_col0)
    if packed.rs2:
        ok = [isinstance(s.tensor, RsOrderedRows) for s in sources]
        if len(sources) != 2 or not ok[0] or ok[1] != (packed.rs2 == 4) or any(s.tensor.dtype != torch.bfloat16 for s in sources):
            raise ValueError("weights packed for the row-split update kernel: [aggregate | e] as bf16 rows, the aggregate (and, format 4, e) RsOrderedRows")
    elif packed.rs_order and packed.precision == "bf16":
        if any(s.tensor.dtype == torch.bfloat16 and not isinstance(s.tensor, RsOrderedRows) for s in sources):
            raise ValueError("weights packed for the row-split kernel: bf16 rows must be RsOrderedRows (its column order)")
    elif any(isinstance(s.tensor, RsOrderedRows) for s in sources) or any(packed.rs_blocks):
        fixed, j = [], 0
        for s in sources:
            tagged = isinstance(s.tensor, RsOrderedRows)
            ok = (not s.additive) and j < len(packed.rs_blocks) and packed.rs_blocks[j] and s.col0 == 0 and s.width == 128
            if not s.additive:
                if j < len(packed.rs_blocks) and packed.rs_blocks[j] and not tagged:
                    raise ValueError(f"input block {j}: the weights expect rows in the row-split order (ops.RsOrderedRows)")
                j += 1
            fixed.append(s if (not tagged or ok) else
                         Source(rs_rows_to_natural(s.tensor), s.index, s.col0, s.width, s.negate, s.pre_act, s.additive, s.segments, s.seg_mean))
        sources = fixed
    dev = _lib.require_hip(*[s.tensor for s in sources], *[s.index for s in sources], out, out_idx32, resid)
    if dev != packed.device:
        raise RuntimeError(f"MLP weights on {packed.device}, inputs on {dev}")
    if tuple(s.width for s in sources if not s.additive) != packed.seg_widths:
        raise ValueError(f"input blocks {[s.width for s in sources if not s.additive]} do not match packed layout {packed.seg_widths}")
    arr = _src_array(sources)
    if any(packed.narrow):
        j = 0
        for a, src in zip(arr, sources):
            if src.additive:
                continue
            if packed.narrow[j]:
                if src.index is not None or src.pre_act != _lib.ACT_NONE:
                    raise ValueError("a narrow input block cannot be gathered through an index or activated on load")
                a.additive, a.w = 2, packed.narrow_w[j].data_ptr()
            j += 1
    fusable = (agg is not None and FUSE_AGG and packed.precision in ("bf16x6", "bf16") and packed.n_out == 128 and head_outs is None
               and rows is None and out_idx32 is None and resid is None and n_rows == agg[0].n and agg[0].tiles() is not None)
    if not store_rows and not fusable:
        raise ValueError("store_rows=False needs an aggregation the launch can fuse (ops.can_fuse_aggregation)")
    reduce_after = None
    if agg is not None and not fusable:
        reduce_after, agg = agg, None
    rows16 = bool(fusable and store_rows and rows_dtype == torch.bfloat16 and packed.precision == "bf16" and out is None)
    if out is None and store_rows:
        out = torch.empty((n_rows, packed.n_out), dtype=torch.bfloat16 if rows16 else torch.float32, device=dev)
    if out is not None and out.dtype not in (torch.float32, torch.bfloat16):
        raise TypeError(f"out: expected float32 or bfloat16, got {out.dtype}")
    row_begin, row_count = rows if rows is not None else (0, n_rows)
    io = _lib.g4c_mlp_io_t(act=act, row_begin=row_begin, row_count=row_count, out=_lib.ptr(out),
                           out_ld=_ld(out) if out is not None else 128, out_idx=_lib.ptr(out_idx32), resid=_lib.ptr(resid),
                           resid_ld=_ld(resid) if resid is not None else 0, resid_col0=resid_col0)
    if out is not None and out.dtype == torch.bfloat16:
        if agg is None and (packed.precision != "bf16" or out_idx32 is not None or resid is not None):
            raise TypeError("a bf16 `out` needs the rounded-bf16 mode and no output index / residual")
        if rows16 and rows_act not in (_lib.ACT_NONE, _lib.ACT_SELU):
            raise ValueError("rows_act: only ACT_SELU")
        io.out_dtype = 2 if (rows16 and rows_act == _lib.ACT_SELU) else 1
    in_bytes = float(sum(s.width * (2 if s.tensor.dtype == torch.bfloat16 else 4) for s in sources if not s.additive))
    nbytes = (in_bytes + 4.0 * packed.n_out) * row_count
    if head_outs is not None:
        if len(head_outs) != packed.n_heads or packed.n_heads == 0:
            raise ValueError(f"{len(head_outs)} head outputs for a packing with {packed.n_heads} heads")
        if out_idx32 is not None or resid is not None:
            raise NotImplementedError("heads with an output index / residual")
        _lib.require_hip(*head_outs)
        if any(h.dtype == torch.bfloat16 for h in head_outs):
            if packed.precision != "bf16" or any(h.dtype != torch.bfloat16 for h in head_outs):
                raise TypeError("bf16 head outputs need the rounded-bf16 mode, and every head in bf16")
        elif out.dtype != torch.float32:
            raise TypeError("heads stored as fp32 need fp32 output rows (bf16 rows: bf16 heads)")
        _set_heads(io, head_outs)
        if packed.precision == "fp32":
            nbytes = 4.0 * (sum(packed.seg_widths) + packed.n_out * (1 + packed.n_heads)) * n_rows
    if agg is not None:
        csr, agg_out, agg_mean = agg
        _lib.require_hip(agg_out)
        if agg_out.dtype not in (torch.float32, torch.bfloat16):
            raise TypeError(f"aggregate: expected float32 (or bfloat16 on the row-split kernel), got {agg_out.dtype}")
        _set_agg(io, csr, agg_out, agg_mean)
        if agg_out.dtype == torch.bfloat16:
            io.agg_mode |= 1 << 16
        out_b = 0 if not store_rows else packed.n_out * (2 if out.dtype == torch.bfloat16 else 4)
        nbytes = (in_bytes + out_b) * n_rows + 4.0 * packed.n_out * csr.n_seg
    if save is not None:
        live = [t for t in save if t is not None]
        _lib.require_hip(*live)
        if any(t.dim() != 2 or t.size(0) < n_rows or t.size(1) < 128 or t.stride(1) != 1 or _ld(t) != _ld(live[0]) for t in live):
            raise ValueError("save tensors must be [n_rows, >= 128] fp32 (or bf16) with one common leading dimension")
        if len(save) > _lib.MAX_LAYERS:
            raise ValueError(f"{len(save)} save tensors for {packed.desc.n_layers} layers")
        io.n_save, io.save_ld = len(save), _ld(live[0]) if live else 128
        io.save[:len(save)] = [_lib.ptr(t) for t in save]
        io.save_dtype = _rows_dtype("save", live)
        if mul is not None:
            lm = [t for t in mul if t is not None]
            _lib.require_hip(*lm)
            if len(mul) != len(save) or any(t.size(0) < n_rows or t.size(1) < 128 or t.stride(1) != 1 or _ld(t) != _ld(lm[0]) for t in lm):
                raise ValueError("mul tensors must be [n_rows, >= 128] fp32 (or bf16) with one common leading dimension, one entry per layer")
            io.mul[:len(mul)] = [_lib.ptr(t) for t in mul]
            io.mul_ld = _ld(lm[0]) if lm else 128
            io.mul_dtype = _rows_dtype("mul", lm)
        nbytes = (4.0 * (sum(packed.seg_widths) + packed.n_out) + 128.0 * sum(t.element_size() for t in live)) * n_rows
    lb = _certify(packed, sources, act, resid is not None or out_idx32 is not None or rows is not None, save is not None)
    try:
        _run(packed, arr, len(sources), n_rows, io, dev, packed.flops_per_row * row_count, nbytes)
    finally:
        packed.desc.range_certified = 0
    _last_bounds = lb
    if reduce_after is not None:
        segment_reduce(out, reduce_after[0], reduce_after[2], out=reduce_after[1])
    return out
```

### include/g4c.h

```cpp
#ifndef G4C_H
#define G4C_H

#include <stdint.h>

#ifdef __cplusplus
extern "C" {
#endif

#define G4C_OK 0
#define G4C_EINVAL (-1)
#define G4C_ELAUNCH (-2)
#define G4C_EUNSUPPORTED (-3)

#define G4C_ACT_NONE 0
#define G4C_ACT_SELU 1
#define G4C_ACT_TANH 2

#define G4C_MAX_SRC 4
#define G4C_MAX_LAYERS 4
#define G4C_MAX_HEADS 2
#define G4C_NARROW_MAX 8

int g4c_version(void);
int g4c_device_info(const void *device_ptr, int32_t *device , int32_t *cu_count );
const char *g4c_last_error(void);


int g4c_plan_csr(const int64_t *keys , int64_t n, int64_t n_seg,
                 int32_t *perm , int32_t *off );

int64_t g4c_plan_pool_edge(const int64_t *idx_hr_to_lr , int64_t n_hr,
                           const int64_t *edge_index , int64_t n_edges,
                           int64_t *coarse_edge_index ,
                           int32_t *perm ,
                           int32_t *off ,
                           int64_t *n_kept );
int64_t g4c_plan_pool_edge_ordered(const int64_t *idx_hr_to_lr, int64_t n_hr, const int64_t *edge_index, int64_t n_edges,
                                   int32_t target_major, int64_t *coarse_edge_index, int32_t *perm, int32_t *off,
                                   int64_t *n_kept);

int g4c_segment_reduce(const float *src, int32_t src_ld, const int32_t *perm, const int32_t *off,
                       int32_t n_seg, int32_t width, int32_t mean, int32_t src_act, int32_t act,
                       float *out, int32_t out_ld, void *stream);

int g4c_weighted_segment_mean(const float *x, int32_t x_ld, const int32_t *x_idx, const float *w,
                              const int32_t *off, int32_t n_seg, int32_t width,
                              float *out, int32_t out_ld, const int32_t *out_idx, void *stream);

#define G4C_DTYPE_F32 0
#define G4C_DTYPE_BF16 1
#define G4C_DTYPE_BF16_SELU 2

typedef struct {
    const float *ptr;
    const int32_t *idx;
    int32_t width;
    int32_t ld;
    int32_t col0;
    int32_t pre_act;
    int32_t additive;
    int32_t seg_mean;
    const float *w;
    const int32_t *seg_off;
    const int32_t *seg_perm;
    int32_t dtype;
} g4c_src_t;

typedef struct {
    int32_t n_layers;
    int32_t k_pad[G4C_MAX_LAYERS];
    int32_t n_pad[G4C_MAX_LAYERS];
    const float *w[G4C_MAX_LAYERS];
    const float *b[G4C_MAX_LAYERS];
    const float *ln_gamma;
    const float *ln_beta;
    float ln_eps;
    int32_t n_out;
    int32_t w_format;
    int32_t range_slot;
    int32_t range_certified;
} g4c_mlp_t;

#define G4C_WFMT_FP32 0
#define G4C_WFMT_F16X2 1
#define G4C_WFMT_BF16X3 2
#define G4C_WFMT_BF16_RS 3
#define G4C_WFMT_BF16_RS2 4
#define G4C_WFMT_BF16_RS2N 5
#define G4C_WFMT_BF16 6

int g4c_mlp_pack_layer(const float *W, int32_t n_out, int32_t k_in, const int32_t *seg_width ,
                       const int32_t *seg_negate , int32_t n_seg, int32_t w_format, void *packed,
                       int32_t k_pad, int32_t n_pad, void *stream);

#define G4C_AGG_UNIFORM(k) ((int32_t)(k) << 8)
#define G4C_AGG_OUT_BF16 ((int32_t)1 << 16)

typedef struct {
    int32_t size;
    int32_t act;
    int64_t row_begin;
    int64_t row_count;
    void *out;
    int32_t out_ld;
    int32_t out_dtype;
    const int32_t *out_idx;
    const float *resid;
    int32_t resid_ld, resid_col0;
    int32_t n_heads;
    int32_t head_ld;
    int32_t head_dtype;
    void *head_out[G4C_MAX_HEADS];
    const int32_t *tile_rows, *tile_seg, *seg_off;
    int32_t n_tiles;
    void *agg;
    int32_t agg_ld;
    int32_t agg_mode;
    int32_t n_save;
    void *save[G4C_MAX_LAYERS];
    int32_t save_ld;
    const void *mul[G4C_MAX_LAYERS];
    int32_t mul_ld;
    const g4c_mlp_t *upd;
    const float *v;
    int32_t v_ld, v_act;
    float *v_out;
    int32_t v_out_ld;
    int32_t *range_flag;
    int32_t save_dtype;
    int32_t mul_dtype;
} g4c_mlp_io_t;

int g4c_mlp_run(const g4c_mlp_t *mlp , const g4c_src_t *srcs , int32_t n_src, int64_t n_rows,
                const g4c_mlp_io_t *io , void *stream);

int g4c_mlp_bx6i_enable(int on);

int g4c_mlp_ws_enable(int on);

int g4c_mlp_small_launch_tiles(int n_tiles);

#define G4C_KERNEL_NONE 0
#define G4C_KERNEL_MLP_SPLIT 1
#define G4C_KERNEL_MLP_BX6 2
#define G4C_KERNEL_MLP_BX6I 3
#define G4C_KERNEL_MLP_WS 4
#define G4C_KERNEL_MLP_RS 5
#define G4C_KERNEL_MLP_RS2 6
#define G4C_KERNEL_MLP_BX6_CERT 7
#define G4C_KERNEL_MLP_WS_CERT 8
int g4c_mlp_last_kernel(void);

#define G4C_TILE_SHAPE_GENERIC 0
#define G4C_TILE_SHAPE_NODE 1
#define G4C_TILE_SHAPE_UP 2
#define G4C_TILE_SHAPE_DOWN 3
int g4c_mlp_shapes_enable(int on);
int g4c_mlp_last_shape(void);

int64_t g4c_plan_tiles(const int32_t *off , int32_t n_seg, int32_t max_rows, int32_t *tile_rows ,
                       int32_t *tile_seg , int64_t capacity);

int g4c_layer_norm(const float *x, int32_t x_ld, int64_t n_rows, int32_t width, const float *gamma, const float *beta, float eps,
                   int32_t act, float *out, int32_t out_ld, void *stream);

int g4c_debug_mean_div(const float *a, const int32_t *count, float *out, int64_t n4, void *stream);

int g4c_project_to_edges(const float *v, int32_t v_ld, const int32_t *node, const float *unit,
                         int64_t n_edges, int32_t n_feat, float *out, int32_t out_ld, void *stream);

int g4c_edge_scalar_to_node_vector(const float *e, int32_t e_ld, const float *unit_inv, int32_t k,
                                   int64_t n_nodes, int32_t n_feat, float *out, int32_t out_ld,
                                   void *stream);

int g4c_knn_grid(const float *pos_sorted, const int32_t *cell_sorted, const int32_t *order,
                 const int32_t *cell_start, int64_t n, int32_t dim, const int32_t *n_cells, const float *origin,
                 float cell_size, int32_t k, int64_t *out, void *stream);

int g4c_knn_grid_query(const float *pos_sorted, const int32_t *order, const int32_t *cell_start, int64_t n, int32_t dim,
                       const int32_t *n_cells, const float *origin, float cell_size, const float *q_pos,
                       const int32_t *q_cell, int64_t m, int32_t k, int64_t *out, void *stream);

int g4c_rollout_advance(float *field, int32_t field_cols, const float *pred, int32_t nf,
                        float *outputs, int32_t out_ld, int32_t *step, int64_t n_nodes, void *stream);

int g4c_add_cols(const float *a, int32_t a_ld, int32_t a_col0, const float *b, int32_t b_ld,
                 float *out, int32_t out_ld, int32_t width, int64_t n_rows, void *stream);

int g4c_activation_inplace(float *x, int64_t n, int32_t act, void *stream);

int g4c_copy_cols(const float *src, int32_t src_ld, int32_t scol0, const int32_t *idx,
                  float *dst, int32_t dst_ld, int32_t dcol0, int32_t width, int64_t n_rows, void *stream);


int g4c_train_gather(const float *src, int32_t src_ld, int32_t scol0, const int32_t *idx, int32_t pre_act, int32_t negate,
                     float *dst, int32_t dst_ld, int32_t dcol0, int32_t width, int64_t n_rows, int32_t accumulate, void *stream);

int g4c_act_grad(const float *dy, int32_t dy_ld, const float *ref, int32_t ref_ld, int32_t from_input, int32_t act,
                 float *dz, int32_t dz_ld, int32_t width, int64_t n_rows, void *stream);

int g4c_act_grad_ref16(const float *dy, int32_t dy_ld, const void *ref, int32_t ref_ld, int32_t from_input, int32_t act,
                       float *dz, int32_t dz_ld, int32_t width, int64_t n_rows, void *stream);

int32_t g4c_layernorm_grad_partials(int64_t n_rows);
int g4c_layernorm_grad(const float *z, int32_t z_ld, const float *gamma, const float *dy, int32_t dy_ld, float *dz,
                       int32_t dz_ld, float *partial, int32_t width, int64_t n_rows, float eps, void *stream);

int g4c_layernorm_grad_z16(const void *z, int32_t z_ld, const float *gamma, const float *dy, int32_t dy_ld, float *dz,
                           int32_t dz_ld, float *partial, int32_t width, int64_t n_rows, float eps, void *stream);

int32_t g4c_colsum_partials(int64_t n_rows);
int g4c_colsum(const float *x, int32_t ld, int32_t width, int64_t n_rows, float *scratch, float *out, void *stream);

int32_t g4c_weight_grad_partials(int64_t n_rows);
int64_t g4c_weight_grad_scratch_floats(int64_t n_rows);
int g4c_weight_grad(const float *g, int32_t g_ld, const float *a, int32_t a_ld, int64_t n_rows, float *scratch, float *out,
                    int32_t with_bias, void *stream);

int g4c_weight_grad_bf16(const float *g, int32_t g_ld, const float *a, int32_t a_ld, int64_t n_rows, float *scratch, float *out,
                         int32_t with_bias, void *stream);

int g4c_weight_grad_bf16_a16(const float *g, int32_t g_ld, const void *a, int32_t a_ld, int64_t n_rows, float *scratch, float *out,
                             int32_t with_bias, void *stream);

int g4c_segment_broadcast(const float *dout, int32_t dout_ld, const int32_t *off, const int32_t *perm, int32_t n_seg,
                          int32_t width, int32_t mean, float *dsrc, int32_t dsrc_ld, void *stream);

#ifdef __cplusplus
}
#endif
#endif
```

Baseline: 268.3.

## Precompute static first-layer edge product and run two-layer weight-stationary message kernel

In the first message-passing block, the edge-attribute part of the message MLP's first layer depends only on the static edge attributes. It is now computed once through a static cache and reused. A new weight-stationary kernel variant (PRE) treats that cached product plus the two gathered node products as additive inputs and runs only the remaining two layers with fused aggregation. This drops one 128x128 GEMM over all edges per step, at the cost of a new kernel instantiation, extra register and pipeline code, and cached state that must be invalidated when precision or edge attributes change.

```diff
diff --git a/graphs4cfd_amd/_lib.py b/graphs4cfd_amd/_lib.py
--- a/graphs4cfd_amd/_lib.py
+++ b/graphs4cfd_amd/_lib.py
@@ -18,8 +18,9 @@
 KERNEL_MLP_RS2 = 6
 KERNEL_MLP_BX6, KERNEL_MLP_WS = 2, 4
 KERNEL_MLP_BX6_CERT, KERNEL_MLP_WS_CERT = 7, 8
+KERNEL_MLP_WS_PRE = 9
 KERNEL_NAMES = {0: "none", 1: "mlp_split_kernel", 2: "mlp_bx6_kernel", 3: "mlp_bx6i_kernel", 4: "mlp_ws_kernel", 5: "mlp_rs1_kernel", 6: "mlp_rs2_kernel",
-                7: "mlp_bx6_kernel", 8: "mlp_ws_kernel"}
+                7: "mlp_bx6_kernel", 8: "mlp_ws_kernel", 9: "mlp_ws_kernel"}
 
 TILE_SHAPE_GENERIC, TILE_SHAPE_NODE, TILE_SHAPE_UP, TILE_SHAPE_DOWN = 0, 1, 2, 3
 
diff --git a/graphs4cfd_amd/csrc/mlp_common.h b/graphs4cfd_amd/csrc/mlp_common.h
--- a/graphs4cfd_amd/csrc/mlp_common.h
+++ b/graphs4cfd_amd/csrc/mlp_common.h
@@ -277,6 +277,7 @@
     int fmt;
     bool round1, f16x2, bx6, row_split;
     bool agg, save;
+    bool pre;
     bool all_vec;
     long long row_begin, row_count;
     int io_n_tiles;
@@ -304,6 +305,7 @@
 bool bx6i_takes(const Launch &L);
 int bx6i_launch(const Launch &L, hipStream_t st, Ran &ran);
 bool ws_takes(const Launch &L);
+bool ws_pre_takes(const Launch &L);
 int ws_launch(const Launch &L, hipStream_t st, Ran &ran);
 bool rs_takes(const Launch &L);
 int rs_launch(const Launch &L, hipStream_t st, Ran &ran);
diff --git a/graphs4cfd_amd/csrc/mlp_run.hip b/graphs4cfd_amd/csrc/mlp_run.hip
--- a/graphs4cfd_amd/csrc/mlp_run.hip
+++ b/graphs4cfd_amd/csrc/mlp_run.hip
@@ -112,7 +112,8 @@
         L.all_vec = L.all_vec && d.vec;
         kp += d.wpad;
     }
-    G4C_REQUIRE(nk >= 1 || p.n_nar >= 1, G4C_EINVAL, "g4c_mlp_run: no input block goes through the weights");
+    L.pre = nk == 0 && p.n_nar == 0 && p.n_add >= 1;
+    G4C_REQUIRE(nk >= 1 || p.n_nar >= 1 || L.pre, G4C_EINVAL, "g4c_mlp_run: no input block goes through the weights");
     p.n_src = nk;
     if (nk == 0) p.src[0] = Src{nullptr, nullptr, 0, 0, 0, 0, 1, 0, nullptr, 0, nullptr, 0};
     for (int s = (nk ? nk : 1); s < G4C_MAX_SRC; ++s) p.src[s] = p.src[0];
@@ -280,6 +281,17 @@
 LaunchFn choose(Launch &L) {
     L.deep_ring = L.p.n_tiles <= g_deep_tiles.load(std::memory_order_relaxed);
     L.shapes = g_shapes.load(std::memory_order_relaxed) != 0;
+    if (L.pre) {
+        G4C_REQUIRE(!L.has_node, nullptr, "g4c_mlp_run: every source additive (first layer precomputed) with upd: the fused MP layer has no such form");
+        G4C_REQUIRE(L.f16x2, nullptr, "g4c_mlp_run: every source additive (first layer precomputed) needs the f16x3 format (G4C_WFMT_F16X2), got w_format %d", L.fmt);
+        G4C_REQUIRE(L.p.n_layers == 3, nullptr, "g4c_mlp_run: every source additive (first layer precomputed) needs three layers (two left), got %d", L.p.n_layers);
+        G4C_REQUIRE(L.agg && !L.save, nullptr, "g4c_mlp_run: every source additive (first layer precomputed) needs the fused aggregation and no save");
+        G4C_REQUIRE(ws_pre_takes(L), nullptr,
+                    "g4c_mlp_run: every source additive (first layer precomputed) is outside the weight-stationary kernel's envelope (three aligned "
+                    "128-wide fp32 additive blocks — the first direct, two through indices —, a plain fp32 128-wide output, no heads / residual "
+                    "/ output index / out_dtype)");
+        return ws_launch;
+    }
     if (L.has_node) {
         G4C_REQUIRE(ws_takes(L), nullptr,
                     "g4c_mlp_run: the message launch of the fused MP layer is outside the weight-stationary kernel's envelope (one 128-wide "
diff --git a/graphs4cfd_amd/csrc/mlp_ws.hip b/graphs4cfd_amd/csrc/mlp_ws.hip
--- a/graphs4cfd_amd/csrc/mlp_ws.hip
+++ b/graphs4cfd_amd/csrc/mlp_ws.hip
@@ -155,6 +155,16 @@
             if (SP == 2 && G4C_WS_SCALED && !(G4C_WS_ABLATE & 48)) put_pair_scaled(o.plane_park + u * 16 * PS + 2 * pr, hold, rng);
             else put_pair<SP>(o.plane_park + u * 16 * PS + 2 * pr, hold, rng);
         }
+    } else if (EK == 5) {
+        if ((pc4 & 1) == 0) {
+            f32x2 x;
+            x[0] = xe[u][2 * pr]; x[1] = xe[u][2 * pr + 1];
+            if (SP == 2 && G4C_WS_SCALED && !(G4C_WS_ABLATE & 48)) hold = selu2w_scaled(x);
+            else hold = selu2w(x);
+        } else {
+            if (SP == 2 && G4C_WS_SCALED && !(G4C_WS_ABLATE & 48)) put_pair_scaled(o.plane_acc + u * 16 * PS + 2 * pr, hold, rng);
+            else put_pair<SP>(o.plane_acc + u * 16 * PS + 2 * pr, hold, rng);
+        }
     } else if (EK == 3) {
         if (pc4 == 0) {
             f32x4 x;
@@ -191,6 +201,9 @@
         if constexpr (EK == 4) {
             other_piece<SP, 3, false>(s, accE, accE1, xe, o, hold, rng);
             other_piece<SP, 2, PACT>(s, accE, accE1, xe, o, hold, rng);
+        } else if constexpr (EK == 6) {
+            other_piece<SP, 3, false>(s, accE, accE1, xe, o, hold, rng);
+            other_piece<SP, 5, false>(s, accE, accE1, xe, o, hold, rng);
         } else {
             other_piece<SP, EK, PACT>(s, accE, accE1, xe, o, hold, rng);
         }
@@ -506,12 +519,13 @@
 }
 
 constexpr int G4C_WS_SP1_MINW = 2;
-template <bool AGG, bool DIRECT, bool ADDS, int SP, int NL, bool XB16, bool AB16 = false, bool NODE = false, bool DENSE = false, bool TRACK = true>
-__global__ __launch_bounds__(512, SP == 1 ? G4C_WS_SP1_MINW : 2) void mlp_ws_kernel(const WsKernArgs ka) {
+template <bool AGG, bool DIRECT, bool ADDS, int SP, int NL, bool XB16, bool AB16, bool NODE, bool DENSE, bool TRACK, bool PRE>
+__device__ __forceinline__ void ws_body(const WsKernArgs &ka) {
     const WsArgs &p = ka.a;
     const int n_pairs = ka.n_pairs;
     static_assert((SP == 1 || SP == 2) && (NL == 2 || NL == 3) && (SP == 1 || !XB16) && (SP == 1 || !AB16) && (ADDS || !AB16) &&
                   (!NODE || (AGG && SP == 2)) && (TRACK || SP == 2), "mlp_ws_kernel: unsupported instantiation");
+    static_assert(!PRE || (AGG && DIRECT && ADDS && SP == 2 && NL == 3 && !NODE && TRACK), "mlp_ws_pre_kernel: unsupported instantiation");
     typedef typename std::conditional<AB16, u32x2, f32x4>::type AddV;
     __shared__ __attribute__((aligned(16))) __bf16 sP[2 * TILE_BF16];
     __shared__ __attribute__((aligned(16))) float sF[2 * FIN];
@@ -673,11 +687,11 @@
         store_tables(v1, 1);
     }
 #pragma unroll
-    for (int l = 0; l < NL; ++l)
+    for (int l = PRE ? 1 : 0; l < NL; ++l)
 #pragma unroll
         for (int ks = 0; ks < 4; ++ks)
 #pragma unroll
-            for (int pl = 0; pl < SP; ++pl) W[l][ks][pl] = ldw(rs, lo_b + 1024u * pl, (unsigned)l * 2u * BLOCK6 + (unsigned)ks * 4u * STEP6);
+            for (int pl = 0; pl < SP; ++pl) W[l][ks][pl] = ldw(rs, lo_b + 1024u * pl, (unsigned)(l - (PRE ? 1 : 0)) * 2u * BLOCK6 + (unsigned)ks * 4u * STEP6);
     if (tid < NL * NP) sBias[tid] = p.b[tid];
     if (tid < NP) sZero[tid] = 0.f;
     if (tid < 2 * NP) sGB[tid] = p.gamma ? (tid < NP ? p.gamma[tid] : p.beta[tid - NP]) : 0.f;
@@ -721,6 +735,22 @@
 #pragma unroll
                 for (int e = 0; e < 4; ++e) acc[rb][e] = (acc[rb][e] + a0[e]) + a1[e];
             }
+        }
+    };
+    auto gather_t = [&](const Meta &m, int t, f32x4 (&tv)[2]) __attribute__((always_inline)) {
+        const int nn = m.n[t] > 0 ? m.n[t] : m.n[0];
+#pragma unroll
+        for (int rb = 0; rb < 2; ++rb) {
+            const int r = n + 16 * rb;
+            tv[rb] = *reinterpret_cast<const f32x4 *>(p.x + (long long)(m.r0[t] + (r < nn ? r : nn - 1)) * p.x_ld + fcol);
+        }
+    };
+    auto start_values_pre = [&](f32x4 (&sv)[2], const f32x4 (&tv)[2], const AddV (&a)[2][2]) __attribute__((always_inline)) {
+        if constexpr (PRE) {
+#pragma unroll
+            for (int rb = 0; rb < 2; ++rb)
+#pragma unroll
+                for (int e = 0; e < 4; ++e) sv[rb][e] = (tv[rb][e] + a[rb][0][e]) + a[rb][1][e];
         }
     };
     auto ln_tail = [&](const Meta &mm, const int its) __attribute__((always_inline)) {
@@ -915,7 +945,17 @@
     };
     AddV adB[2][2];
     unsigned rawB[2][2] = {{0u, 0u}, {0u, 0u}};
-    {
+    if constexpr (PRE) {
+        AddV adA[2][2];
+        f32x4 tA[2], tB[2], sA0[2];
+        gather_t(m0, 0, tA);
+        gather_t(m0, 1, tB);
+        gather_adds(0, 0, adA);
+        gather_adds(1, 0, adB);
+        start_values_pre(sA0, tA, adA);
+        other_all<SP, 5, false>(accA, accA1, sA0, oA, rng);
+        start_values_pre(accB, tB, adB);
+    } else {
         AddV adA[2][2];
         unsigned rawA[2][2] = {{0u, 0u}, {0u, 0u}};
         gather_x(m0, 0, 0, xr[0], rawA);
@@ -929,6 +969,52 @@
     }
     __syncthreads();
 
+    if constexpr (PRE) {
+        for (int it = 0, pair = p_begin; pair < p_end; ++pair, ++it) {
+            WS_STAMP(0);
+            Meta m3raw;
+            if constexpr (!DENSE) m3raw = load_meta(pair + 3);
+            const int tv = load_tables(meta_at(pair + 2, m2));
+            f32x4 ntA[2], ntB[2], nsA[2];
+            AddV nadA[2][2];
+            WS_STAMP(1);
+            bias_init(accA, accA1, 1);
+            gather_t(meta_at(pair + 1, m1), 0, ntA);
+            m_block<SP, 5>(paA, W[1], accA, accA1, accA, accA1, accB, oB, rng);
+            bias_init(accB, accB1, 1);
+            __syncthreads();
+            WS_STAMP(2);
+            gather_adds(0, (it + 1) & 1, nadA);
+            m_block<SP, 1>(paB, W[1], accB, accB1, accA, accA1, ntA, oA, rng);
+            bias_init(accA, accA1, 2);
+            __syncthreads();
+            WS_STAMP(3);
+            gather_t(meta_at(pair + 1, m1), 1, ntB);
+            m_block<SP, 1>(paA, W[2], accA, accA1, accB, accB1, ntA, oB, rng);
+            bias_init(accB, accB1, 2);
+            __syncthreads();
+            WS_STAMP(4);
+            start_values_pre(nsA, ntA, nadA);
+            gather_adds(1, (it + 1) & 1, adB);
+            m_block<SP, 6>(paB, W[2], accB, accB1, accA, accA1, nsA, oA, rng);
+            other_all<SP, 3, false>(accB, accB1, nsA, oB, rng);
+            __syncthreads();
+            WS_STAMP(7);
+            start_values_pre(accB, ntB, adB);
+            asm volatile("" : "+v"(accB[0]), "+v"(accB[1]) :: "memory");
+            Meta m3;
+            if constexpr (!DENSE) m3 = fix_meta(m3raw);
+            store_tables(tv, it + 2);
+            WS_STAMP(8);
+            if (!(G4C_WS_ABLATE & 256)) ln_tail(meta_at(pair, m0), it);
+            WS_STAMP(9);
+            __syncthreads();
+            WS_STAMP(15);
+            if (!(G4C_WS_ABLATE & 128)) agg_tail(meta_at(pair, m0), it);
+            WS_STAMP(10);
+            if constexpr (!DENSE) { m0 = m1; m1 = m2; m2 = m3; }
+        }
+    } else
     for (int it = 0, pair = p_begin; pair < p_end; ++pair, ++it) {
         WS_STAMP(0);
         Meta m3raw;
@@ -1017,7 +1103,19 @@
 }
 
 
-#ifdef G4C_WS_ISA_ONLY
+template <bool AGG, bool DIRECT, bool ADDS, int SP, int NL, bool XB16, bool AB16 = false, bool NODE = false, bool DENSE = false, bool TRACK = true>
+__global__ __launch_bounds__(512, SP == 1 ? G4C_WS_SP1_MINW : 2) void mlp_ws_kernel(const WsKernArgs ka) {
+    ws_body<AGG, DIRECT, ADDS, SP, NL, XB16, AB16, NODE, DENSE, TRACK, false>(ka);
+}
+template <bool DENSE>
+__global__ __launch_bounds__(512, 2) void mlp_ws_pre_kernel(const WsKernArgs ka) {
+    ws_body<true, true, true, 2, 3, false, false, false, DENSE, true, true>(ka);
+}
+
+#if defined(G4C_WS_ISA_ONLY) && G4C_WS_ISA_ONLY == 2
+template __global__ void mlp_ws_pre_kernel<true>(const WsKernArgs);
+template __global__ void mlp_ws_pre_kernel<false>(const WsKernArgs);
+#elif defined(G4C_WS_ISA_ONLY)
 template __global__ void mlp_ws_kernel<true, true, true, 2, 3, false, false, false, true, true>(const WsKernArgs);
 template __global__ void mlp_ws_kernel<true, true, true, 2, 3, false, false, false, true, false>(const WsKernArgs);
 template __global__ void mlp_ws_kernel<true, true, true, 2, 3, false, false, true, false, true>(const WsKernArgs);
@@ -1041,8 +1139,40 @@
     return true;
 }
 
+bool ws_pre_takes(const Launch &L) {
+    const Params &p = L.p;
+    if (!L.f16x2 || !L.agg || L.save || L.has_node || p.n_layers != 3) return false;
+    if (p.n_src != 0 || p.n_nar != 0 || p.n_add != 3 || p.n_heads || p.n_out != NP || p.resid || p.out_idx || p.out_bf16) return false;
+    if (p.add[0].idx || !p.add[1].idx || !p.add[2].idx) return false;
+    for (int a = 0; a < 3; ++a)
+        if (p.add[a].width != NP || p.add[a].bf16 || (p.add[a].ld & 3) || ((uintptr_t)p.add[a].ptr & 15)) return false;
+    if (p.out && ((p.out_ld & 3) || ((uintptr_t)p.out & 15))) return false;
+    if (p.gamma && (((uintptr_t)p.gamma & 15) || ((uintptr_t)p.beta & 15))) return false;
+    return ((uintptr_t)p.b & 15) == 0 && p.M < (1LL << 31);
+}
+
 int ws_launch(const Launch &L, hipStream_t st, Ran &ran) {
     const Params &p = L.p;
+    if (L.pre) {
+        const bool dense = p.agg_deg >= 4 && p.agg_deg <= 8;
+        const int n_pairs = dense ? (int)((p.M + 63) / 64) : (p.n_tiles + 1) / 2;
+        const int n_wg = g4c::cu_count();
+        const dim3 grid(n_pairs < n_wg ? n_pairs : n_wg), blk(512);
+        ran.kernel = G4C_KERNEL_MLP_WS_PRE;
+        WsArgs a{};
+        a.x = p.add[0].ptr; a.x_idx = nullptr; a.x_ld = p.add[0].ld; a.x_pact = 0;
+        for (int j = 0; j < 2; ++j) { a.add_ptr[j] = p.add[1 + j].ptr; a.add_idx[j] = p.add[1 + j].idx; a.add_ld[j] = p.add[1 + j].ld; }
+        a.w = p.w; a.b = p.b; a.gamma = p.gamma; a.beta = p.beta; a.eps = p.eps; a.act = p.act;
+        a.out = p.out; a.out_idx = nullptr; a.out_ld = p.out_ld; a.out_bf16 = 0;
+        a.tile_rows = p.tile_rows; a.tile_seg = p.tile_seg; a.seg_off = p.seg_off;
+        a.agg = p.agg; a.agg_ld = p.agg_ld; a.agg_mean = p.agg_mean; a.agg_deg = p.agg_deg;
+        a.M = (int)p.M; a.row_base = (int)p.row_base; a.n_tiles = p.n_tiles;
+        a.range_flag = p.range_certified ? nullptr : p.range_flag; a.range_slot = p.range_slot;
+        const WsKernArgs ka{a, n_pairs, L.node};
+        if (dense) mlp_ws_pre_kernel<true><<<grid, blk, 0, st>>>(ka);
+        else mlp_ws_pre_kernel<false><<<grid, blk, 0, st>>>(ka);
+        return g4c::check_launch("g4c_mlp_run (ws, first layer precomputed)");
+    }
     const bool agg = L.agg, round1 = L.round1, node = L.has_node;
     const bool dense = agg && !node && p.agg_deg >= 4 && p.agg_deg <= 8;
     const int n_pairs = dense ? (int)((p.M + 63) / 64) : (p.n_tiles + 1) / 2;
diff --git a/graphs4cfd_amd/nn/blocks.py b/graphs4cfd_amd/nn/blocks.py
--- a/graphs4cfd_amd/nn/blocks.py
+++ b/graphs4cfd_amd/nn/blocks.py
@@ -523,6 +523,42 @@
     return int(v.size(1)) == 128 and int(e_t.size(1)) == 128 and e_t.dtype == torch.float32
 
 
+def static_first_layer(msg_mlp: MLP, upd_mlp: MLP, e_src: Source, e_static, edge_index: Tensor, n_nodes: int, csr, hoists: bool) -> bool:
+    if not (ops.STATIC_FIRST_LAYER and e_static and ops.StaticCache.active is not None and not ops.grad_mode() and hoists):
+        return False
+    if ops.mlp_precision() != "f16x3" or ops.effective_precision([128]) != "f16x3":
+        return False
+    lm = msg_mlp._linears()
+    if len(lm) != 3 or any(l.out_features != 128 for l in lm) or msg_mlp.input_size != 384:
+        return False
+    if (e_src.pre_act != _lib.ACT_NONE or e_src.index is not None or e_src.col0 != 0 or e_src.negate or e_src.segments is not None
+            or e_src.additive or e_src.width != 128 or e_src.tensor.dtype != torch.float32):
+        return False
+    if will_fuse_layer(msg_mlp, upd_mlp, edge_index, n_nodes):
+        return False
+    return ops.can_fuse_aggregation(csr, msg_mlp.output_size)
+
+
+def _static_first_message(msg_mlp: MLP, e_src: Source, e_static, gathered, n_rows: int, products, gathered_bounds, product_bounds,
+                          agg, store_rows: bool) -> Optional[Tensor]:
+    H = 128
+    first = ops.static_launch(STATIC_FIRST_NAME, list(e_static), lambda: ops.mlp_forward(
+        msg_mlp._image(msg_mlp._spec([H], [False], layers=(0, 1), cols=(0, H), bias=True)), [Source(e_src.tensor, bound=e_src.bound)], n_rows))
+    adds = []
+    for j, (t, idx) in enumerate(gathered):
+        if products is not None:
+            part, part_bound = products[j], (product_bounds[j] if product_bounds is not None else None)
+        else:
+            part = ops.mlp_forward(msg_mlp._packed_cols(H * (1 + j), H * (2 + j), [H], [False], True),
+                                   [Source(t, bound=gathered_bounds[j])], int(t.size(0)))
+            part_bound = ops.take_bounds().out
+        adds.append(Source(part, index=idx, additive=True, bound=part_bound))
+    return ops.mlp_forward_precomputed(msg_mlp._packed_cols(0, H, [H], [False], False), first, adds, n_rows, agg, store_rows=store_rows)
+
+
+STATIC_FIRST_NAME = "first_mp_layer.edge_product"
+
+
 def _fused_layer(msg_mlp: MLP, upd_mlp: MLP, v: Tensor, e_src: Source, ep, csr, mean: bool, act_code: int, products,
                  next_msg: Optional[MLP], keep_e: bool, rb: ops.RangeBounds):
     H = 128
@@ -556,7 +592,7 @@
              products: Optional[Sequence[Tensor]] = None, next_msg: Optional[MLP] = None, keep_e: bool = True,
              n_targets: Optional[int] = None, v_out: Optional[Tensor] = None, compact_messages: bool = False,
              next_graph: Optional[Tuple[int, "plan.CsrPlan"]] = None, compact_v: bool = False,
-             bounds: Optional[ops.RangeBounds] = None):
+             bounds: Optional[ops.RangeBounds] = None, e_static: Optional[Sequence[Tensor]] = None):
     if aggr not in ("mean", "sum", "add"):
         raise ValueError(f"unsupported aggr {aggr!r}")
     n_t = int(v.size(0)) if n_targets is None else int(n_targets)
@@ -572,7 +608,16 @@
         return (v_new, e_new, nxt) if next_msg is not None else (v_new, e_new)
     hoist_kw = dict(gathered_bounds=[rb.v if v_src is None else None, rb.v], product_bounds=rb.products)
     v_in = Source(v, bound=rb.v)
-    if ops.can_fuse_aggregation(csr, msg_mlp.output_size):
+    static_first = (e_static is not None and v_src is None and n_targets is None and v_out is None and not compact_messages
+                    and static_first_layer(msg_mlp, upd_mlp, e_src, e_static, index, int(v.size(0)), csr,
+                                           ep.n_edges >= HOIST_MIN_ROWS or products is not None))
+    if static_first:
+        agg = torch.empty((csr.n_seg, 128), dtype=torch.float32, device=v.device)
+        e_new = _static_first_message(msg_mlp, e_src, e_static, [(senders, ep.row), (v, ep.col)], ep.n_edges, products,
+                                      hoist_kw["gathered_bounds"], hoist_kw["product_bounds"], (csr, agg, mean), keep_e)
+        rb.e = ops.take_bounds().out
+        agg_src = Source(agg, bound=ops.agg_bound(rb.e, csr, mean))
+    elif ops.can_fuse_aggregation(csr, msg_mlp.output_size):
         kw = dict(store_rows=keep_e, rows_dtype=torch.bfloat16 if compact_messages and COMPACT_MESSAGES else None,
                   rows_act=_lib.ACT_SELU if compact_messages and COMPACT_MESSAGES else _lib.ACT_NONE)
         gathered = [(senders, ep.row), (v, ep.col)]
@@ -662,9 +707,9 @@
 
     def step(self, v: Tensor, e: Tensor, edge_index: Tensor, act_code: int, e_pre_act: int = _lib.ACT_NONE,
              products: Optional[Sequence[Tensor]] = None, next_msg: Optional[MLP] = None, keep_e: bool = True,
-             bounds: Optional[ops.RangeBounds] = None):
+             bounds: Optional[ops.RangeBounds] = None, e_static: Optional[Sequence[Tensor]] = None):
         return _mp_step(self.edge_mlp, self.node_mlp, v, e, edge_index, self.aggr, act_code, e_pre_act,
-                        products=products, next_msg=next_msg, keep_e=keep_e, bounds=bounds)
+                        products=products, next_msg=next_msg, keep_e=keep_e, bounds=bounds, e_static=e_static)
 
     def forward(self, v: Tensor, e: Tensor, edge_index: Tensor, *, activation=None) -> Tuple[Tensor, Tensor]:
         return _public_mp(self.edge_mlp, self.node_mlp, v, e, edge_index, self.aggr, activation)
diff --git a/graphs4cfd_amd/nn/mus_gnn.py b/graphs4cfd_amd/nn/mus_gnn.py
--- a/graphs4cfd_amd/nn/mus_gnn.py
+++ b/graphs4cfd_amd/nn/mus_gnn.py
@@ -78,12 +78,14 @@
                 rb.v, rb.products = lb.out, (lb.heads if products is not None else None)
             else:
                 nxt = prog[k + 1] if k + 1 < len(prog) else ""
+                e_static = [graph.edge_attr] if k == 0 else None
                 if nxt.startswith("mp"):
                     v, e, products = block.step(v, e, edge_index, SELU, e_pre_act=e_pending, products=products,
-                                                next_msg=getattr(self, nxt).edge_mlp, bounds=rb)
+                                                next_msg=getattr(self, nxt).edge_mlp, bounds=rb, e_static=e_static)
                 else:
                     drop_e = nxt.startswith("up_mp") or nxt == ""
-                    v, e = block.step(v, e, edge_index, SELU, e_pre_act=e_pending, products=products, keep_e=not drop_e, bounds=rb)
+                    v, e = block.step(v, e, edge_index, SELU, e_pre_act=e_pending, products=products, keep_e=not drop_e, bounds=rb,
+                                      e_static=e_static)
                     products = None
                 e_pending = SELU
         nf = self.num_fields
diff --git a/graphs4cfd_amd/ops.py b/graphs4cfd_amd/ops.py
--- a/graphs4cfd_amd/ops.py
+++ b/graphs4cfd_amd/ops.py
@@ -62,6 +62,9 @@
 
     def __enter__(self):
         self._prev, StaticCache.active = StaticCache.active, self
+        prec = mlp_precision()
+        for name in [n for n, hit in self.store.items() if hit[0][1] != prec]:
+            del self.store[name]
         return self
 
     def __exit__(self, *exc):
@@ -1015,6 +1018,44 @@
         msg.desc.range_certified = upd.desc.range_certified = 0
     _last_bounds = LaunchBounds(None, lb_upd.out, lb_upd.heads, e=lb_msg.out)
     return e_out, v_out, head_outs
+
+
+STATIC_FIRST_LAYER = os.environ.get("G4C_STATIC_FIRST_LAYER", "1") != "0"
+
+
+def mlp_forward_precomputed(packed: PackedMLP, first: Tensor, products: Sequence[Source], n_rows: int,
+                            agg: Tuple[CsrPlan, Tensor, bool], act: int = _lib.ACT_NONE, store_rows: bool = True) -> Optional[Tensor]:
+    global _last_bounds
+    _last_bounds = None
+    csr, agg_out, agg_mean = agg
+    dev = _lib.require_hip(first, agg_out, *[s.tensor for s in products], *[s.index for s in products])
+    if dev != packed.device:
+        raise RuntimeError(f"MLP weights on {packed.device}, inputs on {dev}")
+    if packed.split != "f16x2" or packed.desc.n_layers != 3 or packed.seg_widths != (128,) or packed.n_out != 128 or packed.n_heads:
+        raise NotImplementedError("mlp_forward_precomputed: a three-layer 128-wide MLP over one 128-wide block, packed for f16x3, no heads")
+    if len(products) != 2 or any(not s.additive or s.index is None or s.width != 128 or s.tensor.dtype != torch.float32 for s in products):
+        raise ValueError("mlp_forward_precomputed: two additive 128-wide fp32 sources gathered through an index")
+    first = _rows_f32(first, "first", cols=128, min_rows=n_rows)
+    if csr.tiles() is None or n_rows != csr.n:
+        raise ValueError("mlp_forward_precomputed: the rows must be in segment order with segments of at most 32 rows")
+    if agg_out.dtype != torch.float32:
+        raise TypeError(f"aggregate: expected float32, got {agg_out.dtype}")
+    out = torch.empty((n_rows, 128), dtype=torch.float32, device=dev) if store_rows else None
+    desc = _lib.g4c_mlp_t()
+    C.memmove(C.byref(desc), C.byref(packed.desc), C.sizeof(desc))
+    desc.k_pad[0], desc.w[0], desc.range_certified = 0, packed.desc.w[1], 0
+    srcs = [Source(first, additive=True)] + list(products)
+    io = _lib.g4c_mlp_io_t(act=act, row_count=n_rows, out=_lib.ptr(out), out_ld=128 if out is None else _ld(out))
+    _set_agg(io, csr, agg_out, agg_mean)
+    io.range_flag = _launch_flags(dev).data_ptr()
+    flops = float(2 * 2 * 128 * 128) * n_rows
+    nbytes = 4.0 * 128 * (n_rows * (2 if store_rows else 1) + csr.n_seg)
+    arr = _src_array(srcs)
+    _timed("mlp_bx6_kernel", flops, nbytes, lambda: _lib.check(_lib.load().g4c_mlp_run(C.byref(desc), arr, 3, n_rows, C.byref(io),
+                                                                                       _lib.stream_handle(dev))))
+    ln = packed.norms["ln"] if packed.norms is not None else None
+    _last_bounds = LaunchBounds(None, act_bound((packed.norms["n_out"] - 1) ** 0.5 * ln[0] + ln[1], act) if ln is not None else None)
+    return out
 
 
 def _rows_dtype(what: str, tensors: Sequence[Tensor]) -> int:
diff --git a/include/g4c.h b/include/g4c.h
--- a/include/g4c.h
+++ b/include/g4c.h
@@ -149,6 +149,7 @@
 #define G4C_KERNEL_MLP_RS2 6
 #define G4C_KERNEL_MLP_BX6_CERT 7
 #define G4C_KERNEL_MLP_WS_CERT 8
+#define G4C_KERNEL_MLP_WS_PRE 9
 int g4c_mlp_last_kernel(void);
 
 #define G4C_TILE_SHAPE_GENERIC 0
```

Result: faster. 273.0 (median of 6 runs) (+1.7%).
